# buckbaskin/parakeet_slam

Measured on AMD Instinct MI355X. Metric: particle*landmark EKF updates/sec (whole filter step), higher is better.
Workload: dtype f64

## Files before the change

### include/parakeet_slam.h

```cpp
#ifndef PARAKEET_SLAM_H_
#define PARAKEET_SLAM_H_

#include <stddef.h>
#include <stdint.h>

#ifdef __cplusplus
extern "C" {
#endif
#if defined(__GNUC__)
#pragma GCC visibility push(default)
#endif

#define PK_ABI_VERSION 1

typedef enum pk_status {
  PK_OK = 0,
  PK_ERR_INVALID = -1,
  PK_ERR_HIP = -2,
  PK_ERR_STATE = -3,
  PK_ERR_UNSUPPORTED = -4,
  PK_ERR_NOMEM = -5
} pk_status;

#define PK_LANDMARK_POTENTIAL 0x40000000
// ... 109 lines not shown
int pk_shard_plan_balanced_dev(pk_filter* f, const double* dev_global_state, int64_t global_particles, const double* dev_gmax,
                               int32_t weight_domain, double u, int32_t world, int32_t rank, int64_t* dev_table);
int pk_shard_pack_balanced_dev(pk_filter* f, const int64_t* table, int32_t world, int32_t rank, void* dev_buf);
int pk_shard_adopt_balanced_dev(pk_filter* f, const int64_t* table, int32_t world, int32_t rank, const void* dev_recv,
                                int64_t n_received, int32_t mode);
int pk_shard_pack_balanced_loop_dev(pk_filter* f, int64_t keep, int64_t a0, int64_t a1, void* dev_buf);
int pk_shard_download_logical(pk_filter* f, int64_t* logical);
int pk_shard_upload_logical(pk_filter* f, const int64_t* logical);
int pk_shard_download_balanced_plan(pk_filter* f, int64_t* rel, int64_t* Hl, int32_t* alive);
int pk_shard_reset_placement(pk_filter* f);
int pk_shard_download_balanced_offspring(pk_filter* f, int64_t global_particles, int64_t* H);
int pk_shard_balanced_errors(pk_filter* f, int64_t* count);

#define PK_PROBE_LEN 79
int pk_probe(int32_t device, const double pose[3], const double mean[5], const double cov[25],
             const double blob[4], const double Qt[16], double* out);

int pk_enable_timing(pk_filter* f, int32_t mask);
int pk_reset_timings(pk_filter* f);
int pk_timings(pk_filter* f, double ms[PK_T_COUNT], int64_t launches[PK_T_COUNT]);
int pk_observe_bytes(const pk_filter* f, int32_t num_blobs, int64_t* algorithmic, int64_t* moved);
enum {
  PK_ROUTE_NONE = 0,
  PK_ROUTE_KNOWN_IDS = 1,
  PK_ROUTE_ML_GENERAL = 2,
  PK_ROUTE_ML_HANDOFF = 3,
  PK_ROUTE_ML_SWEEP = 4,
  PK_ROUTE_ML_FUSED = 5,
  PK_ROUTE_ML_REGS = 6,
  PK_ROUTE_DENSE = 8,
  PK_ROUTE_ML_PUB_BIG = 9,
};
int pk_observe_route(const pk_filter* f);
int pk_download_sources(pk_filter* f, int32_t* src);
int pk_observe_flagged(pk_filter* f, int64_t* flagged, int64_t* cand_overflow);
int pk_observe_retry_rows(pk_filter* f, int64_t* wanted, int64_t* capacity);
int pk_observe_published(pk_filter* f, int32_t* published);
int pk_observe_pub_stats(pk_filter* f, int64_t stats[6]);
int pk_observe_flags(pk_filter* f, uint8_t* flags);

typedef struct pk_rng pk_rng;
int pk_rng_create_numpy(uint32_t seed, pk_rng** out);
int pk_rng_create_python(uint32_t seed, pk_rng** out);
int pk_rng_destroy(pk_rng* r);
int pk_rng_standard_normal(pk_rng* r, int64_t n, double* out);
int pk_rng_random(pk_rng* r, int64_t n, double* out);

#if defined(__GNUC__)
#pragma GCC visibility pop
#endif
#ifdef __cplusplus
}
#endif
#endif
```

### parakeet_slam_amd/_lib.py

```python
from __future__ import annotations

import ctypes as C
import os

import numpy as np

HERE = os.path.dirname(os.path.abspath(__file__))
LIB_PATH = os.path.join(HERE, "libparakeet_slam.so")

PK_OK = 0
PK_ERR_INVALID, PK_ERR_HIP, PK_ERR_STATE, PK_ERR_UNSUPPORTED, PK_ERR_NOMEM = -1, -2, -3, -4, -5
PK_WEIGHTS_LINEAR, PK_WEIGHTS_LOG = 0, 1
PK_LANDMARK_POTENTIAL = 0x40000000
PK_T_NAMES = ("motion", "assoc", "observe", "weights", "resample", "summary", "materialise")
PK_T_COUNT = len(PK_T_NAMES)
PK_PROBE_LEN = 79
PK_ABI_VERSION = 1

_dp = C.POINTER(C.c_double)
_ip = C.POINTER(C.c_int32)
_lp = C.POINTER(C.c_int64)
_bp = C.POINTER(C.c_uint8)
_h = C.c_void_p

# ... 43 lines not shown
    "pk_shard_plan_global_dev": (C.c_int, [_h, C.c_void_p, C.c_int64, C.c_void_p, C.c_int32, C.c_double, C.c_int32, C.c_int32,
                                           C.c_void_p]),
    "pk_shard_download_offspring": (C.c_int, [_h, _lp]),
    "pk_shard_pack_dev": (C.c_int, [_h, _lp, C.c_int32, C.c_int32, C.c_void_p]),
    "pk_shard_pack_slots_dev": (C.c_int, [_h, C.c_int64, C.c_int64, C.c_int64, C.c_int64, C.c_void_p]),
    "pk_shard_adopt_dev": (C.c_int, [_h, C.c_int32, C.c_void_p, C.c_int64]),
    "pk_shard_local_span_dev": (C.c_int, [_h, C.c_void_p]),
    "pk_shard_adopt_local_dev": (C.c_int, [_h, C.c_int32]),
    "pk_shard_adopt_remote_dev": (C.c_int, [_h, C.c_int32, C.c_void_p, C.c_int64]),
    "pk_shard_state_dev": (C.c_int, [_h, C.c_void_p]),
    "pk_shard_plan_balanced_dev": (C.c_int, [_h, C.c_void_p, C.c_int64, C.c_void_p, C.c_int32, C.c_double, C.c_int32, C.c_int32,
                                             C.c_void_p]),
    "pk_shard_pack_balanced_dev": (C.c_int, [_h, _lp, C.c_int32, C.c_int32, C.c_void_p]),
    "pk_shard_adopt_balanced_dev": (C.c_int, [_h, _lp, C.c_int32, C.c_int32, C.c_void_p, C.c_int64, C.c_int32]),
    "pk_shard_pack_balanced_loop_dev": (C.c_int, [_h, C.c_int64, C.c_int64, C.c_int64, C.c_void_p]),
    "pk_shard_download_logical": (C.c_int, [_h, _lp]),
    "pk_shard_reset_placement": (C.c_int, [_h]),
    "pk_shard_upload_logical": (C.c_int, [_h, _lp]),
    "pk_shard_download_balanced_plan": (C.c_int, [_h, _lp, _lp, _ip]),
    "pk_shard_download_balanced_offspring": (C.c_int, [_h, C.c_int64, _lp]),
    "pk_shard_balanced_errors": (C.c_int, [_h, _lp]),
    "pk_motion_range": (C.c_int, [_h, C.c_double, C.c_double, C.c_double, C.c_uint64, C.c_uint64, C.c_int64, C.c_int64]),
    "pk_staged_takes_regs": (C.c_int, [_h]),
    "pk_observe_staged_range": (C.c_int, [_h, C.c_int32, C.c_int64, C.c_int64, C.c_int32, C.c_int32]),
    "pk_particle_bytes": (C.c_int64, [_h]),
    "pk_pack_particles": (C.c_int, [_h, _lp, C.c_int64, C.c_void_p]),
    "pk_adopt_particles": (C.c_int, [_h, _lp, C.c_void_p, C.c_int64]),
    "pk_probe": (C.c_int, [C.c_int32, _dp, _dp, _dp, _dp, _dp, _dp]),
    "pk_enable_timing": (C.c_int, [_h, C.c_int32]),
    "pk_reset_timings": (C.c_int, [_h]),
    "pk_timings": (C.c_int, [_h, _dp, _lp]),
    "pk_observe_bytes": (C.c_int, [_h, C.c_int32, _lp, _lp]),
    "pk_observe_route": (C.c_int, [_h]),
    "pk_download_sources": (C.c_int, [_h, _ip]),
    "pk_observe_flagged": (C.c_int, [_h, _lp, _lp]),
    "pk_observe_retry_rows": (C.c_int, [_h, _lp, _lp]),
    "pk_grow_enable": (C.c_int, [_h, C.c_int32, C.c_int32, C.c_double]),
    "pk_grow_download": (C.c_int, [_h, C.c_int64, C.c_int64, _ip, _dp, _ip]),
    "pk_grow_upload": (C.c_int, [_h, C.c_int64, C.c_int64, _ip, _dp, _ip]),
    "pk_grow_shape": (C.c_int, [_h, C.POINTER(C.c_int32), C.POINTER(C.c_int32), C.POINTER(C.c_int32)]),
    "pk_observe_published": (C.c_int, [_h, C.POINTER(C.c_int32)]),
    "pk_observe_flags": (C.c_int, [_h, _bp]),
    "pk_observe_pub_stats": (C.c_int, [_h, _lp]),
    "pk_rng_create_numpy": (C.c_int, [C.c_uint32, C.POINTER(_h)]),
    "pk_rng_create_python": (C.c_int, [C.c_uint32, C.POINTER(_h)]),
    "pk_rng_destroy": (C.c_int, [_h]),
    "pk_rng_standard_normal": (C.c_int, [_h, C.c_int64, _dp]),
    "pk_rng_random": (C.c_int, [_h, C.c_int64, _dp]),
}


class PkError(RuntimeError):
    def __init__(self, status, message):
        super().__init__("parakeet_slam [%d]: %s" % (status, message))
        self.status = status


_lib = None


def load():
    global _lib
    if _lib is not None:
        return _lib
    if not os.path.exists(LIB_PATH):
        raise OSError(
# ... 264 lines not shown

    def shard_download_balanced_plan(self):
        rel, Hl, alive = np.empty(self.P + 1, dtype=np.int64), np.empty(self.P, dtype=np.int64), np.empty(self.P, dtype=np.int32)
        check(self._lib.pk_shard_download_balanced_plan(self._h, lptr(rel), lptr(Hl), iptr(alive)))
        return rel, Hl, alive[alive >= 0]

    def reset_placement(self):
        check(self._lib.pk_shard_reset_placement(self._h))

    def shard_download_balanced_offspring(self, global_particles):
        out = np.empty(int(global_particles) + 1, dtype=np.int64)
        check(self._lib.pk_shard_download_balanced_offspring(self._h, int(global_particles), lptr(out)))
        return out

    def shard_balanced_errors(self):
        out = np.zeros(1, dtype=np.int64)
        check(self._lib.pk_shard_balanced_errors(self._h, lptr(out)))
        return int(out[0])

    def motion_range(self, v, w, dt, seed, draw, p0, p1):
        check(self._lib.pk_motion_range(self._h, float(v), float(w), float(dt), int(seed), int(draw), int(p0), int(p1)))

    def staged_takes_regs(self):
        return bool(self._lib.pk_staged_takes_regs(self._h))

    def observe_staged_range(self, fresh, p0, p1, first, last):
        check(self._lib.pk_observe_staged_range(self._h, 1 if fresh else 0, int(p0), int(p1), 1 if first else 0, 1 if last else 0))

    ROUTES = {0: "none", 1: "known_ids", 2: "ml_general", 3: "ml_handoff", 4: "ml_sweep", 5: "ml_fused", 6: "ml_regs", 8: "dense", 9: "ml_pub_big"}

    def observe_route(self):
        return self.ROUTES[int(self._lib.pk_observe_route(self._h))]

    def observe_flagged(self):
        a, b = C.c_int64(), C.c_int64()
        check(self._lib.pk_observe_flagged(self._h, C.byref(a), C.byref(b)))
        return int(a.value), int(b.value)

    def observe_pub_stats(self):
        a = np.zeros(6, dtype=np.int64)
        check(self._lib.pk_observe_pub_stats(self._h, lptr(a)))
        return dict(zip(("entries", "contested_blobs", "multi_landmarks", "longest_list", "entry_capacity", "instance"), (int(v) for v in a)))

    def grow_enable(self, preset_landmarks, reading_capacity=64, pair_threshold=30.0):
        check(self._lib.pk_grow_enable(self._h, int(preset_landmarks), int(reading_capacity), float(pair_threshold)))

    def grow_shape(self):
        a, b, c = C.c_int32(), C.c_int32(), C.c_int32()
        check(self._lib.pk_grow_shape(self._h, C.byref(a), C.byref(b), C.byref(c)))
        return int(a.value), int(b.value), int(c.value)

    def grow_download(self, p0=0, p1=None, counters=True, readings=True, slot_ids=True):
        p1 = self.P if p1 is None else p1
        _, S, R = self.grow_shape()
        n = p1 - p0
        c = np.empty((n, 4), dtype=np.int32) if counters else None
        r = np.empty((n, R, 8), dtype=np.float64) if readings else None
        s = np.empty((n, S), dtype=np.int32) if slot_ids else None
        check(self._lib.pk_grow_download(self._h, int(p0), int(p1), iptr(c), dptr(r), iptr(s)))
        return c, r, s

    def grow_upload(self, p0, p1, counters=None, readings=None, slot_ids=None):
        _, S, R = self.grow_shape()
        n = p1 - p0
        c = None if counters is None else np.ascontiguousarray(counters, dtype=np.int32).reshape(n, 4)
        r = None if readings is None else f64(readings, (n, R, 8))
# ... 94 lines not shown
```

### parakeet_slam_amd/build.py

```python
from __future__ import annotations

import os
import shutil
import subprocess
import sys

_NO_LICM = ["-mllvm", "-disable-machine-licm"]
EXTRA_FLAGS = {"pk_k_observe_ml.hip": _NO_LICM, "pk_k_step_pub.hip": _NO_LICM, "pk_k_cand_entries.hip": _NO_LICM, "pk_k_assoc.hip": _NO_LICM}

HERE = os.path.dirname(os.path.abspath(__file__))
CSRC = os.path.join(HERE, "csrc")
LIB = os.path.join(HERE, "libparakeet_slam.so")
OBJDIR = os.path.join(HERE, "csrc", "_obj")

HIP_SOURCES = ["pk_k_motion.hip", "pk_k_assoc.hip", "pk_k_observe.hip", "pk_k_observe_ml.hip", "pk_k_step_pub.hip", "pk_k_cand_entries.hip", "pk_k_dense.hip", "pk_k_resample.hip", "pk_k_grow.hip", "pk_api.hip"]
CXX_SOURCES = ["pk_rng.cpp"]
HEADERS = [
    "pk_math.hpp", "pk_layout.hpp", "pk_kernels.hpp", "pk_philox.hpp", "pk_device.hpp", "pk_pub_math.hpp", "pk_pub_layout.hpp", "pk_k_step_duo.inl",
    os.path.join("..", "..", "include", "parakeet_slam.h"),
]

HIPCC_FLAGS = [
    "--offload-arch=gfx950", "-O3", "-std=c++17", "-fPIC", "-fvisibility=hidden",
    "-Wall", "-Wno-unused-function",
    "-ffp-contract=on",
]


def _hipcc():
    for cand in (os.environ.get("HIPCC"), shutil.which("hipcc"), "/opt/rocm/bin/hipcc"):
        if cand and os.path.exists(cand):
            return cand
    raise RuntimeError("hipcc not found (set HIPCC or add /opt/rocm/bin to PATH)")


def _stale(target, deps):
    if not os.path.exists(target):
        return True
    t = os.path.getmtime(target)
    return any(os.path.getmtime(d) > t for d in deps)


CXX_FLAGS = ["-x", "c++", "-O2", "-std=c++17", "-fPIC", "-fvisibility=hidden", "-ffp-contract=off", "-Wall"]


def _cxx_objects(hipcc, verbose=True):
    os.makedirs(OBJDIR, exist_ok=True)
    objs = []
# ... 68 lines not shown
```

### parakeet_slam_amd/csrc/pk_api.hip

```cpp
#include <hip/hip_runtime.h>

#include <cmath>
#include <cstdarg>
#include <cstdio>
#include <cstring>
#include <new>
#include <string>
#include <vector>

#include "../../include/parakeet_slam.h"
#include "pk_kernels.hpp"

using namespace pk;

extern "C" {
int pk_download_landmarks(pk_filter* f, int64_t p0, int64_t p1, double* means, double* covs, int32_t* counts);
int pk_upload_landmarks(pk_filter* f, int64_t p0, int64_t p1, const double* means, const double* covs, const int32_t* counts);
}

#ifdef PK_STAMPS
namespace pk { void debug_read_stamps(unsigned long long* out, bool reset); void debug_read_fused_stamps(unsigned long long* out, bool reset); void debug_read_regs_stamps(unsigned long long* out, bool reset); void debug_read_pub_stamps(unsigned long long* out, bool reset); void debug_read_pub_wave_stamps(unsigned long long* out, bool reset); }
#endif

namespace {
// ... 83 lines not shown
  int64_t* rlohi_dev = nullptr;
  int64_t rlohi_cap = 0;
  BalancedBuffers bal{};
  int64_t bal_m = -1;
  int64_t bal_loop_keep = -1;
  int assoc_kernel = 0;
  int assoc_dup = 1;
  struct Staged {
    bool valid = false;
    int B = 0;
    unsigned char* st = nullptr;
    int slot = 0;
    BlobGrid g{};
    int n9 = 0;
    bool use_grid = false;
    size_t tab_bytes = 0;
    bool uploaded = false;
  } staged;
  int route = PK_ROUTE_NONE;
  int upload_kernel = 1;
  int fused_step = 1;
  unsigned* bcnt_dev = nullptr;
  uint4* brec_dev = nullptr;
  int64_t bcand_cap = 0;
  int cand_lists = 1;
  int64_t loop_lo = INT64_MIN, loop_hi = INT64_MAX;
  uint4* cand_dev = nullptr;
  int regs_step = 1;
  int pub_step = 1;
  bool flag_folded = false;
  int pub_small = -1;
  int duo_park_limit = -1;
  int duo_on = 0;
  int pub_entry_limit = 0;
  uint4* erec_dev = nullptr;
  uint4* erec_dev2 = nullptr;
  unsigned* binfo_dev = nullptr;
  unsigned char* npass_dev = nullptr;
  unsigned* unm_dev = nullptr;
  int unm_words = 0;
  int64_t unm_cap = 0;
  bool grow_bits = false;
  uint4* prim_dev = nullptr;
  float4* gate4_dev = nullptr;
  uint4* far_dev = nullptr;
  int far_prune = 1;
  unsigned* glist_dev = nullptr;
  struct Split {
    bool active = false;
    AssocLaunch al;
    CandTable cand;
    int B = 0;
    bool reset = false;
  } split;
  bool adopt_local_done = false;
  int pub_ecap = 0;
  int split_reserve_cus = 16;
  int regs_retry = 1;
  int regs_warm = 1;
  int fast_observe = 1;
  uint4* sweep_results = nullptr;
  size_t sweep_cap = 0;
  unsigned* retry_seen = nullptr;
  int64_t retry_rows_min = 0;
  FastHandoff fh{};
  int64_t fh_cap_l = 0, fh_cap_b = 0;
// ... 153 lines not shown
    f->stage_cap = cap;
  }
  int i = f->stage_next;
  f->stage_next = (i + 1) % pk_filter::kRing;
  const uint64_t need = f->slot_seq[i];
  if (need != 0) {
    int ev = -1;
    for (int j = 0; j < pk_filter::kRing; ++j)
      if (f->event_seq[j] >= need && (ev < 0 || f->event_seq[j] < f->event_seq[ev])) ev = j;
    if (ev < 0) {
      PK_HIP(hipEventRecord(f->stage_done[i], f->stream));
      f->event_seq[i] = f->upload_seq;
      ev = i;
    }
    PK_HIP(hipEventSynchronize(f->stage_done[ev]));
    f->slot_seq[i] = 0;
  }
  *out = f->stage[i];
  *slot = i;
  return PK_OK;
}

int materialise(pk_filter* f) {
  if (f->src_identity) return PK_OK;
  {
    Span t(f, PK_T_MATERIALISE);
    launch_materialise(f->stream, f->d);
  }
  f->src_identity = true;
  f->d.alt = nullptr;
  return PK_OK;
}

void pack_landmark(const MapLayout& lay, unsigned char* slot, int l, const double* mean, const double* cov) {
  double* fl = reinterpret_cast<double*>(slot);
  const int Lp = lay.Lp;
  for (int i = 0; i < 5; ++i) fl[(size_t)i * Lp + l] = mean[i];
  if (lay.fields == kDenseFields) {
    for (int i = 0; i < 25; ++i) fl[(size_t)(5 + i) * Lp + l] = cov[i];
    return;
  }
  fl[(size_t)F_PXX * Lp + l] = cov[0];
  fl[(size_t)F_PXY * Lp + l] = 0.5 * (cov[1] + cov[5]);
  fl[(size_t)F_PYY * Lp + l] = cov[6];
  fl[(size_t)F_CRR * Lp + l] = cov[12];
  fl[(size_t)F_CRG * Lp + l] = 0.5 * (cov[13] + cov[17]);
  fl[(size_t)F_CRB * Lp + l] = 0.5 * (cov[14] + cov[22]);
  fl[(size_t)F_CGG * Lp + l] = cov[18];
  fl[(size_t)F_CGB * Lp + l] = 0.5 * (cov[19] + cov[23]);
  fl[(size_t)F_CBB * Lp + l] = cov[24];
}

void unpack_landmark(const MapLayout& lay, const unsigned char* slot, int l, double* mean, double* cov) {
  const double* fl = reinterpret_cast<const double*>(slot);
  const int Lp = lay.Lp;
  if (mean)
    for (int i = 0; i < 5; ++i) mean[i] = fl[(size_t)i * Lp + l];
  if (cov && lay.fields == kDenseFields) {
    for (int i = 0; i < 25; ++i) cov[i] = fl[(size_t)(5 + i) * Lp + l];
  } else if (cov) {
    for (int i = 0; i < 25; ++i) cov[i] = 0.0;
    cov[0] = fl[(size_t)F_PXX * Lp + l];
    cov[1] = cov[5] = fl[(size_t)F_PXY * Lp + l];
    cov[6] = fl[(size_t)F_PYY * Lp + l];
    cov[12] = fl[(size_t)F_CRR * Lp + l];
    cov[13] = cov[17] = fl[(size_t)F_CRG * Lp + l];
// ... 255 lines not shown
        (!onepass_only || (step_pub_entry_capacity(B) > 0 && regs_cand_lds_bytes(f->d.lay.Lp, B) <= kMaxDynLds && B <= 32 * 96))) {
      out->retry = f->regs_retry && observe_sweep_plan(f->d, B).grid > 0;
      if ((rc = ensure_handoff(f, B, out->retry ? kSweepSlots : kFastSlots, out->retry, true))) return rc;
      out->regs = true;
      out->grid = g;
      out->n9 = n9;
      out->tables = f->scan_dev + o_tab;
      out->exact = reinterpret_cast<const double*>(f->scan_dev + o_exact);
      const size_t cs_b = ((size_t)(g.ncell + 1) * 2 + 15) & ~(size_t)15;
      out->order = reinterpret_cast<const unsigned short*>(f->scan_dev + o_tab + cs_b + (size_t)B * 16 + (size_t)n9 * 2);
      return PK_OK;
    }
    if (out && want_fast && !finalize && f->fast_observe == 1 && f->pub_step && f->cand_lists && f->d.lay.L > kRegsMaxL &&
        f->d.lay.L <= kPubBigMaxL && B > 0 && step_pub_big_entry_capacity(B) > 0 && observe_sweep_plan(f->d, B).grid > 0 && pub_ok) {
      if ((rc = ensure_handoff(f, B, kSweepSlots, true, true))) return rc;
      out->big = true;
      out->retry = true;
      out->grid = g;
      out->n9 = n9;
      out->tables = f->scan_dev + o_tab;
      out->exact = reinterpret_cast<const double*>(f->scan_dev + o_exact);
      const size_t cs_b = ((size_t)(g.ncell + 1) * 2 + 15) & ~(size_t)15;
      out->order = reinterpret_cast<const unsigned short*>(f->scan_dev + o_tab + cs_b + (size_t)B * 16 + (size_t)n9 * 2);
      return PK_OK;
    }
    if (want_fast && !onepass_only && !finalize && f->fast_observe && B > 0 &&
        (sweep ? observe_sweep_plan(f->d, B).grid > 0 : observe_fast_lds_bytes(B) <= kMaxDynLds)) {
      const int slots = (sweep && (B >= 3000 || f->fast_observe == 3)) ? kSweepSlots : kFastSlots;
      if ((rc = ensure_handoff(f, B, slots))) return rc;
      f->fh.slots = slots;
      fh = f->fh;
      fh.n_flagged = ctl_n_flagged(f);
    }
    Span t(f, PK_T_ASSOC);
    CandTable cand;
    if (fh.lmpass && f->cand_lists && f->d.lay.L < 65535) {
      if (!f->cand_dev && (rc = dev_alloc(f, &f->cand_dev, ((size_t)f->d.lay.Lp + kCandSpare) * 3))) return rc;
      launch_summary_partials(f->stream, f->d, f->partial, f->out4);
      launch_candidates(f->stream, f->d, B, reinterpret_cast<const double*>(f->scan_dev + o_exact), 0, f->cand_dev, ctl_cand_over(f),
                        nullptr, nullptr, nullptr, 2 * kCandSlots, f->out4);
      cand.rec = f->cand_dev;
      cand.over = ctl_cand_over(f);
      cand.slots = 2 * kCandSlots;
    }
    launch_assoc_grid(f->stream, f->d, B, g, n9, f->scan_dev + o_tab, reinterpret_cast<const double*>(f->scan_dev + o_exact),
                      f->ids_dev, finalize, fh, cand);
    if (out) {
      out->fast = fh.lmpass != nullptr;
      out->exact = reinterpret_cast<const double*>(f->scan_dev + o_exact);
      const size_t cs_b = ((size_t)(g.ncell + 1) * 2 + 15) & ~(size_t)15;
      out->order = reinterpret_cast<const unsigned short*>(f->scan_dev + o_tab + cs_b + (size_t)B * 16 + (size_t)n9 * 2);
    }
    return PK_OK;
  }
  if (assoc_brute_lds_bytes(B) > kMaxDynLds)
    return fail(PK_ERR_UNSUPPORTED,
                "maximum-likelihood association of %d blobs: neither the colour-grid tables nor the brute-force kernel's "
                "%zu bytes of per-blob state fit the workgroup's %zu bytes of LDS", B, assoc_brute_lds_bytes(B), (size_t)kMaxDynLds);
  Span t(f, PK_T_ASSOC);
  launch_assoc_brute(f->stream, f->d, blobs_dev, dir_dev, B, f->ids_dev);
  return PK_OK;
}

int classify_covariance(const double* cov, int l) {
  double scale = 0.0;
  for (int i = 0; i < 25; ++i) {
    if (!std::isfinite(cov[i])) return fail(PK_ERR_INVALID, "landmark %d: covariance not finite", l + 1);
    if (i % 6 == 0) scale = fmax(scale, fabs(cov[i]));
  }
  const double tol = 1e-9 * (scale > 0 ? scale : 1.0);
  for (int i = 0; i < 2; ++i)
    for (int j = 2; j < 5; ++j)
      if (fabs(cov[i * 5 + j]) > 1e-14 * scale || fabs(cov[j * 5 + i]) > 1e-14 * scale) return 1;
  for (int i = 0; i < 5; ++i)
    for (int j = i + 1; j < 5; ++j)
      if (fabs(cov[i * 5 + j] - cov[j * 5 + i]) > tol) return 1;
  return 0;
}

int check_block_diagonal(const double* cov, int l) {
  double scale = 0.0;
  for (int i = 0; i < 5; ++i) scale = fmax(scale, fabs(cov[i * 6]));
  if (!(scale >= 0.0) || !std::isfinite(scale))
    return fail(PK_ERR_INVALID, "landmark %d: covariance diagonal is not finite", l + 1);
  const double tol = 1e-9 * (scale > 0 ? scale : 1.0);
  for (int i = 0; i < 2; ++i)
    for (int j = 2; j < 5; ++j)
      if (fabs(cov[i * 5 + j]) > 1e-14 * scale || fabs(cov[j * 5 + i]) > 1e-14 * scale)
        return fail(PK_ERR_UNSUPPORTED,
                    "landmark %d: covariance couples position and colour (entry [%d][%d]); the compact "
                    "device layout holds xy 2x2 (+) rgb 3x3 only",
                    l + 1, i, j);
  for (int i = 0; i < 5; ++i)
    for (int j = i + 1; j < 5; ++j) {
      if (!std::isfinite(cov[i * 5 + j])) return fail(PK_ERR_INVALID, "landmark %d: covariance not finite", l + 1);
      if (fabs(cov[i * 5 + j] - cov[j * 5 + i]) > tol)
        return fail(PK_ERR_UNSUPPORTED, "landmark %d: covariance is not symmetric", l + 1);
    }
  return PK_OK;
}

int relayout(pk_filter* f, bool dense, bool keep) {
  if (f->dense == dense) return PK_OK;
  int rc;
  DeviceState& d = f->d;
  const MapLayout old = d.lay;
  const MapLayout neu = MapLayout::make(old.L, sizeof(double), dense ? kDenseFields : (int)F_COUNT_FIELDS);
  const int64_t P = d.P;
  const int L = old.L;
  std::vector<double> means, covs;
  std::vector<int32_t> counts;
  if (keep && L > 0) {
    if ((rc = materialise(f))) return rc;
    if (!dense)
      return fail(PK_ERR_STATE, "relayout: a dense map cannot be folded back into the compact layout");
    try {
      means.resize((size_t)P * L * 5);
      covs.resize((size_t)P * L * 25);
      counts.resize((size_t)P * L);
    } catch (const std::bad_alloc&) {
      return fail(PK_ERR_NOMEM, "relayout: no host memory to stage %lld x %d landmarks for the layout conversion", (long long)P, L);
    }
    if ((rc = pk_download_landmarks(f, 0, P, means.data(), covs.data(), counts.data()))) return rc;
  }
  PK_HIP(hipStreamSynchronize(f->stream));
  for (int i = 0; i < 2; ++i) {
    if (d.map[i]) (void)hipFree(d.map[i]);
    d.map[i] = nullptr;
    f->device_bytes -= (int64_t)((size_t)P * old.slot_bytes);
  }
  if (f->slot_tmp) (void)hipFree(f->slot_tmp);
  f->slot_tmp = nullptr;
  f->device_bytes -= (int64_t)old.slot_bytes;
  d.lay = neu;
  f->dense = dense;
  d.alt = nullptr;
  for (int i = 0; i < 2; ++i) {
// ... 120 lines not shown
  }
  for (auto e : f->pool) (void)hipEventDestroy(e);
  DeviceState& d = f->d;
  for (int i = 0; i < 2; ++i) {
    (void)hipFree(d.x[i]);
    (void)hipFree(d.y[i]);
    (void)hipFree(d.h[i]);
    (void)hipFree(d.logw[i]);
    (void)hipFree(d.src[i]);
    (void)hipFree(d.map[i]);
  }
  if (f->scan_dev) (void)hipFree(f->scan_dev);
  for (void* q : {(void*)f->fh.lmpass, (void*)f->fh.bcount, (void*)f->fh.pflag, (void*)f->fh.row_of, (void*)f->sweep_results, (void*)f->cand_dev, (void*)f->bcnt_dev, (void*)f->brec_dev, (void*)f->erec_dev, (void*)f->erec_dev2, (void*)f->binfo_dev, (void*)f->glist_dev, (void*)f->gate4_dev, (void*)f->npass_dev, (void*)f->far_dev, (void*)f->prim_dev, (void*)f->unm_dev})
    if (q) (void)hipFree(q);
  for (int i = 0; i < 2; ++i)
    for (void* q : {(void*)f->grow.hyp[i], (void*)f->grow.cnt[i], (void*)f->grow.slot_id[i]})
      if (q) (void)hipFree(q);
  for (void* q : {(void*)f->g_totals, (void*)f->g_offsets, (void*)f->hi_dev, (void*)f->gl_clocal, (void*)f->gl_totals, (void*)f->gl_offsets, (void*)f->plan_ticket, (void*)f->idx_dev, (void*)f->srcs_dev, (void*)f->rlohi_dev})
    if (q) (void)hipFree(q);
  for (void* q : {(void*)d.logical[0], (void*)d.logical[1], (void*)f->bal.glogw, (void*)f->bal.clocal, (void*)f->bal.totals, (void*)f->bal.offsets,
                  (void*)f->bal.sum, (void*)f->bal.H, (void*)f->bal.cloc, (void*)f->bal.ctot, (void*)f->bal.coff, (void*)f->bal.rel, (void*)f->bal.Hl,
                  (void*)f->bal.alive, (void*)f->bal.bad})
    if (q) (void)hipFree(q);
  void* rest[] = {d.immutable, f->z_dev,  f->ids_dev,
                  f->partial,  f->gmax,   f->clocal,    f->totals,      f->offsets,   f->sum,      f->out4, f->pose_part,
                  f->anc,      f->slot_tmp};
  for (void* p : rest)
    if (p) (void)hipFree(p);
  for (int i = 0; i < pk_filter::kRing; ++i) {
    if (f->stage[i]) (void)hipHostFree(f->stage[i]);
    if (f->stage_done[i]) (void)hipEventDestroy(f->stage_done[i]);
  }
  if (f->retry_seen) (void)hipHostFree(f->retry_seen);
  if (f->own_stream) (void)hipStreamDestroy(f->own_stream);
  delete f;
  return PK_OK;
}

int pk_set_stream(pk_filter* f, void* hip_stream) {
  if (!f) return fail(PK_ERR_INVALID, "pk_set_stream: NULL handle");
  int rc;
  if ((rc = use_device(f))) return rc;
  if ((rc = drain_timings(f))) return rc;
  PK_HIP(hipStreamSynchronize(f->stream));
  f->stream = hip_stream ? (hipStream_t)hip_stream : f->own_stream;
  return PK_OK;
}

int pk_synchronize(pk_filter* f) {
  if (!f) return fail(PK_ERR_INVALID, "pk_synchronize: NULL handle");
  int rc;
  if ((rc = use_device(f))) return rc;
  PK_HIP(hipStreamSynchronize(f->stream));
  return PK_OK;
}

int64_t pk_num_particles(const pk_filter* f) { return f ? f->d.P : -1; }
int32_t pk_num_landmarks(const pk_filter* f) { return f ? f->d.lay.L : -1; }
int64_t pk_device_bytes(const pk_filter* f) { return f ? f->device_bytes : -1; }

int pk_set_measurement_noise(pk_filter* f, const double Qt[16]) {
  if (!f || !Qt) return fail(PK_ERR_INVALID, "pk_set_measurement_noise: NULL argument");
  for (int i = 0; i < 16; ++i)
    if (!std::isfinite(Qt[i])) return fail(PK_ERR_INVALID, "Qt is not finite");
  double scale = 0;
  for (int i = 0; i < 4; ++i) scale = fmax(scale, fabs(Qt[i * 5]));
  bool coupled = false;
  for (int j = 1; j < 4; ++j)
    if (fabs(Qt[j]) > 1e-14 * scale || fabs(Qt[j * 4]) > 1e-14 * scale) coupled = true;
  for (int i = 1; i < 4; ++i)
    for (int j = i + 1; j < 4; ++j)
      if (fabs(Qt[i * 4 + j] - Qt[j * 4 + i]) > 1e-9 * (scale > 0 ? scale : 1.0)) coupled = true;
  int rc;
  if ((rc = use_device(f))) return rc;
  if (coupled && !f->dense && (rc = relayout(f, true, f->map_loaded))) return rc;
  for (int i = 0; i < 16; ++i) f->qt16[i] = Qt[i];
  f->qt_dense = coupled;
  f->qt = NoiseD{Qt[0], Qt[5], 0.5 * (Qt[6] + Qt[9]), 0.5 * (Qt[7] + Qt[13]), Qt[10], 0.5 * (Qt[11] + Qt[14]), Qt[15]};
  return PK_OK;
}

int pk_upload_map(pk_filter* f, const double* means, const double* covs, const uint8_t* immutable) {
  if (!f) return fail(PK_ERR_INVALID, "pk_upload_map: NULL handle");
  const MapLayout& lay = f->d.lay;
  const int L = lay.L;
  if (L > 0 && (!means || !covs)) return fail(PK_ERR_INVALID, "pk_upload_map: NULL means/covs");
  int rc;
  if ((rc = use_device(f))) return rc;
  bool need_dense = f->qt_dense;
  for (int l = 0; l < L; ++l) {
    for (int i = 0; i < 5; ++i)
      if (!std::isfinite(means[l * 5 + i])) return fail(PK_ERR_INVALID, "landmark %d: mean is not finite", l + 1);
    const int c = classify_covariance(covs + (size_t)l * 25, l);
    if (c < 0) return c;
    need_dense |= c == 1;
  }
  if ((rc = relayout(f, need_dense, false))) return rc;
  std::vector<unsigned char> slot(lay.slot_bytes, 0);
  std::vector<unsigned char> imm((size_t)lay.Lp, 0);
  for (int l = 0; l < L; ++l) {
    pack_landmark(lay, slot.data(), l, means + (size_t)l * 5, covs + (size_t)l * 25);
    imm[l] = immutable ? (immutable[l] != 0) : 0;
  }
  PK_HIP(hipMemcpyAsync(f->slot_tmp, slot.data(), lay.slot_bytes, hipMemcpyHostToDevice, f->stream));
  PK_HIP(hipMemcpyAsync(f->d.immutable, imm.data(), imm.size(), hipMemcpyHostToDevice, f->stream));
  launch_broadcast_slot(f->stream, f->d, f->slot_tmp);
  PK_HIP(hipStreamSynchronize(f->stream));
  f->src_identity = true;
  f->map_loaded = true;
  return PK_OK;
}

int pk_upload_poses(pk_filter* f, const double* xyhw) {
  if (f) f->pose_part_ok = false;
  if (!f || !xyhw) return fail(PK_ERR_INVALID, "pk_upload_poses: NULL argument");
  int rc;
  if ((rc = use_device(f))) return rc;
  const int64_t P = f->d.P;
  std::vector<double> soa((size_t)P * 4);
  for (int64_t i = 0; i < P; ++i) {
    soa[i] = xyhw[4 * i];
    soa[P + i] = xyhw[4 * i + 1];
    soa[2 * P + i] = xyhw[4 * i + 2];
    double w = xyhw[4 * i + 3];
    if (!(w >= 0.0) || !std::isfinite(w)) return fail(PK_ERR_INVALID, "pk_upload_poses: weight of particle %lld is negative, infinite or NaN", (long long)i);
    soa[3 * P + i] = std::log(w);
  }
  const int c = f->d.cur;
  PK_HIP(hipMemcpyAsync(f->d.x[c], soa.data(), P * 8, hipMemcpyHostToDevice, f->stream));
  PK_HIP(hipMemcpyAsync(f->d.y[c], soa.data() + P, P * 8, hipMemcpyHostToDevice, f->stream));
  PK_HIP(hipMemcpyAsync(f->d.h[c], soa.data() + 2 * P, P * 8, hipMemcpyHostToDevice, f->stream));
  PK_HIP(hipMemcpyAsync(f->d.logw[c], soa.data() + 3 * P, P * 8, hipMemcpyHostToDevice, f->stream));
  PK_HIP(hipStreamSynchronize(f->stream));
  f->gmax_fused = false;
  return PK_OK;
}

int pk_upload_pose(pk_filter* f, int64_t p, const double xyhw[4]) {
  if (!f || !xyhw) return fail(PK_ERR_INVALID, "pk_upload_pose: NULL argument");
// ... 20 lines not shown
  const int64_t P = f->d.P;
  std::vector<double> soa((size_t)P * 4);
  const int c = f->d.cur;
  PK_HIP(hipMemcpyAsync(soa.data(), f->d.x[c], P * 8, hipMemcpyDeviceToHost, f->stream));
  PK_HIP(hipMemcpyAsync(soa.data() + P, f->d.y[c], P * 8, hipMemcpyDeviceToHost, f->stream));
  PK_HIP(hipMemcpyAsync(soa.data() + 2 * P, f->d.h[c], P * 8, hipMemcpyDeviceToHost, f->stream));
  PK_HIP(hipMemcpyAsync(soa.data() + 3 * P, f->d.logw[c], P * 8, hipMemcpyDeviceToHost, f->stream));
  PK_HIP(hipStreamSynchronize(f->stream));
  for (int64_t i = 0; i < P; ++i) {
    xyhw[4 * i] = soa[i];
    xyhw[4 * i + 1] = soa[P + i];
    xyhw[4 * i + 2] = soa[2 * P + i];
    xyhw[4 * i + 3] = std::exp(soa[3 * P + i]);
  }
  return PK_OK;
}

int pk_download_log_weights(pk_filter* f, double* logw) {
  if (!f || !logw) return fail(PK_ERR_INVALID, "pk_download_log_weights: NULL argument");
  int rc;
  if ((rc = use_device(f))) return rc;
  PK_HIP(hipMemcpyAsync(logw, f->d.logw[f->d.cur], (size_t)f->d.P * sizeof(double), hipMemcpyDeviceToHost, f->stream));
  PK_HIP(hipStreamSynchronize(f->stream));
  return PK_OK;
}

int pk_download_landmarks(pk_filter* f, int64_t p0, int64_t p1, double* means, double* covs, int32_t* counts) {
  if (!f) return fail(PK_ERR_INVALID, "pk_download_landmarks: NULL handle");
  if (p0 < 0 || p1 < p0 || p1 > f->d.P) return fail(PK_ERR_INVALID, "pk_download_landmarks: bad particle range");
  if (!f->map_loaded) return fail(PK_ERR_STATE, "pk_download_landmarks: no map uploaded");
  int rc;
  if ((rc = use_device(f))) return rc;
  if ((rc = materialise(f))) return rc;
  const MapLayout& lay = f->d.lay;
  const int L = lay.L;
  const int64_t chunk = std::max<int64_t>(1, (int64_t)(64u << 20) / (int64_t)lay.slot_bytes);
  std::vector<unsigned char> host((size_t)std::min<int64_t>(chunk, p1 - p0) * lay.slot_bytes);
  for (int64_t q0 = p0; q0 < p1; q0 += chunk) {
    int64_t q1 = std::min(p1, q0 + chunk);
    PK_HIP(hipMemcpyAsync(host.data(), f->d.map[f->d.mcur] + (size_t)q0 * lay.slot_bytes,
                          (size_t)(q1 - q0) * lay.slot_bytes, hipMemcpyDeviceToHost, f->stream));
    PK_HIP(hipStreamSynchronize(f->stream));
    for (int64_t q = q0; q < q1; ++q) {
      const unsigned char* slot = host.data() + (size_t)(q - q0) * lay.slot_bytes;
      const int32_t* cnt = reinterpret_cast<const int32_t*>(slot + lay.count_off);
      for (int l = 0; l < L; ++l) {
        size_t o = (size_t)(q - p0) * L + l;
        unpack_landmark(lay, slot, l, means ? means + o * 5 : nullptr, covs ? covs + o * 25 : nullptr);
        if (counts) counts[o] = cnt[l];
      }
    }
  }
  return PK_OK;
}

int pk_upload_landmarks(pk_filter* f, int64_t p0, int64_t p1, const double* means, const double* covs,
                        const int32_t* counts) {
  if (!f) return fail(PK_ERR_INVALID, "pk_upload_landmarks: NULL handle");
  if (p0 < 0 || p1 < p0 || p1 > f->d.P) return fail(PK_ERR_INVALID, "pk_upload_landmarks: bad particle range");
  if (!f->map_loaded) return fail(PK_ERR_STATE, "pk_upload_landmarks: no map uploaded");
  int rc;
  if ((rc = use_device(f))) return rc;
  if ((rc = materialise(f))) return rc;
  const int L = f->d.lay.L;
  if (means)
    for (int64_t o = 0; o < (p1 - p0) * L * 5; ++o)
      if (!std::isfinite(means[o])) return fail(PK_ERR_INVALID, "pk_upload_landmarks: mean of landmark %d not finite", (int)((o / 5) % L) + 1);
  if (covs) {
    bool need_dense = false;
    for (int64_t o = 0; o < (p1 - p0) * L; ++o) {
      const int c = classify_covariance(covs + (size_t)o * 25, (int)(o % L));
      if (c < 0) return c;
      need_dense |= c == 1;
    }
    if (need_dense && !f->dense && (rc = relayout(f, true, true))) return rc;
  }
  const MapLayout& lay = f->d.lay;
  const int64_t chunk = std::max<int64_t>(1, (int64_t)(64u << 20) / (int64_t)lay.slot_bytes);
  std::vector<unsigned char> host;
  try {
    host.resize((size_t)std::min<int64_t>(chunk, p1 - p0) * lay.slot_bytes);
  } catch (const std::bad_alloc&) {
    return fail(PK_ERR_NOMEM, "pk_upload_landmarks: no host memory for the staging buffer");
  }
  for (int64_t q0 = p0; q0 < p1; q0 += chunk) {
    int64_t q1 = std::min(p1, q0 + chunk);
    unsigned char* dev = f->d.map[f->d.mcur] + (size_t)q0 * lay.slot_bytes;
    PK_HIP(hipMemcpyAsync(host.data(), dev, (size_t)(q1 - q0) * lay.slot_bytes, hipMemcpyDeviceToHost, f->stream));
    PK_HIP(hipStreamSynchronize(f->stream));
    for (int64_t q = q0; q < q1; ++q) {
      unsigned char* slot = host.data() + (size_t)(q - q0) * lay.slot_bytes;
      int32_t* cnt = reinterpret_cast<int32_t*>(slot + lay.count_off);
      for (int l = 0; l < L; ++l) {
        size_t o = (size_t)(q - p0) * L + l;
        double m[5], c[25];
// ... 205 lines not shown
      const bool fold = whole && (far != nullptr || f->grow_on || al.fused);
      launch_cand_entries(f->stream, f->d, B, f->cand_dev, f->erec_dev, f->bcnt_dev, f->brec_dev, f->binfo_dev, f->glist_dev, ctl_cand_over(f),
                          ctl_skip_pub(f), ctl_skip_cand(f), ecap, kCandSlots, nullptr, nullptr, f->npass_dev, far != nullptr, ctl_pub_stats(f),
                          nullptr, nullptr, DuoLimits(), nullptr, fold ? f->fh.pflag : nullptr, fold ? ctl_n_flagged(f) : nullptr);
      f->flag_folded = fold;
      cand->far = far;
      cand->skip_cand = ctl_skip_cand(f);
      f->pub_ecap = ecap;
    } else {
      launch_candidates(f->stream, f->d, B, al.exact, ref, f->cand_dev, ctl_cand_over(f), nullptr, nullptr, nullptr, kCandSlots, f->out4, nullptr, nullptr, part);
    }
  }
  return PK_OK;
}
static int onepass_launch(pk_filter* f, const AssocLaunch& al, int B, const ObserveExtras& ex, const CandTable& cand, int64_t p0,
                          int64_t p1, int reserve_cus = 0) {
  FastHandoff fh = f->fh;
  fh.n_flagged = ctl_n_flagged(f);
  fh.flags_only = true;
  Span t(f, PK_T_OBSERVE);
  ObserveExtras e1 = ex;
  e1.flip = false;
  if (al.big) {
    const DuoLimits duo = duo_limits(f, B);
    if (duo.tbytes > 0)
      launch_step_pub_duo(f->stream, f->d, B, al.exact, al.order, fh, f->qt, e1, cand, f->erec_dev2, f->glist_dev, ctl_skip_duo(f), ctl_pub_stats(f), duo,
                          f->gate4_dev, f->prim_dev, p0, p1, reserve_cus);
    launch_step_pub_big(f->stream, f->d, B, al.exact, al.order, fh, f->qt, e1, cand, f->erec_dev2, f->glist_dev, ctl_skip_big(f), f->pub_ecap, f->gate4_dev,
                        p0, p1, reserve_cus, f->prim_dev, ctl_pub_stats(f));
    if (!f->flag_folded) launch_flag_range_if(f->stream, ctl_skip_pub(f), fh.pflag, fh.n_flagged, p0, p1);
  } else if (al.regs) {
    if (f->pub_ecap > 0 && cand.rec)
      launch_step_pub(f->stream, f->d, B, al.exact, al.order, fh, f->qt, e1, cand, f->erec_dev, f->glist_dev, ctl_skip_pub(f), f->pub_ecap,
                      p0, p1, reserve_cus);
    if ((cand.far || f->grow_on) && f->pub_ecap > 0) {
      if (!f->flag_folded) launch_flag_range_if(f->stream, ctl_skip_pub(f), fh.pflag, fh.n_flagged, p0, p1);
    } else
      launch_step_regs(f->stream, f->d, B, al.grid, al.n9, al.tables, al.exact, al.order, fh, f->qt, e1, f->regs_warm, cand, p0, p1,
                       reserve_cus);
  } else {
    if (f->pub_ecap > 0 && cand.rec)
      launch_step_pub(f->stream, f->d, B, al.exact, al.order, fh, f->qt, e1, cand, f->erec_dev, f->glist_dev, ctl_skip_pub(f), f->pub_ecap,
                      p0, p1, reserve_cus);
    if (f->pub_ecap > 0 && cand.rec) {
      if (!f->flag_folded) launch_flag_range_if(f->stream, ctl_skip_pub(f), fh.pflag, fh.n_flagged, p0, p1);
    } else
      launch_step_fused(f->stream, f->d, B, al.grid, al.n9, al.tables, al.exact, al.order, fh, f->qt, e1,
                        (f->pub_ecap > 0 && cand.rec) ? ctl_skip_pub(f) : nullptr);
  }
  return PK_OK;
}
static int onepass_finish(pk_filter* f, const AssocLaunch& al, int B, const ObserveExtras& ex, const CandTable& cand) {
  int rc;
  FastHandoff fh = f->fh;
  fh.n_flagged = ctl_n_flagged(f);
  fh.flags_only = true;
  if ((al.regs || al.big) && al.retry) {
    Span t(f, PK_T_ASSOC);
    const SweepPlan plan = observe_sweep_plan(f->d, B);
    const size_t need = (size_t)plan.grid * plan.results_per_wg;
    if (need > f->sweep_cap) {
      PK_HIP(hipStreamSynchronize(f->stream));
      if (f->sweep_results) (void)hipFree(f->sweep_results);
      f->sweep_results = nullptr;
      f->sweep_cap = 0;
      if ((rc = dev_alloc(f, &f->sweep_results, need))) return rc;
      f->sweep_cap = need;
    }
    FastHandoff fr = f->fh;
    fr.slots = kSweepSlots;
    fr.retry = true;
    fr.n_flagged = ctl_n_flagged(f);
    fr.row_next = ctl_retry_rows(f);
    fr.row_cap = retry_rows(f);
    launch_assoc_grid(f->stream, f->d, B, al.grid, al.n9, al.tables, al.exact, f->ids_dev, false, fr, cand.far ? CandTable{} : cand);
    ObserveExtras e3 = ex;
// ... 9 lines not shown
  launch_assoc_grid(f->stream, f->d, B, al.grid, al.n9, al.tables, al.exact, f->ids_dev, false, fh);
  ObserveExtras e2 = ex;
  e2.only_flagged = f->fh.pflag;
  e2.n_flagged = ctl_n_flagged(f);
  launch_observe(f->stream, f->d, al.blobs, al.dir, B, nullptr, nullptr, 0, f->ids_dev, f->qt, e2);
  return PK_OK;
}

static int observe_impl(pk_filter* f, const double* blobs, int32_t B, const int32_t* ids, int32_t* ids_out,
                        bool reset) {
  if (!f) return fail(PK_ERR_INVALID, "pk_observe: NULL handle");
  if (B < 0 || (B > 0 && !blobs)) return fail(PK_ERR_INVALID, "pk_observe: bad blobs");
  if (!f->map_loaded) return fail(PK_ERR_STATE, "pk_observe: no map uploaded (pk_upload_map)");
  if (f->split.active) return fail(PK_ERR_STATE, "pk_observe: a split observe is in progress (pk_observe_staged_range with last = 1 ends it)");
  int rc;
  if ((rc = use_device(f))) return rc;
  const MapLayout& lay = f->d.lay;
  const int L = lay.L;
  for (int i = 0; i < 4 * B; ++i)
    if (!std::isfinite(blobs[i])) return fail(PK_ERR_INVALID, "pk_observe: blob %d is not finite", i / 4);
  static const int32_t no_ids = 0;
  if (!ids && B == 0) ids = &no_ids;
  if (ids)
    for (int b = 0; b < B; ++b)
      if (ids[b] < 0 || ids[b] > L) return fail(PK_ERR_INVALID, "pk_observe: ids[%d] = %d outside 0..%d", b, ids[b], L);
  const bool grow = f->grow_on && B > 0;
  if (grow && ids) return fail(PK_ERR_STATE, "pk_observe: the new-landmark bookkeeping (pk_grow_enable) follows the maximum-likelihood association: no ids");
  if (grow && f->dense)
    return fail(PK_ERR_STATE, "pk_observe: the new-landmark bookkeeping (pk_grow_enable) writes the compact landmark layout; this filter "
                              "is on the dense one (a covariance or Qt that couples position and colour)");
  if (f->dense) return dense_observe(f, blobs, B, ids, ids_out, reset, true);
  ObserveExtras ex;
  ex.reset = reset;
  if (ids) {
    f->staged.valid = false;
    const size_t o_blobs = kCtlBytes;
    const size_t o_first = o_blobs + (size_t)B * 4 * sizeof(double);
    const size_t o_next = o_first + (size_t)lay.Lp * sizeof(int32_t);
    const size_t total = o_next + (size_t)B * sizeof(int32_t);
    unsigned char* st = nullptr;
    int slot = 0;
    if ((rc = take_stage(f, total, &st, &slot))) return rc;
    if ((rc = ensure_scan_capacity(f, total))) return rc;
    memset(st, 0, kCtlBytes);
    if (B > 0) memcpy(st + o_blobs, blobs, (size_t)B * 4 * sizeof(double));
    int32_t* first = reinterpret_cast<int32_t*>(st + o_first);
    int32_t* next = reinterpret_cast<int32_t*>(st + o_next);
    std::vector<int32_t> last((size_t)lay.Lp, -1);
    for (int l = 0; l < lay.Lp; ++l) first[l] = -1;
    int n0 = 0;
    ex.single_sightings = true;
    for (int b = 0; b < B; ++b) {
      next[b] = -1;
      int id = ids[b];
      if (id == 0) {
        ++n0;
        continue;
      }
      if (first[id - 1] < 0) {
        first[id - 1] = b;
      } else {
        next[last[id - 1]] = b;
        ex.single_sightings = false;
      }
      last[id - 1] = b;
    }
// ... 11 lines not shown
    f->d.alt = nullptr;
    f->gmax_fused = true;
    f->route = PK_ROUTE_KNOWN_IDS;
    if (ids_out)
      for (int64_t p = 0; p < f->d.P; ++p) memcpy(ids_out + (size_t)p * B, ids, (size_t)B * 4);
    return PK_OK;
  }
  AssocLaunch al;
  if ((rc = enqueue_association(f, blobs, B, false, ids_out == nullptr, &al, grow))) return rc;
  f->grow_bits = false;
  if (grow && (al.fused || al.regs || al.big)) {
    al.retry = false;
    const int words = 2 * ((B + 63) / 64);
    if ((int64_t)f->d.P * words > f->unm_cap) {
      PK_HIP(hipStreamSynchronize(f->stream));
      if (f->unm_dev) (void)hipFree(f->unm_dev);
      f->unm_dev = nullptr;
      f->unm_cap = 0;
      const int64_t cap = (int64_t)f->d.P * (words + words / 4 + 2);
      if ((rc = dev_alloc(f, &f->unm_dev, (size_t)cap))) return rc;
      f->unm_cap = cap;
    }
    f->unm_words = words;
    ex.unm = f->unm_dev;
    ex.unm_words = words;
    f->grow_bits = true;
  }
  ex.gmax_key = ctl_gmax_key(f);
  f->route = al.big ? PK_ROUTE_ML_PUB_BIG
             : al.fused ? PK_ROUTE_ML_FUSED
             : al.regs ? PK_ROUTE_ML_REGS
             : !al.fast ? PK_ROUTE_ML_GENERAL
             : (f->d.lay.L > kFastMaxL || f->fast_observe >= 2) ? PK_ROUTE_ML_SWEEP : PK_ROUTE_ML_HANDOFF;
  if (al.fused || al.regs || al.big) {
    CandTable cand;
    if ((rc = onepass_prepare(f, al, B, &cand, 0, true))) return rc;
    if ((rc = onepass_launch(f, al, B, ex, cand, 0, f->d.P))) return rc;
    if ((rc = onepass_finish(f, al, B, ex, cand))) return rc;
  } else {
    Span t(f, PK_T_OBSERVE);
    if (al.fast) {
      ObserveExtras e1 = ex;
      e1.flip = false;
      if (f->d.lay.L > kFastMaxL || f->fast_observe >= 2) {
        const SweepPlan plan = observe_sweep_plan(f->d, B);
        const size_t need = (size_t)plan.grid * plan.results_per_wg;
        if (need > f->sweep_cap) {
          PK_HIP(hipStreamSynchronize(f->stream));
          if (f->sweep_results) (void)hipFree(f->sweep_results);
          f->sweep_results = nullptr;
          f->sweep_cap = 0;
          if ((rc = dev_alloc(f, &f->sweep_results, need))) return rc;
          f->sweep_cap = need;
        }
        launch_observe_sweep(f->stream, f->d, B, al.exact, al.order, f->fh, f->qt, e1, plan, f->sweep_results);
      } else {
        launch_observe_fast(f->stream, f->d, B, al.exact, al.order, f->fh, f->qt, e1);
      }
      ObserveExtras e2 = ex;
      e2.only_flagged = f->fh.pflag;
      e2.n_flagged = ctl_n_flagged(f);
      launch_observe(f->stream, f->d, al.blobs, al.dir, B, nullptr, nullptr, 0, f->ids_dev, f->qt, e2);
    } else {
      launch_observe(f->stream, f->d, al.blobs, al.dir, B, nullptr, nullptr, 0, f->ids_dev, f->qt, ex);
    }
  }
  PK_LAUNCH_CHECK("pk_observe");
  f->src_identity = true;
  f->d.alt = nullptr;
  f->gmax_fused = true;
  if (grow) {
// ... 26 lines not shown
  int rc;
  if ((rc = use_device(f))) return rc;
  if (f->dense) {
    f->dense_staged.assign(blobs, blobs + 4 * (size_t)B);
    return PK_OK;
  }
  f->dense_staged.clear();
  return stage_ml_scan(f, blobs, B);
}

int pk_observe_staged(pk_filter* f, int32_t fresh) {
  if (!f) return fail(PK_ERR_INVALID, "pk_observe_staged: NULL handle");
  if (f->dense && !f->dense_staged.empty()) {
    std::vector<double> b;
    b.swap(f->dense_staged);
    return observe_impl(f, b.data(), (int32_t)(b.size() / 4), nullptr, nullptr, fresh != 0);
  }
  if (!f->staged.valid) return fail(PK_ERR_STATE, "pk_observe_staged: no staged scan (pk_stage_scan)");
  const double* blobs = reinterpret_cast<const double*>(f->staged.st + kCtlBytes);
  return observe_impl(f, blobs, f->staged.B, nullptr, nullptr, fresh != 0);
}

int pk_staged_takes_regs(pk_filter* f) {
  if (!f || f->dense || f->grow_on || !f->staged.valid || !f->staged.use_grid) return 0;
  return regs_route_taken(f, f->staged.g, f->staged.B, f->staged.n9) ? 1 : 0;
}

int pk_observe_staged_range(pk_filter* f, int32_t fresh, int64_t p0, int64_t p1, int32_t first, int32_t last) {
  if (!f) return fail(PK_ERR_INVALID, "pk_observe_staged_range: NULL handle");
  if (p0 < 0 || p1 < p0 || p1 > f->d.P) return fail(PK_ERR_INVALID, "pk_observe_staged_range: bad particle range [%lld, %lld)", (long long)p0, (long long)p1);
  if (f->grow_on) return fail(PK_ERR_STATE, "pk_observe_staged_range: the new-landmark bookkeeping (pk_grow_enable) runs behind whole observes (pk_observe / pk_observe_staged)");
  int rc;
  if ((rc = use_device(f))) return rc;
  pk_filter::Split& sp = f->split;
  if (first) {
    if (sp.active) return fail(PK_ERR_STATE, "pk_observe_staged_range: the previous split observe was not finished (last = 1)");
    if (!pk_staged_takes_regs(f))
      return fail(PK_ERR_STATE, "pk_observe_staged_range: needs a staged scan that takes the register route (pk_staged_takes_regs)");
    const double* blobs = reinterpret_cast<const double*>(f->staged.st + kCtlBytes);
    sp.B = f->staged.B;
    sp.reset = fresh != 0;
    sp.al = AssocLaunch();
    if ((rc = enqueue_association(f, blobs, sp.B, false, true, &sp.al))) return rc;
    if (!sp.al.regs && !sp.al.big) return fail(PK_ERR_STATE, "pk_observe_staged_range: the scan did not take the register route");
    f->route = sp.al.big ? PK_ROUTE_ML_PUB_BIG : PK_ROUTE_ML_REGS;
    sp.cand = CandTable();
    if ((rc = onepass_prepare(f, sp.al, sp.B, &sp.cand, p1 > p0 ? p0 : 0))) return rc;
    sp.active = true;
  } else if (!sp.active) {
    return fail(PK_ERR_STATE, "pk_observe_staged_range: no split observe in progress (first = 1)");
  }
  ObserveExtras ex;
  ex.reset = sp.reset;
  ex.gmax_key = ctl_gmax_key(f);
  if (p1 > p0 && (rc = onepass_launch(f, sp.al, sp.B, ex, sp.cand, p0, p1, (first && !last) ? f->split_reserve_cus : 0))) {
    sp.active = false;
    return rc;
  }
  if (last) {
    sp.active = false;
    if ((rc = onepass_finish(f, sp.al, sp.B, ex, sp.cand))) return rc;
    PK_LAUNCH_CHECK("pk_observe_staged_range");
    f->src_identity = true;
    f->d.alt = nullptr;
    f->gmax_fused = true;
  }
  return PK_OK;
}

int pk_motion_range(pk_filter* f, double v, double w, double dt, uint64_t seed, uint64_t draw, int64_t p0, int64_t p1) {
  if (f) f->pose_part_ok = false;
  if (!f) return fail(PK_ERR_INVALID, "pk_motion_range: NULL handle");
  if (!std::isfinite(v) || !std::isfinite(w) || !std::isfinite(dt)) return fail(PK_ERR_INVALID, "pk_motion_range: non-finite control");
  if (p0 < 0 || p1 < p0 || p1 > f->d.P) return fail(PK_ERR_INVALID, "pk_motion_range: bad particle range [%lld, %lld)", (long long)p0, (long long)p1);
  int rc;
  if ((rc = use_device(f))) return rc;
  Span t(f, PK_T_MOTION);
  launch_motion_range(f->stream, f->d, v, w, dt, seed, draw, p0, p1);
  PK_LAUNCH_CHECK("pk_motion_range");
  return PK_OK;
}

int pk_associate(pk_filter* f, const double* blobs, int32_t B, int32_t* ids_out) {
  if (!f || !ids_out) return fail(PK_ERR_INVALID, "pk_associate: NULL argument");
  if (B < 0 || (B > 0 && !blobs)) return fail(PK_ERR_INVALID, "pk_associate: bad blobs");
  if (!f->map_loaded) return fail(PK_ERR_STATE, "pk_associate: no map uploaded (pk_upload_map)");
  if (B == 0) return PK_OK;
  int rc;
  if ((rc = use_device(f))) return rc;
  for (int i = 0; i < 4 * B; ++i)
    if (!std::isfinite(blobs[i])) return fail(PK_ERR_INVALID, "pk_associate: blob %d is not finite", i / 4);
  if (f->dense) return dense_observe(f, blobs, B, nullptr, ids_out, false, false);
  if ((rc = enqueue_association(f, blobs, B, true, false, nullptr))) return rc;
  PK_LAUNCH_CHECK("pk_associate");
  PK_HIP(hipMemcpyAsync(ids_out, f->ids_dev, (size_t)f->d.P * B * 4, hipMemcpyDeviceToHost, f->stream));
  PK_HIP(hipStreamSynchronize(f->stream));
  return PK_OK;
}

int pk_set_option(pk_filter* f, const char* name, int64_t value) {
  if (!f || !name) return fail(PK_ERR_INVALID, "pk_set_option: NULL argument");
  if (!strcmp(name, "assoc_kernel")) {
    if (value != 0 && value != 1) return fail(PK_ERR_INVALID, "assoc_kernel: 0 (colour grid) or 1 (brute force)");
    f->assoc_kernel = (int)value;
    return PK_OK;
  }
  if (!strcmp(name, "fast_observe")) {
    if (value < 0 || value > 3)
      return fail(PK_ERR_INVALID, "fast_observe: 0 (general kernels), 1 (default), 2 (always the sweep kernel) or 3 (... with eight slots)");
    f->fast_observe = (int)value;
    return PK_OK;
  }
  if (!strcmp(name, "timing_stride")) {
    if (value < 1 || value > 1000000) return fail(PK_ERR_INVALID, "timing_stride: 1 .. 1000000");
    f->timing_stride = (int)value;
    return PK_OK;
  }
  if (!strcmp(name, "upload_kernel")) {
    f->upload_kernel = value != 0;
    return PK_OK;
  }
  if (!strcmp(name, "fused_step")) {
    f->fused_step = value != 0;
    return PK_OK;
  }
  if (!strcmp(name, "cand_lists")) {
    f->cand_lists = value != 0;
    return PK_OK;
  }
  if (!strcmp(name, "pub_step")) {
    f->pub_step = value != 0;
    return PK_OK;
  }
  if (!strcmp(name, "pub_small")) {
// ... 148 lines not shown
        {
          Span t(f, PK_T_MOTION);
          launch_motion(f->stream, f->d, v, w, dt, nullptr, seed, draw, 0, f->scan_dev, dev_view, staged_upload_bytes(sg), f->pose_part);
      f->pose_part_ok = true;
        }
        sg.uploaded = true;
        f->gmax_fused = false;
        if ((rc = note_upload(f, sg.slot))) return rc;
        const double* staged_blobs = reinterpret_cast<const double*>(sg.st + kCtlBytes);
        if ((rc = observe_impl(f, staged_blobs, B, nullptr, nullptr, true))) return rc;
        return pk_resample(f, u, weight_domain, nullptr);
      }
      (void)hipGetLastError();
    }
  }
  if ((rc = pk_motion(f, v, w, dt, z, seed, draw))) return rc;
  if ((rc = observe_impl(f, blobs, B, ids, nullptr, true))) return rc;
  return pk_resample(f, u, weight_domain, nullptr);
}

int pk_grow_enable(pk_filter* f, int32_t preset_landmarks, int32_t reading_capacity, double pair_threshold) {
  if (!f) return fail(PK_ERR_INVALID, "pk_grow_enable: NULL handle");
  const int L = f->d.lay.L;
  if (preset_landmarks < 0 || preset_landmarks >= L)
    return fail(PK_ERR_INVALID, "pk_grow_enable: %d preset landmarks leave no spare slot among the filter's %d", preset_landmarks, L);
  if (reading_capacity < 1 || reading_capacity > 65536) return fail(PK_ERR_INVALID, "pk_grow_enable: reading_capacity %d outside 1..65536", reading_capacity);
  if (!(pair_threshold >= 0.0)) return fail(PK_ERR_INVALID, "pk_grow_enable: pair_threshold %g", pair_threshold);
  if (f->grow_on) return fail(PK_ERR_STATE, "pk_grow_enable: already enabled on this filter");
  if (f->dense)
    return fail(PK_ERR_STATE, "pk_grow_enable: the bookkeeping kernel writes the compact landmark layout; this filter is on the dense one "
                              "(a covariance or Qt that couples position and colour)");
  int rc;
  if ((rc = use_device(f))) return rc;
  GrowState& g = f->grow;
  g.L0 = preset_landmarks;
  g.S = L - preset_landmarks;
  g.R = reading_capacity;
  g.pair_threshold = pair_threshold;
  g.cur = 0;
  const size_t P = (size_t)f->d.P;
  for (int i = 0; i < 2; ++i) {
    if ((rc = dev_alloc(f, &g.hyp[i], P * g.R * 8))) return rc;
    if ((rc = dev_alloc(f, &g.cnt[i], P * 4))) return rc;
    if ((rc = dev_alloc(f, &g.slot_id[i], P * g.S))) return rc;
  }
  std::vector<int32_t> c0(P * 4, 0);
  for (size_t p = 0; p < P; ++p) c0[4 * p + 2] = preset_landmarks + 1;
  PK_HIP(hipMemcpyAsync(g.cnt[0], c0.data(), P * 16, hipMemcpyHostToDevice, f->stream));
  PK_HIP(hipStreamSynchronize(f->stream));
  f->grow_on = true;
  return PK_OK;
}

static int grow_range(pk_filter* f, const char* who, int64_t p0, int64_t p1) {
  if (!f) return fail(PK_ERR_INVALID, "%s: NULL handle", who);
  if (!f->grow_on) return fail(PK_ERR_STATE, "%s: pk_grow_enable was not called on this filter", who);
  if (p0 < 0 || p1 < p0 || p1 > f->d.P) return fail(PK_ERR_INVALID, "%s: particles [%lld, %lld) of %lld", who, (long long)p0, (long long)p1, (long long)f->d.P);
  return use_device(f);
}

int pk_grow_download(pk_filter* f, int64_t p0, int64_t p1, int32_t* counters, double* readings, int32_t* slot_ids) {
  int rc;
  if ((rc = grow_range(f, "pk_grow_download", p0, p1))) return rc;
  const GrowState& g = f->grow;
  const size_t n = (size_t)(p1 - p0);
  if (n == 0) return PK_OK;
  if (counters) PK_HIP(hipMemcpyAsync(counters, g.cnt[g.cur] + 4 * p0, n * 16, hipMemcpyDeviceToHost, f->stream));
  if (readings) PK_HIP(hipMemcpyAsync(readings, g.hyp[g.cur] + (size_t)p0 * g.R * 8, n * g.R * 64, hipMemcpyDeviceToHost, f->stream));
  if (slot_ids) PK_HIP(hipMemcpyAsync(slot_ids, g.slot_id[g.cur] + (size_t)p0 * g.S, n * g.S * 4, hipMemcpyDeviceToHost, f->stream));
  PK_HIP(hipStreamSynchronize(f->stream));
  return PK_OK;
}

int pk_grow_upload(pk_filter* f, int64_t p0, int64_t p1, const int32_t* counters, const double* readings, const int32_t* slot_ids) {
  int rc;
  if ((rc = grow_range(f, "pk_grow_upload", p0, p1))) return rc;
  const GrowState& g = f->grow;
// ... 14 lines not shown
int pk_grow_shape(const pk_filter* f, int32_t* preset_landmarks, int32_t* spare_slots, int32_t* reading_capacity) {
  if (!f) return fail(PK_ERR_INVALID, "pk_grow_shape: NULL handle");
  if (preset_landmarks) *preset_landmarks = f->grow_on ? f->grow.L0 : 0;
  if (spare_slots) *spare_slots = f->grow_on ? f->grow.S : 0;
  if (reading_capacity) *reading_capacity = f->grow_on ? f->grow.R : 0;
  return PK_OK;
}

int pk_shard_max_logw(pk_filter* f, double* max_logw) {
  if (!f || !max_logw) return fail(PK_ERR_INVALID, "pk_shard_max_logw: NULL argument");
  int rc;
  if ((rc = use_device(f))) return rc;
  launch_block_max(f->stream, f->d, f->partial, f->gmax);
  PK_HIP(hipMemcpyAsync(max_logw, f->gmax, sizeof(double), hipMemcpyDeviceToHost, f->stream));
  PK_HIP(hipStreamSynchronize(f->stream));
  return PK_OK;
}

int64_t pk_shard_num_blocks(const pk_filter* f) { return f ? f->nblocks : -1; }

int pk_shard_block_totals(pk_filter* f, double gmax, int32_t weight_domain, double* totals) {
  if (!f || !totals) return fail(PK_ERR_INVALID, "pk_shard_block_totals: NULL argument");
  int rc;
  if ((rc = use_device(f))) return rc;
  PK_HIP(hipMemcpyAsync(f->gmax, &gmax, sizeof(double), hipMemcpyHostToDevice, f->stream));
  launch_scan_local(f->stream, f->d, f->gmax, weight_domain, f->clocal, f->totals);
  PK_HIP(hipMemcpyAsync(totals, f->totals, (size_t)f->nblocks * sizeof(double), hipMemcpyDeviceToHost, f->stream));
  PK_HIP(hipStreamSynchronize(f->stream));
  return PK_OK;
}

int pk_set_shard(pk_filter* f, int64_t global_offset) {
  if (!f || global_offset < 0) return fail(PK_ERR_INVALID, "pk_set_shard: bad argument");
  f->d.global_offset = global_offset;
  return PK_OK;
}

int pk_shard_offspring(pk_filter* f, const double* global_totals, int64_t n_global_blocks, int64_t first_block,
                       int64_t global_particles, double u, int32_t last_shard, int64_t* slot_hi) {
  if (!f || !global_totals || !slot_hi) return fail(PK_ERR_INVALID, "pk_shard_offspring: NULL argument");
  if (!(u >= 0.0 && u < 1.0)) return fail(PK_ERR_INVALID, "pk_shard_offspring: u = %g outside [0,1)", u);
  if (first_block < 0 || first_block + f->nblocks > n_global_blocks || global_particles < f->d.P)
    return fail(PK_ERR_INVALID, "pk_shard_offspring: shard [%lld, +%lld) does not fit %lld global blocks",
                (long long)first_block, (long long)f->nblocks, (long long)n_global_blocks);
  int rc;
  if ((rc = use_device(f))) return rc;
  if (n_global_blocks > f->gblocks_cap) {
    PK_HIP(hipStreamSynchronize(f->stream));
    if (f->g_totals) (void)hipFree(f->g_totals);
    if (f->g_offsets) (void)hipFree(f->g_offsets);
    f->g_totals = f->g_offsets = nullptr;
    f->gblocks_cap = 0;
    if ((rc = dev_alloc(f, &f->g_totals, (size_t)n_global_blocks))) return rc;
    if ((rc = dev_alloc(f, &f->g_offsets, (size_t)n_global_blocks + 1))) return rc;
    f->gblocks_cap = n_global_blocks;
  }
  if (!f->hi_dev && (rc = dev_alloc(f, &f->hi_dev, (size_t)f->d.P + 1))) return rc;
  PK_HIP(hipMemcpyAsync(f->g_totals, global_totals, (size_t)n_global_blocks * sizeof(double), hipMemcpyHostToDevice,
                        f->stream));
  {
    Span t(f, PK_T_WEIGHTS);
    launch_scan_blocks(f->stream, f->g_totals, n_global_blocks, f->g_offsets, f->sum);
    launch_offspring(f->stream, f->clocal, f->g_offsets, f->sum, first_block, f->d.P, global_particles, u,
                     last_shard ? 1 : 0, f->hi_dev);
  }
  PK_HIP(hipMemcpyAsync(slot_hi, f->hi_dev, ((size_t)f->d.P + 1) * sizeof(int64_t), hipMemcpyDeviceToHost, f->stream));
  PK_HIP(hipStreamSynchronize(f->stream));
  return PK_OK;
}

static size_t record_stride(const pk_filter* f) { return kPoseRecordBytes + f->d.lay.slot_bytes + (f->grow_on ? grow_tail_bytes(f->grow) : 0); }
int64_t pk_particle_bytes(const pk_filter* f) { return f ? (int64_t)record_stride(f) : -1; }

int pk_pack_particles(pk_filter* f, const int64_t* local_idx, int64_t n, void* dev_buf) {
  if (!f || n < 0 || (n > 0 && (!local_idx || !dev_buf))) return fail(PK_ERR_INVALID, "pk_pack_particles: bad argument");
  if (f->grow_on) return fail(PK_ERR_STATE, "pk_pack_particles: the new-landmark bookkeeping (pk_grow_enable) travels with the balanced placement only (pk_shard_*_balanced_dev)");
  if (n > f->d.P) return fail(PK_ERR_INVALID, "pk_pack_particles: %lld records from %lld particles", (long long)n, (long long)f->d.P);
  for (int64_t i = 0; i < n; ++i)
    if (local_idx[i] < 0 || local_idx[i] >= f->d.P) return fail(PK_ERR_INVALID, "pk_pack_particles: index %lld out of range", (long long)local_idx[i]);
  if (n == 0) return PK_OK;
  int rc;
  if ((rc = use_device(f))) return rc;
  if (!f->idx_dev && (rc = dev_alloc(f, &f->idx_dev, (size_t)f->d.P))) return rc;
  PK_HIP(hipMemcpyAsync(f->idx_dev, local_idx, (size_t)n * sizeof(int64_t), hipMemcpyHostToDevice, f->stream));
  {
    Span t(f, PK_T_RESAMPLE);
    launch_pack(f->stream, f->d, f->idx_dev, n, static_cast<unsigned char*>(dev_buf));
  }
  PK_HIP(hipStreamSynchronize(f->stream));
  return PK_OK;
}

int pk_adopt_particles(pk_filter* f, const int64_t* src, const void* dev_buf, int64_t n_received) {
  if (f) f->pose_part_ok = false;
  if (!f || !src || n_received < 0 || (n_received > 0 && !dev_buf)) return fail(PK_ERR_INVALID, "pk_adopt_particles: bad argument");
  if (f->grow_on) return fail(PK_ERR_STATE, "pk_adopt_particles: the new-landmark bookkeeping (pk_grow_enable) travels with the balanced placement only (pk_shard_*_balanced_dev)");
  const int64_t P = f->d.P;
  for (int64_t k = 0; k < P; ++k)
    if (src[k] >= P || src[k] < -n_received) return fail(PK_ERR_INVALID, "pk_adopt_particles: src[%lld] = %lld out of range", (long long)k, (long long)src[k]);
  if (f->d.logical[0]) return fail(PK_ERR_STATE, "pk_adopt_particles: the balanced placement is active on this filter (its slots carry logical indices): resample through pk_shard_plan_balanced_dev / pk_shard_adopt_balanced_dev");
  int rc;
  if ((rc = use_device(f))) return rc;
  if (f->d.alt) {
    f->src_identity = false;
    if ((rc = materialise(f))) return rc;
  }
  if (!f->srcs_dev && (rc = dev_alloc(f, &f->srcs_dev, (size_t)P))) return rc;
  PK_HIP(hipMemcpyAsync(f->srcs_dev, src, (size_t)P * sizeof(int64_t), hipMemcpyHostToDevice, f->stream));
  {
    Span t(f, PK_T_RESAMPLE);
    launch_adopt(f->stream, f->d, f->srcs_dev, static_cast<const unsigned char*>(dev_buf));
  }
  if (n_received == 0) f->d.alt = nullptr;
  f->src_identity = false;
  f->gmax_fused = false;
  PK_HIP(hipStreamSynchronize(f->stream));
  return PK_OK;
}

int pk_shard_max_logw_dev(pk_filter* f, double* dev_out) {
  if (!f || !dev_out) return fail(PK_ERR_INVALID, "pk_shard_max_logw_dev: NULL argument");
  int rc;
  if ((rc = use_device(f))) return rc;
  Span t(f, PK_T_WEIGHTS);
  if (f->gmax_fused)
    launch_keys_max(f->stream, ctl_gmax_key(f), dev_out);
  else
    launch_block_max(f->stream, f->d, f->partial, dev_out);
  return PK_OK;
}

int pk_shard_block_totals_dev(pk_filter* f, const double* dev_gmax, int32_t weight_domain, double* dev_totals) {
  if (!f || !dev_totals || (weight_domain == PK_WEIGHTS_LOG && !dev_gmax))
    return fail(PK_ERR_INVALID, "pk_shard_block_totals_dev: NULL argument");
  int rc;
// ... 70 lines not shown
    if ((rc = dev_alloc(f, &f->gl_clocal, (size_t)global_particles))) return rc;
    if ((rc = dev_alloc(f, &f->gl_totals, (size_t)nbg))) return rc;
    if ((rc = dev_alloc(f, &f->gl_offsets, (size_t)nbg + 1))) return rc;
    f->gl_cap = global_particles;
  }
  if (!f->hi_dev && (rc = dev_alloc(f, &f->hi_dev, (size_t)P + 1))) return rc;
  Span t(f, PK_T_WEIGHTS);
  launch_scan_local_of(f->stream, dev_global_logw, global_particles, dev_gmax ? dev_gmax : f->gmax, weight_domain, f->gl_clocal,
                       f->gl_totals);
  launch_scan_blocks(f->stream, f->gl_totals, nbg, f->gl_offsets, f->sum);
  launch_offspring_global(f->stream, f->gl_clocal, f->gl_offsets, f->sum, goff, P, global_particles, u, last_shard ? 1 : 0,
                          f->hi_dev);
  launch_shard_ranges(f->stream, f->hi_dev, P, world, dev_ranges);
  PK_LAUNCH_CHECK("pk_shard_plan_global_dev");
  return PK_OK;
}

int pk_shard_download_offspring(pk_filter* f, int64_t* slot_hi) {
  if (!f || !slot_hi) return fail(PK_ERR_INVALID, "pk_shard_download_offspring: NULL argument");
  if (!f->hi_dev) return fail(PK_ERR_STATE, "pk_shard_download_offspring: no plan yet");
  int rc;
  if ((rc = use_device(f))) return rc;
  PK_HIP(hipMemcpyAsync(slot_hi, f->hi_dev, ((size_t)f->d.P + 1) * sizeof(int64_t), hipMemcpyDeviceToHost, f->stream));
  PK_HIP(hipStreamSynchronize(f->stream));
  return PK_OK;
}

int pk_shard_pack_dev(pk_filter* f, const int64_t* ranges, int32_t world, int32_t rank, void* dev_buf) {
  if (f && f->grow_on) return fail(PK_ERR_STATE, "pk_shard_pack_dev: the new-landmark bookkeeping (pk_grow_enable) travels with the balanced placement only (pk_shard_*_balanced_dev)");
  if (!f || !ranges || world < 1 || rank < 0 || rank >= world) return fail(PK_ERR_INVALID, "pk_shard_pack_dev: bad argument");
  if (!f->hi_dev) return fail(PK_ERR_STATE, "pk_shard_pack_dev: call pk_shard_plan_dev first");
  int rc;
  if ((rc = use_device(f))) return rc;
  const int64_t P = f->d.P;
  const size_t stride = kPoseRecordBytes + f->d.lay.slot_bytes;
  int64_t rec = 0;
  Span t(f, PK_T_RESAMPLE);
  for (int d = 0; d < world; ++d) {
    if (d == rank) continue;
    const int64_t j0 = ranges[2 * d], j1 = ranges[2 * d + 1];
    if (j0 < 0 || j1 < j0 || j1 > P) return fail(PK_ERR_INVALID, "pk_shard_pack_dev: range [%lld, %lld) for rank %d", (long long)j0, (long long)j1, d);
    if (j1 > j0 && !dev_buf) return fail(PK_ERR_INVALID, "pk_shard_pack_dev: NULL buffer");
    launch_pack_range(f->stream, f->d, f->hi_dev, j0, j1 - j0, (int64_t)d * P, (int64_t)(d + 1) * P,
                      static_cast<unsigned char*>(dev_buf) + (size_t)rec * stride);
    rec += j1 - j0;
  }
  return PK_OK;
}

int pk_shard_pack_slots_dev(pk_filter* f, int64_t j0, int64_t j1, int64_t slot_lo, int64_t slot_hi, void* dev_buf) {
  if (f && f->grow_on) return fail(PK_ERR_STATE, "pk_shard_pack_slots_dev: the new-landmark bookkeeping (pk_grow_enable) travels with the balanced placement only (pk_shard_*_balanced_dev)");
  if (!f || j0 < 0 || j1 < j0 || j1 > f->d.P || slot_hi < slot_lo) return fail(PK_ERR_INVALID, "pk_shard_pack_slots_dev: bad argument");
  if (!f->hi_dev) return fail(PK_ERR_STATE, "pk_shard_pack_slots_dev: call pk_shard_plan_dev first");
  if (j1 > j0 && !dev_buf) return fail(PK_ERR_INVALID, "pk_shard_pack_slots_dev: NULL buffer");
  int rc;
  if ((rc = use_device(f))) return rc;
  Span t(f, PK_T_RESAMPLE);
  launch_pack_range(f->stream, f->d, f->hi_dev, j0, j1 - j0, slot_lo, slot_hi, static_cast<unsigned char*>(dev_buf));
  PK_LAUNCH_CHECK("pk_shard_pack_slots_dev");
  return PK_OK;
}

int pk_shard_adopt_dev(pk_filter* f, int32_t rank, const void* dev_recv, int64_t n_received) {
  if (f && f->grow_on) return fail(PK_ERR_STATE, "pk_shard_adopt_dev: the new-landmark bookkeeping (pk_grow_enable) travels with the balanced placement only (pk_shard_*_balanced_dev)");
  if (f) f->pose_part_ok = false;
  if (!f || rank < 0 || n_received < 0 || (n_received > 0 && !dev_recv)) return fail(PK_ERR_INVALID, "pk_shard_adopt_dev: bad argument");
  if (!f->hi_dev) return fail(PK_ERR_STATE, "pk_shard_adopt_dev: call pk_shard_plan_dev first");
  if (f->d.logical[0]) return fail(PK_ERR_STATE, "pk_shard_adopt_dev: the balanced placement is active on this filter (its slots carry logical indices): resample through pk_shard_plan_balanced_dev / pk_shard_adopt_balanced_dev");
  int rc;
  if ((rc = use_device(f))) return rc;
  if (f->d.alt) {
    f->src_identity = false;
    if ((rc = materialise(f))) return rc;
  }
  if (n_received > f->rlohi_cap) {
    PK_HIP(hipStreamSynchronize(f->stream));
    if (f->rlohi_dev) (void)hipFree(f->rlohi_dev);
    f->rlohi_dev = nullptr;
    f->rlohi_cap = 0;
    if ((rc = dev_alloc(f, &f->rlohi_dev, (size_t)(2 * n_received + 2 * n_received / 4 + 16)))) return rc;
    f->rlohi_cap = n_received + n_received / 4;
  }
  Span t(f, PK_T_RESAMPLE);
  launch_adopt_dev(f->stream, f->d, f->hi_dev, (int64_t)rank * f->d.P, static_cast<const unsigned char*>(dev_recv),
                   n_received, f->rlohi_dev);
  f->src_identity = false;
  f->gmax_fused = false;
  return PK_OK;
}

int pk_shard_adopt_local_dev(pk_filter* f, int32_t rank) {
  if (f && f->grow_on) return fail(PK_ERR_STATE, "pk_shard_adopt_local_dev: the new-landmark bookkeeping (pk_grow_enable) travels with the balanced placement only (pk_shard_*_balanced_dev)");
  if (f) f->pose_part_ok = false;
  if (!f || rank < 0) return fail(PK_ERR_INVALID, "pk_shard_adopt_local_dev: bad argument");
  if (!f->hi_dev) return fail(PK_ERR_STATE, "pk_shard_adopt_local_dev: call pk_shard_plan_dev first");
  if (f->d.logical[0]) return fail(PK_ERR_STATE, "pk_shard_adopt_local_dev: the balanced placement is active on this filter (its slots carry logical indices): resample through pk_shard_plan_balanced_dev / pk_shard_adopt_balanced_dev");
  int rc;
  if ((rc = use_device(f))) return rc;
  if (f->d.alt) {
    f->src_identity = false;
    if ((rc = materialise(f))) return rc;
  }
  Span t(f, PK_T_RESAMPLE);
  const int64_t base = (int64_t)rank * f->d.P;
  launch_adopt_dev(f->stream, f->d, f->hi_dev, base, nullptr, 0, nullptr, 1, f->loop_lo == INT64_MIN ? INT64_MIN : base + f->loop_lo,
                   f->loop_hi == INT64_MAX ? INT64_MAX : base + f->loop_hi);
  f->src_identity = false;
  f->gmax_fused = false;
  f->adopt_local_done = true;
  return PK_OK;
}

int pk_shard_adopt_remote_dev(pk_filter* f, int32_t rank, const void* dev_recv, int64_t n_received) {
  if (f && f->grow_on) return fail(PK_ERR_STATE, "pk_shard_adopt_remote_dev: the new-landmark bookkeeping (pk_grow_enable) travels with the balanced placement only (pk_shard_*_balanced_dev)");
  if (f) f->pose_part_ok = false;
  if (!f || rank < 0 || n_received < 0 || (n_received > 0 && !dev_recv)) return fail(PK_ERR_INVALID, "pk_shard_adopt_remote_dev: bad argument");
  if (!f->hi_dev) return fail(PK_ERR_STATE, "pk_shard_adopt_remote_dev: call pk_shard_plan_dev first");
  if (!f->adopt_local_done)
    return fail(PK_ERR_STATE, "pk_shard_adopt_remote_dev: pk_shard_adopt_local_dev first (it makes the new generation current)");
  f->adopt_local_done = false;
  int rc;
  if ((rc = use_device(f))) return rc;
  if (n_received > f->rlohi_cap) {
    PK_HIP(hipStreamSynchronize(f->stream));
    if (f->rlohi_dev) (void)hipFree(f->rlohi_dev);
    f->rlohi_dev = nullptr;
    f->rlohi_cap = 0;
    if ((rc = dev_alloc(f, &f->rlohi_dev, (size_t)(2 * n_received + 2 * n_received / 4 + 16)))) return rc;
    f->rlohi_cap = n_received + n_received / 4;
  }
  Span t(f, PK_T_RESAMPLE);
  const int64_t base = (int64_t)rank * f->d.P;
  launch_adopt_dev(f->stream, f->d, f->hi_dev, base, static_cast<const unsigned char*>(dev_recv), n_received, f->rlohi_dev, 2,
                   f->loop_lo == INT64_MIN ? INT64_MIN : base + f->loop_lo, f->loop_hi == INT64_MAX ? INT64_MAX : base + f->loop_hi);
  f->loop_lo = INT64_MIN;
  f->loop_hi = INT64_MAX;
  return PK_OK;
}

int pk_shard_local_span_dev(pk_filter* f, int64_t* dev_out2) {
  if (!f || !dev_out2) return fail(PK_ERR_INVALID, "pk_shard_local_span_dev: NULL argument");
  if (!f->hi_dev) return fail(PK_ERR_STATE, "pk_shard_local_span_dev: no plan yet");
  int rc;
  if ((rc = use_device(f))) return rc;
  PK_HIP(hipMemcpyAsync(dev_out2, f->hi_dev, sizeof(int64_t), hipMemcpyDeviceToDevice, f->stream));
  PK_HIP(hipMemcpyAsync(dev_out2 + 1, f->hi_dev + f->d.P, sizeof(int64_t), hipMemcpyDeviceToDevice, f->stream));
  return PK_OK;
}

static int ensure_logical(pk_filter* f) {
  DeviceState& d = f->d;
  if (d.logical[0]) return PK_OK;
  int rc;
  int64_t *a = nullptr, *b = nullptr;
  if ((rc = dev_alloc(f, &a, (size_t)d.P))) return rc;
// ... 123 lines not shown
  if (!f->bal.H || global_particles != f->bal.cap) return fail(PK_ERR_STATE, "pk_shard_download_balanced_offspring: no balanced plan of %lld particles yet", (long long)global_particles);
  int rc;
  if ((rc = use_device(f))) return rc;
  PK_HIP(hipMemcpyAsync(H, f->bal.H, ((size_t)global_particles + 1) * sizeof(int64_t), hipMemcpyDeviceToHost, f->stream));
  PK_HIP(hipStreamSynchronize(f->stream));
  return PK_OK;
}

static int balanced_row_check(const int64_t* table, int world, int64_t P, const char* who) {
  const int row = 2 * world + 4;
  int64_t e_sum = 0, d_sum = 0;
  for (int r = 0; r < world; ++r) {
    const int64_t n = table[(size_t)r * row + 2 * world], m = table[(size_t)r * row + 2 * world + 1];
    if (n < 0 || m != (n < P ? n : P) || table[(size_t)r * row + 2 * world + 2] != e_sum || table[(size_t)r * row + 2 * world + 3] != d_sum)
      return fail(PK_ERR_INVALID, "%s: the plan table is not one pk_shard_plan_balanced_dev wrote (rank %d)", who, r);
    e_sum += n - m;
    d_sum += P - m;
    for (int d = 0; d < world; ++d) {
      const int64_t a0 = table[(size_t)r * row + 2 * d], a1 = table[(size_t)r * row + 2 * d + 1];
      if (a0 < 0 || a1 < a0 || a1 > P) return fail(PK_ERR_INVALID, "%s: range [%lld, %lld) from rank %d to rank %d", who, (long long)a0, (long long)a1, r, d);
    }
  }
  if (e_sum != d_sum) return fail(PK_ERR_INVALID, "%s: excess %lld and free slots %lld differ", who, (long long)e_sum, (long long)d_sum);
  return PK_OK;
}

int pk_shard_pack_balanced_dev(pk_filter* f, const int64_t* table, int32_t world, int32_t rank, void* dev_buf) {
  if (!f || !table || world < 1 || world > 64 || rank < 0 || rank >= world) return fail(PK_ERR_INVALID, "pk_shard_pack_balanced_dev: bad argument");
  if (!f->bal.rel || !f->d.logical[0]) return fail(PK_ERR_STATE, "pk_shard_pack_balanced_dev: call pk_shard_plan_balanced_dev first");
  int rc;
  const int64_t P = f->d.P;
  if ((rc = balanced_row_check(table, world, P, "pk_shard_pack_balanced_dev"))) return rc;
  if ((rc = use_device(f))) return rc;
  const int row = 2 * world + 4;
  const size_t stride = record_stride(f);
  const int64_t ebase_s = table[(size_t)rank * row + 2 * world + 2];
  int64_t rec = 0;
  Span t(f, PK_T_RESAMPLE);
  for (int d = 0; d < world; ++d) {
    if (d == rank) continue;
    const int64_t a0 = table[(size_t)rank * row + 2 * d], a1 = table[(size_t)rank * row + 2 * d + 1];
    if (a1 <= a0) continue;
    if (!dev_buf) return fail(PK_ERR_INVALID, "pk_shard_pack_balanced_dev: NULL buffer");
    const int64_t m_d = table[(size_t)d * row + 2 * world + 1], dbase_d = table[(size_t)d * row + 2 * world + 3];
    launch_bal_pack(f->stream, f->d, f->bal, a0, a1 - a0, ebase_s, dbase_d, P - m_d, m_d,
                    static_cast<unsigned char*>(dev_buf) + (size_t)rec * stride, stride, f->grow_on ? &f->grow : nullptr);
    rec += a1 - a0;
  }
  PK_LAUNCH_CHECK("pk_shard_pack_balanced_dev");
  return PK_OK;
}

int pk_shard_pack_balanced_loop_dev(pk_filter* f, int64_t keep, int64_t a0, int64_t a1, void* dev_buf) {
  if (!f || keep < 0 || keep > f->d.P || a0 < 0 || a1 < a0 || a1 > f->d.P || (a1 > a0 && !dev_buf))
    return fail(PK_ERR_INVALID, "pk_shard_pack_balanced_loop_dev: bad argument");
  if (!f->bal.rel || !f->d.logical[0]) return fail(PK_ERR_STATE, "pk_shard_pack_balanced_loop_dev: call pk_shard_plan_balanced_dev first");
  int rc;
  if ((rc = use_device(f))) return rc;
  Span t(f, PK_T_RESAMPLE);
  launch_bal_pack(f->stream, f->d, f->bal, a0, a1 - a0, 0, 0, f->d.P - keep, keep, static_cast<unsigned char*>(dev_buf), record_stride(f),
                  f->grow_on ? &f->grow : nullptr, keep);
  PK_LAUNCH_CHECK("pk_shard_pack_balanced_loop_dev");
  return PK_OK;
}

int pk_shard_adopt_balanced_dev(pk_filter* f, const int64_t* table, int32_t world, int32_t rank, const void* dev_recv,
                                int64_t n_received, int32_t mode) {
  if (f) f->pose_part_ok = false;
  if (!f || !table || world < 1 || world > 64 || rank < 0 || rank >= world || n_received < 0 || mode < 0 || mode > 2 ||
      (n_received > 0 && !dev_recv))
    return fail(PK_ERR_INVALID, "pk_shard_adopt_balanced_dev: bad argument");
  if (!f->bal.rel || !f->d.logical[0]) return fail(PK_ERR_STATE, "pk_shard_adopt_balanced_dev: call pk_shard_plan_balanced_dev first");
  if (f->grow_on && mode != 0) return fail(PK_ERR_STATE, "pk_shard_adopt_balanced_dev: the new-landmark bookkeeping (pk_grow_enable) is adopted whole (mode 0)");
  int rc;
  const int64_t P = f->d.P;
  if ((rc = balanced_row_check(table, world, P, "pk_shard_adopt_balanced_dev"))) return rc;
  const int row = 2 * world + 4;
  int64_t m = table[(size_t)rank * row + 2 * world + 1];
  const bool loop = f->bal_loop_keep >= 0 && world == 1;
  if (loop) m = f->bal_loop_keep < m ? f->bal_loop_keep : m;
  if (mode == 2) {
    if (!f->adopt_local_done) return fail(PK_ERR_STATE, "pk_shard_adopt_balanced_dev: mode 1 first (it makes the new generation current)");
    f->adopt_local_done = false;
  }
  if (mode != 1) {
    int64_t expect = 0;
    for (int s = 0; s < world; ++s)
      if (s != rank) expect += table[(size_t)s * row + 2 * rank + 1] - table[(size_t)s * row + 2 * rank];
    if (!loop && expect != n_received) return fail(PK_ERR_INVALID, "pk_shard_adopt_balanced_dev: %lld records received, the plan sends %lld", (long long)n_received, (long long)expect);
    if (m < P && n_received == 0) return fail(PK_ERR_INVALID, "pk_shard_adopt_balanced_dev: %lld free slots and no records", (long long)(P - m));
    f->bal_loop_keep = -1;
  }
  if ((rc = use_device(f))) return rc;
  if (mode != 2 && f->d.alt) {
    f->src_identity = false;
    if ((rc = materialise(f))) return rc;
  }
  if (3 * n_received > 2 * f->rlohi_cap) {
    PK_HIP(hipStreamSynchronize(f->stream));
    if (f->rlohi_dev) (void)hipFree(f->rlohi_dev);
    f->rlohi_dev = nullptr;
    f->rlohi_cap = 0;
    if ((rc = dev_alloc(f, &f->rlohi_dev, (size_t)(3 * n_received + 3 * n_received / 4 + 16)))) return rc;
    f->rlohi_cap = (3 * n_received + 3 * n_received / 4) / 2;
  }
  Span t(f, PK_T_RESAMPLE);
  const size_t stride = record_stride(f);
// ... 80 lines not shown

int pk_enable_timing(pk_filter* f, int32_t on) {
  if (!f) return fail(PK_ERR_INVALID, "pk_enable_timing: NULL handle");
  int rc;
  if ((rc = use_device(f))) return rc;
  if ((rc = drain_timings(f))) return rc;
  f->timing_mask = on < 0 ? 0xffffffffu : (uint32_t)on;
  return PK_OK;
}
int pk_reset_timings(pk_filter* f) {
  if (!f) return fail(PK_ERR_INVALID, "pk_reset_timings: NULL handle");
  int rc;
  if ((rc = use_device(f))) return rc;
  if ((rc = drain_timings(f))) return rc;
  for (int i = 0; i < PK_T_COUNT; ++i) {
    f->ms[i] = 0;
    f->launches[i] = 0;
    f->timing_seen[i] = 0;
  }
  return PK_OK;
}
int pk_timings(pk_filter* f, double ms[PK_T_COUNT], int64_t launches[PK_T_COUNT]) {
  if (!f || !ms || !launches) return fail(PK_ERR_INVALID, "pk_timings: NULL argument");
  int rc;
  if ((rc = use_device(f))) return rc;
  if ((rc = drain_timings(f))) return rc;
  for (int i = 0; i < PK_T_COUNT; ++i) {
    ms[i] = f->ms[i];
    launches[i] = f->launches[i];
  }
  return PK_OK;
}
int pk_observe_route(const pk_filter* f) { return f ? f->route : PK_ROUTE_NONE; }
int pk_observe_flagged(pk_filter* f, int64_t* flagged, int64_t* cand_overflow) {
  if (!f) return fail(PK_ERR_INVALID, "pk_observe_flagged: NULL handle");
  int rc;
  if ((rc = use_device(f))) return rc;
  unsigned w[2] = {0u, 0u};
  if (f->scan_dev && f->route != PK_ROUTE_NONE && f->route != PK_ROUTE_KNOWN_IDS) {
    PK_HIP(hipMemcpyAsync(w, ctl_n_flagged(f), sizeof(w), hipMemcpyDeviceToHost, f->stream));
    PK_HIP(hipStreamSynchronize(f->stream));
  }
  if (flagged) *flagged = w[0];
  if (cand_overflow) *cand_overflow = w[1];
  return PK_OK;
}
int pk_observe_retry_rows(pk_filter* f, int64_t* wanted, int64_t* capacity) {
  if (!f) return fail(PK_ERR_INVALID, "pk_observe_retry_rows: NULL handle");
  int rc;
  if ((rc = use_device(f))) return rc;
  PK_HIP(hipStreamSynchronize(f->stream));
  if (wanted) *wanted = f->retry_seen ? (int64_t)*f->retry_seen : 0;
  if (capacity) *capacity = retry_rows(f);
  return PK_OK;
}
int pk_observe_flags(pk_filter* f, uint8_t* flags) {
  if (!f || !flags) return fail(PK_ERR_INVALID, "pk_observe_flags: NULL argument");
  int rc;
  if ((rc = use_device(f))) return rc;
  const bool onepass = f->route == PK_ROUTE_ML_REGS || f->route == PK_ROUTE_ML_FUSED || f->route == PK_ROUTE_ML_PUB_BIG;
  if (onepass && f->fh.pflag) {
    PK_HIP(hipMemcpyAsync(flags, f->fh.pflag, (size_t)f->d.P, hipMemcpyDeviceToHost, f->stream));
    PK_HIP(hipStreamSynchronize(f->stream));
  } else {
    memset(flags, 0, (size_t)f->d.P);
  }
// ... 50 lines not shown
```

### parakeet_slam_amd/csrc/pk_k_step_pub.hip

```cpp
#include <type_traits>

#include "pk_device.hpp"
#include "pk_pub_math.hpp"
#include "pk_pub_layout.hpp"

namespace pk {

#ifndef PK_PUB_ABLATE
#define PK_PUB_ABLATE 0
#endif

typedef double Double2 __attribute__((ext_vector_type(2)));
typedef int Int2 __attribute__((ext_vector_type(2)));

__device__ __forceinline__ double pose_scalar(const double* a, int64_t p) {
  return ((const __attribute__((address_space(4))) double*)a)[p];
}
__device__ __forceinline__ int32_t regs_source_pub(const int32_t* src, int64_t p) {
  return ((const __attribute__((address_space(4))) int32_t*)src)[p];
}

struct PubArgs {
  SlotSource ss;
  unsigned char* map_dst;
  size_t count_off;
  int32_t* src;
  const double *x, *y, *h;
  double* logw;
  const double* exact;
  const unsigned short* order;
  const unsigned char* immutable;
  const uint4* cand;
  const uint4* erec;
  const unsigned* glist;
  const unsigned* skip;
  const float4* gate4;
  const uint4* far;
  unsigned char* pflag_out;
  unsigned* n_flagged;
  int64_t P, p_begin;
  int L, Lp, B;
  int ecap;
  int reset;
  unsigned long long* gmax_key;
  Noise<double> qt;
  const unsigned* stats;
  int tbytes;
  const uint4* prim;
  unsigned* unm;
  int unm_words;
};

constexpr int kPubUnmWords = 176;
template <int THREADS>
__device__ __forceinline__ void pub_note_unmatched(int tid, const unsigned char* anyc, const unsigned short* order, int B, unsigned Bp, unsigned* ubits) {
  for (unsigned w = (unsigned)tid; w < Bp / 4u; w += THREADS) {
    const unsigned v = reinterpret_cast<const unsigned*>(anyc)[w];
#pragma unroll
    for (int b = 0; b < 4; ++b)
      if ((int)(4 * w + b) < B && ((v >> (8 * b)) & 0xFFu) == 0u) {
        const unsigned o = order[4 * w + b];
        atomicOr(&ubits[o >> 5], 1u << (o & 31u));
      }
  }
}
template <int THREADS>
__device__ __forceinline__ void pub_store_unmatched(int tid, unsigned* ubits, unsigned* row, int words) {
  for (int w = tid; w < words; w += THREADS) {
    row[w] = ubits[w];
    ubits[w] = 0u;
  }
}

struct PubPrim {
  const uint4* tab;
  size_t Lpp;
  int lc;
  __device__ __forceinline__ double2 z01(int j) const { return reinterpret_cast<const double2*>(tab + Lpp)[lc + j]; }
  __device__ __forceinline__ double2 z23(int j) const { return reinterpret_cast<const double2*>(tab + 2 * Lpp)[lc + j]; }
  __device__ __forceinline__ double2 dir(int j) const { return reinterpret_cast<const double2*>(tab + 3 * Lpp)[lc + j]; }
  __device__ __forceinline__ unsigned t0(int j) const { return reinterpret_cast<const unsigned*>(tab + 4 * Lpp)[lc + j]; }
};

// ... 753 lines not shown
#endif

typedef const __attribute__((address_space(4))) PubArgs* PubArgsPtr;
__device__ __forceinline__ PubArgsPtr pub_args_now(PubArgsPtr rp) {
  asm volatile("" : "+s"(rp));
  return rp;
}
__device__ __forceinline__ SlotSource pub_slot_source(PubArgsPtr R) {
  return SlotSource{R->ss.map, R->ss.slot_bytes, R->ss.alt, R->ss.alt_stride, R->ss.alt_off};
}
__device__ __forceinline__ Noise<double> pub_noise(PubArgsPtr R) {
  return Noise<double>{R->qt.q00, R->qt.rr, R->qt.rg, R->qt.rb, R->qt.gg, R->qt.gb, R->qt.bb, R->qt.diag};
}

#ifdef PK_DIAG_NO_XCD_RUNS
__device__ __forceinline__ int64_t pub_walk_first(int64_t p_begin, int64_t) { return p_begin + blockIdx.x; }
__device__ __forceinline__ int64_t pub_walk_stride() { return (int64_t)gridDim.x; }
__device__ __forceinline__ int64_t pub_walk_limit(int64_t, int64_t p_end) { return p_end; }
#else
__device__ __forceinline__ int64_t pub_walk_first(int64_t p_begin, int64_t p_end) {
  const unsigned g = gridDim.x, b = blockIdx.x;
  if ((g & 7u) != 0u) return p_begin + b;
  const int64_t chunk = (p_end - p_begin + 7) / 8;
  return p_begin + (int64_t)(b & 7u) * chunk + (int64_t)(b >> 3);
}
__device__ __forceinline__ int64_t pub_walk_stride() { return (gridDim.x & 7u) != 0u ? (int64_t)gridDim.x : (int64_t)(gridDim.x >> 3); }
__device__ __forceinline__ int64_t pub_walk_limit(int64_t p_begin, int64_t p_end) {
  const unsigned g = gridDim.x, b = blockIdx.x;
  if ((g & 7u) != 0u) return p_end;
  const int64_t chunk = (p_end - p_begin + 7) / 8, e = p_begin + (int64_t)((b & 7u) + 1u) * chunk;
  return e < p_end ? e : p_end;
}
#endif
template <int NP, int THREADS>
__global__ void __launch_bounds__(THREADS, THREADS == 256 ? 3 : 1) k_step_pub(PubArgs a_unused) {
  constexpr int kPubThreads = THREADS, kPubWaves = THREADS / kWave;
  extern __shared__ __align__(16) unsigned char smem[];
  __shared__ double red[2][kPubWaves];
  __shared__ int wg_flag[2];
  constexpr bool kPerm = NP == 2 && THREADS == 512;
  __shared__ unsigned short s_perm[kPerm ? 2 * kPubOctets : 1];
  __shared__ unsigned s_rb[kCandSlots];
  constexpr int kUnmWords = THREADS == kPubSmallThreads ? 32 : 96;
  __shared__ unsigned s_ubits[kUnmWords];
#define PK_PUB_L0(q_, t_) (!kPerm ? 2 * kPubThreads * (q_) + 2 * (t_) : (int)(((lw >> (16 + 8 * (q_))) & 0xFFu) << 4) + 2 * ((t_)&7))
  PubArgsPtr rp = (PubArgsPtr)__builtin_amdgcn_kernarg_segment_ptr();
  const int tid0 = threadIdx.x;
  int B, Lp, L, ecap;
  {
    PubArgsPtr R = pub_args_now(rp);
    if (*R->skip != 0u) return;
    B = R->B;
    Lp = R->Lp;
    L = R->L;
    ecap = R->ecap;
  }
  const unsigned Bp = ((unsigned)B + 15u) & ~15u;
  const unsigned o_pub = Bp * 48u, o_binfo = o_pub + ((unsigned)ecap + 2u) * 8u, o_order = o_binfo + Bp * 4u, o_any = o_order + Bp * 2u;
  const unsigned o_imm = o_any + 2u * (Bp + 16u);
  const unsigned o_bnd = o_imm + (unsigned)kPubImmBytes;
  const unsigned dump = (unsigned)ecap, anydump = Bp;
  unsigned G;
  {
    const int tid = tid0;
    PubArgsPtr R = pub_args_now(rp);
    {
// ... 22 lines not shown
    }
    for (unsigned i = (unsigned)tid; i < 2u * (Bp + 16u) / 4u; i += kPubThreads) reinterpret_cast<unsigned*>(smem + o_any)[i] = 0u;
    const unsigned char* gi = R->immutable;
    for (int i = tid; i < Lp; i += kPubThreads) smem[o_imm + (unsigned)i] = i < L ? gi[i] : (unsigned char)0;
    if constexpr (kPerm) {
      if (tid < 2 * kPubOctets) s_perm[tid] = reinterpret_cast<const unsigned short*>(gb + B + 1)[tid];
    }
    if (tid < kCandSlots) s_rb[tid] = gb[B + 1 + kPubTailWords + tid];
    for (int i = tid; i < kUnmWords; i += kPubThreads) s_ubits[i] = 0u;
    if (tid == 0) {
      wg_flag[0] = 0;
      wg_flag[1] = 0;
    }
  }
  __syncthreads();

  int64_t prev = -1;
  int cur = 0;
  int32_t nsrc;
  {
    PubArgsPtr R = pub_args_now(rp);
    const int64_t p0 = pub_walk_first(R->p_begin, R->P), pl = pub_walk_limit(R->p_begin, R->P);
    nsrc = regs_source_pub(R->src, p0 < pl ? p0 : pl - 1);
  }
#ifdef PK_STAMPS
  unsigned long long pst[12] = {0, 0, 0, 0, 0, 0, 0, 0, 0, 0, 0, 0};
#endif
#define PK_PUB_ROW(q_, field, F)                                                                  \
  {                                                                                               \
    const Double2 v_ = *reinterpret_cast<const Double2*>(sf_ + (size_t)F * Lp + lbq_);            \
    S[2 * (q_)].field = v_.x;                                                                     \
    S[2 * (q_) + 1].field = v_.y;                                                                 \
  }
#define PK_PUB_LOAD_MEANS(q_, sslot_, lb_)                                                        \
  {                                                                                               \
    const double* sf_ = reinterpret_cast<const double*>(sslot_);                                  \
    const int lbq_ = (lb_);                                                                       \
    PK_PUB_ROW(q_, mx, F_MX)                                                                      \
    PK_PUB_ROW(q_, my, F_MY)                                                                      \
    PK_PUB_ROW(q_, mr, F_MR)                                                                      \
    PK_PUB_ROW(q_, mg, F_MG)                                                                      \
    PK_PUB_ROW(q_, mb, F_MB)                                                                      \
    asm volatile("" ::: "memory");                                                                \
  }
#define PK_PUB_LOAD_COVS(q_, sslot_, coff_, lb_)                                                  \
  {                                                                                               \
    const double* sf_ = reinterpret_cast<const double*>(sslot_);                                  \
    const int* sc_ = reinterpret_cast<const int*>((sslot_) + (coff_));                            \
    const int lbq_ = (lb_);                                                                       \
    PK_PUB_ROW(q_, pxx, F_PXX)                                                                    \
    PK_PUB_ROW(q_, pxy, F_PXY)                                                                    \
    PK_PUB_ROW(q_, pyy, F_PYY)                                                                    \
    PK_PUB_ROW(q_, crr, F_CRR)                                                                    \
    PK_PUB_ROW(q_, crg, F_CRG)                                                                    \
    PK_PUB_ROW(q_, crb, F_CRB)                                                                    \
    PK_PUB_ROW(q_, cgg, F_CGG)                                                                    \
    PK_PUB_ROW(q_, cgb, F_CGB)                                                                    \
    PK_PUB_ROW(q_, cbb, F_CBB)                                                                    \
    const Int2 c_ = *reinterpret_cast<const Int2*>(sc_ + lbq_);                                   \
    S[2 * (q_)].count = c_.x;                                                                     \
    S[2 * (q_) + 1].count = c_.y;                                                                 \
    asm volatile("" ::: "memory");                                                                \
  }
#define PK_PUB_LOAD_PAIR(q_, sslot_, coff_, lb_)                                                  \
  {                                                                                               \
    const double* sf_ = reinterpret_cast<const double*>(sslot_);                                  \
    const int* sc_ = reinterpret_cast<const int*>((sslot_) + (coff_));                            \
    const int lbq_ = (lb_);                                                                       \
    PK_PUB_ROW(q_, mx, F_MX)                                                                      \
    PK_PUB_ROW(q_, my, F_MY)                                                                      \
    PK_PUB_ROW(q_, mr, F_MR)                                                                      \
    PK_PUB_ROW(q_, mg, F_MG)                                                                      \
    PK_PUB_ROW(q_, mb, F_MB)                                                                      \
    asm volatile("" ::: "memory");                                                                \
    PK_PUB_ROW(q_, pxx, F_PXX)                                                                    \
    PK_PUB_ROW(q_, pxy, F_PXY)                                                                    \
    PK_PUB_ROW(q_, pyy, F_PYY)                                                                    \
    PK_PUB_ROW(q_, crr, F_CRR)                                                                    \
    PK_PUB_ROW(q_, crg, F_CRG)                                                                    \
    PK_PUB_ROW(q_, crb, F_CRB)                                                                    \
    PK_PUB_ROW(q_, cgg, F_CGG)                                                                    \
    PK_PUB_ROW(q_, cgb, F_CGB)                                                                    \
    PK_PUB_ROW(q_, cbb, F_CBB)                                                                    \
    const Int2 c_ = *reinterpret_cast<const Int2*>(sc_ + lbq_);                                   \
    S[2 * (q_)].count = c_.x;                                                                     \
    S[2 * (q_) + 1].count = c_.y;                                                                 \
    asm volatile("" ::: "memory");                                                                \
  }
  Landmark<double> S[2 * NP];
  constexpr int kPipe = 1;
  unsigned lane_word = (unsigned)tid0;
  if constexpr (kPerm) {
    const unsigned octs = (unsigned)(s_perm[tid0 >> 3] & 0xFFu) | ((unsigned)(s_perm[kPubOctets + (tid0 >> 3)] & 0xFFu) << 8);
    lane_word = (unsigned)tid0 | (octs << 16);
  }
  {
    const unsigned lw = lane_word;
    PubArgsPtr R = pub_args_now(rp);
    const unsigned char* ns = pub_slot_source(R).at(nsrc);
    const int coff = R->count_off;
#pragma unroll
    for (int q = 0; q < kPipe; ++q) PK_PUB_LOAD_PAIR(q, ns, coff, min(PK_PUB_L0(q, tid0), Lp - 2))
  }
  for (int64_t p = pub_walk_first(pub_args_now(rp)->p_begin, pub_args_now(rp)->P);; p += pub_walk_stride(), cur ^= 1) {
    unsigned lw = lane_word;
    asm volatile("" : "+v"(lw));
    int tid;
    if constexpr (!kPerm) {
      tid = (int)lw;
    } else {
      tid = (int)(lw & 0xFFFFu);
    }
    double* ex = reinterpret_cast<double*>(smem);
    double* pub = reinterpret_cast<double*>(smem + o_pub);
    const unsigned* glist = reinterpret_cast<const unsigned*>(smem + o_binfo);
    const unsigned short* order = reinterpret_cast<const unsigned short*>(smem + o_order);
    unsigned char* anyc = smem + o_any + (unsigned)cur * (Bp + 16u);
    PubSlots Q[2 * NP];
    double pse[2 * NP];
    bool done;
    PK_STAMP(s0)
#ifdef PK_STAMPS
// ... 12 lines not shown
#pragma unroll
        for (int q = 0; q < NP; ++q) lbase[q] = min(PK_PUB_L0(q, tid), Lp - 2);
        uint4 cref[2 * NP], ccw[2 * NP], cew[2 * NP];
        auto request_cand = [&](int q) {
          PubArgsPtr R2 = pub_args_now(rp);
#ifdef PK_DIAG_TAIL_LISTS
          const int lc = lbase[q];
#else
          const int lc = min(PK_PUB_L0(q, tid), Lp);
#endif
          const uint4* cr = R2->cand + 2 * (size_t)lc;
          const uint4* er = R2->erec + lc;
          cref[2 * q] = cr[0];
          ccw[2 * q] = cr[1];
          cref[2 * q + 1] = cr[2];
          ccw[2 * q + 1] = cr[3];
          cew[2 * q] = er[0];
          cew[2 * q + 1] = er[1];
        };
        request_cand(0);
        asm volatile("" ::: "memory");
        {
          PubArgsPtr R4 = pub_args_now(rp);
          const int64_t pn = p + pub_walk_stride(), pl = pub_walk_limit(R4->p_begin, R4->P);
          nsrc = regs_source_pub(R4->src, pn < pl ? pn : pl - 1);
          asm volatile("" : "+s"(nsrc));
        }
        PK_STAMP(s1)
        PK_PSTAMP(0, s0, s1)
        auto do_pair = [&](auto qc) {
          constexpr int q = decltype(qc)::value;

    const int l0 = PK_PUB_L0(q, tid);
    const PubGateIn gi[2] = {{cref[2 * q], {ccw[2 * q], ccw[2 * q]}, {cew[2 * q], cew[2 * q]}, S[2 * q].mx, S[2 * q].my,
                              S[2 * q].mr, S[2 * q].mg, S[2 * q].mb, l0 < L},
                             {cref[2 * q + 1], {ccw[2 * q + 1], ccw[2 * q + 1]}, {cew[2 * q + 1], cew[2 * q + 1]},
                              S[2 * q + 1].mx, S[2 * q + 1].my, S[2 * q + 1].mr, S[2 * q + 1].mg, S[2 * q + 1].mb,
                              l0 + 1 < L}};
    PubSlots qq[2] = {kPubNoSlots,
                      kPubNoSlots};
    double pp[2] = {0.0, 0.0};
    if constexpr (THREADS == kPubSmallThreads) {
      
#pragma unroll
      for (int j_ = 0; j_ < 2; ++j_) {
        const PubGateIn g1[1] = {gi[j_]};
        PubSlots q1[1] = {qq[j_]};
        double p1[1] = {0.0};
        const Landmark<double>* const l1[1] = {&S[2 * q + j_]};
        if (PK_PUB_ABLATE < 4) pub_gatesN<1>(q1, p1, g1, ex, pub, dump, &wg_flag[cur], sx, sy, sh);
        if (PK_PUB_ABLATE < 3) {
          struct Chk1 {
            const float2* bnd_;
            int l_, L_, Lp_;
            PubArgsPtr rp_;
            double sh;
            __device__ __forceinline__ float2 bnd(int) const { return bnd_[min(l_, Lp_ - 1)]; }
            __device__ __forceinline__ bool has(int) const { return l_ < L_; }
            __device__ __forceinline__ const uint4* far_row() const {
              const uint4* fr = pub_args_now(rp_)->far;
              return fr ? fr + 2 * (size_t)min(l_, Lp_) : nullptr;
            }
          };
          const Chk1 chk{reinterpret_cast<const float2*>(smem + o_bnd), l0 + j_, L, Lp, rp, sh};
          pub_keysN<1, kPubSlots, false, true, 1, Chk1>(q1, l1, p1, ex, pub, dump, anyc, anydump, &wg_flag[cur], sx, sy, nullptr, nullptr, chk);
        }
// ... 10 lines not shown
          unsigned lw, tid_;
          int L_, Lp_;
          PubArgsPtr rp_;
          double sh;
          __device__ __forceinline__ int l0() const { const unsigned lw = this->lw; const int tid = (int)tid_; (void)tid; return PK_PUB_L0(q, tid); }
          __device__ __forceinline__ float2 bnd(int j) const { return bnd_[min(l0() + j, Lp_ - 1)]; }
          __device__ __forceinline__ bool has(int j) const { return l0() + j < L_; }
          __device__ __forceinline__ const uint4* far_row() const {
            const uint4* fr = pub_args_now(rp_)->far;
            return fr ? fr + 2 * (size_t)min(l0(), Lp_) : nullptr;
          }
        };
        const Chk2 chk{reinterpret_cast<const float2*>(smem + o_bnd), lw, (unsigned)tid, L, Lp, rp, sh};
        pub_keysN<2, kPubSlots, false, true, 1, Chk2>(qq, l2, pp, ex, pub, dump, anyc, anydump, &wg_flag[cur], sx, sy, nullptr, nullptr, chk);
        {
          PubArgsPtr R9 = pub_args_now(rp);
          const int lc9 = min(l0, Lp);
          if (pub_refill_slots<2>(qq, R9->cand + 2 * (size_t)lc9, R9->erec + lc9, &wg_flag[cur]))
            pub_keysN<2>(qq, l2, pp, ex, pub, dump, anyc, anydump, &wg_flag[cur], sx, sy);
        }
      }
      PK_STAMP(sk1_)
      PK_PSTAMP(2, sk0_, sk1_)
    }
    Q[2 * q] = qq[0];
    Q[2 * q + 1] = qq[1];
    pse[2 * q] = pp[0];
    pse[2 * q + 1] = pp[1];
  
        };
        if (!done) {
          do_pair(std::integral_constant<int, 0>{});
          if constexpr (NP > 1) {
            PK_PUB_LOAD_MEANS(1, sslot, lbase[1])
            request_cand(NP - 1);
            {
              asm volatile("" ::: "memory");
              PubArgsPtr R7 = pub_args_now(rp);
              PK_PUB_LOAD_COVS(1, sslot, R7->count_off, lbase[1])
            }
            do_pair(std::integral_constant<int, 1>{});
          }
        }
        PK_STAMP(s2)
        PK_PSTAMP(1, s1, s2)
#ifdef PK_STAMPS
        s3 = s2;
#endif
      }
    }
    lds_barrier();
    PK_STAMP(s4)
    PK_PSTAMP(3, s3, s4)
    if (prev >= 0 && tid == 0) {
      PubArgsPtr R = pub_args_now(rp);
      double tot = red[cur ^ 1][0];
#pragma unroll
      for (int i = 1; i < kPubWaves; ++i) tot += red[cur ^ 1][i];
      double* logw = R->logw;
      const double w = (R->reset ? 0.0 : logw[prev]) + tot;
      logw[prev] = w;
      unsigned long long* gk = R->gmax_key;
      if (gk) atomicMax(gk + (prev & (kGmaxKeys - 1)), double_to_key(w));
      R->src[prev] = (int32_t)prev;
    }
    if (done) break;
    prev = -1;
    double acc;
    {
      int nun = 0;
      for (unsigned w = (unsigned)tid; w < Bp / 4u; w += kPubThreads) {
        const unsigned v = reinterpret_cast<const unsigned*>(anyc)[w];
// ... 47 lines not shown
      {
        double nprod = 1.0;
        auto do_apply = [&](auto qc) {
          constexpr int q = decltype(qc)::value;
          const int l0 = PK_PUB_L0(q, tid);
#pragma unroll
          for (int j = 0; j < 2; ++j) {
            const int i = 2 * q + j;
            const bool imm = immutable[min(l0 + j, Lp - 1)] != 0;
            if (PK_PUB_ABLATE < 1)
              acc += THREADS == kPubSmallThreads ? pub_apply_loop(Q[i], ex, order, qt, S[i], imm, sx, sy, pse[i], nullptr, 0, 0, 0xFFFFu, PK_PROD_PTR(nprod))
                                                 : pub_apply(Q[i], ex, order, qt, S[i], imm, sx, sy, pse[i], PK_PROD_PTR(nprod));
          }
          pub_fold_norms(acc, nprod, q == NP - 1);
        };
        auto do_store = [&](auto qc) {
          constexpr int q = decltype(qc)::value;
          const int l0 = PK_PUB_L0(q, tid);
          PK_STAMP(su0_)
          if (l0 < Lp) {
#define PK_PUB_STORE(field, F)                                                             \
    {                                                                                        \
      const Double2 v = {S[2 * q].field, S[2 * q + 1].field};                                \
      __builtin_nontemporal_store(v, reinterpret_cast<Double2*>(df + (size_t)F * Lp + l0)); \
    }
            PK_PUB_STORE(mx, F_MX)
            PK_PUB_STORE(my, F_MY)
            PK_PUB_STORE(mr, F_MR)
            PK_PUB_STORE(mg, F_MG)
            PK_PUB_STORE(mb, F_MB)
            PK_PUB_STORE(pxx, F_PXX)
            PK_PUB_STORE(pxy, F_PXY)
            PK_PUB_STORE(pyy, F_PYY)
            PK_PUB_STORE(crr, F_CRR)
            PK_PUB_STORE(crg, F_CRG)
            PK_PUB_STORE(crb, F_CRB)
            PK_PUB_STORE(cgg, F_CGG)
            PK_PUB_STORE(cgb, F_CGB)
            PK_PUB_STORE(cbb, F_CBB)
#undef PK_PUB_STORE
            const Int2 c = {S[2 * q].count, S[2 * q + 1].count};
            __builtin_nontemporal_store(c, reinterpret_cast<Int2*>(dc + l0));
          }
          if (q < kPipe) {
            PubArgsPtr R6 = pub_args_now(rp);
            const unsigned char* ns = pub_slot_source(R6).at(nsrc);
            PK_PUB_LOAD_PAIR(q, ns, R6->count_off, min(PK_PUB_L0(q, tid), Lp - 2))
          }
          PK_STAMP(su1_)
          PK_PSTAMP(10, su0_, su1_)
        };
        using Q0 = std::integral_constant<int, 0>;
        using Q1 = std::integral_constant<int, 1>;
        do_apply(Q0{});
        do_store(Q0{});
        if constexpr (NP == 2) {
          do_apply(Q1{});
          do_store(Q1{});
        }
      }
    }
    PK_STAMP(s7)
    PK_PSTAMP(6, s6, s7)
    {
      const double ws = wave_sum(acc);
      if ((tid & (kWave - 1)) == 0) red[cur][tid / kWave] = ws;
      prev = p;
    }
    PK_STAMP(s8)
    PK_PSTAMP(7, s7, s8)
    PK_PSTAMP(8, s0, s8)
#ifdef PK_STAMPS
    pst[9] += 1ull;
#endif
  }
#ifdef PK_STAMPS
  if ((tid0 & 63) == 0)
    for (int k = 0; k < 12; ++k) {
      atomicAdd(&pk_pstamp_acc[k], pst[k]);
      if (THREADS == 512) atomicAdd(&pk_pstamp_wave[tid0 >> 6][k], pst[k]);
    }
#endif
}

constexpr int kPubBigSlots = 2 * kCandSlots;
constexpr int kPubBigGateSlots = 8;
__device__ __forceinline__ PubSlots pub_keep_positive(const PubSlotsT<kPubBigGateSlots>& g, int* flag) {
  PubSlots o = kPubNoSlots;
#pragma unroll
  for (int k = kPubBigGateSlots - 1; k >= 0; --k) {
    const bool pos = ((g.st >> (4 * k)) & 1u) != 0u;
    o.s[3] = pos ? o.s[2] : o.s[3];
    o.s[2] = pos ? o.s[1] : o.s[2];
    o.s[1] = pos ? o.s[0] : o.s[1];
    o.s[0] = pos ? g.s[k] : o.s[0];
    o.st = pos ? ((o.st << 4) | 1u) : o.st;
  }
  if (flag && __popc(g.st & 0x11111111u) > kPubSlots) *flag = 1;
  o.st &= 0xFFFFu;
  return o;
}
__device__ __forceinline__ uint4 pub_positive_beyond_four(const PubSlotsT<kPubBigGateSlots>& g) {
  unsigned x[4] = {0xFFFFFFFFu, 0xFFFFFFFFu, 0xFFFFFFFFu, 0xFFFFFFFFu};
  int c = 0;
#pragma unroll
  for (int k = 0; k < kPubBigGateSlots; ++k) {
    const bool pos = ((g.st >> (4 * k)) & 1u) != 0u;
// ... 540 lines not shown
  a.gate4 = gate4_dev;
  a.far = cand.far;
  a.prim = prim_dev;
  a.stats = stats_dev;
  a.tbytes = 0;
  a.unm = ex.unm;
  a.unm_words = ex.unm_words;
  a.pflag_out = fh.pflag;
  a.n_flagged = fh.n_flagged;
  a.P = p1;
  a.p_begin = p0;
  a.L = d.lay.L;
  a.Lp = d.lay.Lp;
  a.B = B;
  a.ecap = ecap;
  a.reset = ex.reset ? 1 : 0;
  a.gmax_key = ex.gmax_key;
  a.qt = make_noise(qt.q00, qt.rr, qt.rg, qt.rb, qt.gg, qt.gb, qt.bb);
  const int n_cu = device_cu_count();
  int64_t grid_n = n_cu - (reserve_cus > 0 && reserve_cus < n_cu ? reserve_cus : 0);
  if (grid_n > p1 - p0) grid_n = p1 - p0;
  const size_t lds = step_pub_big_lds_bytes(B, ecap);
  const int nch = (d.lay.Lp + 2 * kPubThreads - 1) / (2 * kPubThreads);
  if (nch <= 3)
    hipLaunchKernelGGL(k_step_pub_big<3>, dim3((unsigned)grid_n), dim3(kPubThreads), lds, s, a);
  else if (nch <= 5)
    hipLaunchKernelGGL(k_step_pub_big<5>, dim3((unsigned)grid_n), dim3(kPubThreads), lds, s, a);
  else
    hipLaunchKernelGGL(k_step_pub_big<6>, dim3((unsigned)grid_n), dim3(kPubThreads), lds, s, a);
}

void launch_step_pub(hipStream_t s, DeviceState& d, int B, const double* exact_dev, const unsigned short* order_dev,
                     const FastHandoff& fh, const NoiseD& qt, const ObserveExtras& ex, const CandTable& cand, const uint4* erec_dev,
                     const unsigned* glist_dev, const unsigned* skip_dev, int ecap, int64_t p0, int64_t p1, int reserve_cus) {
  if (p1 < 0) p1 = d.P;
  if (d.P == 0 || p1 <= p0) return;
  static bool attr_set[kMaxDevices] = {false};
  if (first_time_on_this_device(attr_set)) {
    for (const void* fn : {reinterpret_cast<const void*>(k_step_pub<1, kPubSmallThreads>), reinterpret_cast<const void*>(k_step_pub<1, kPubThreads>),
                           reinterpret_cast<const void*>(k_step_pub<2, kPubThreads>)})
      if (hipFuncSetAttribute(fn, hipFuncAttributeMaxDynamicSharedMemorySize, (int)kMaxDynLds) != hipSuccess) (void)hipGetLastError();
  }
  PubArgs a;
  a.ss = slot_source(d);
  a.map_dst = d.map[d.mcur ^ 1];
  a.count_off = d.lay.count_off;
  a.src = d.src[d.cur];
  a.x = d.x[d.cur];
  a.y = d.y[d.cur];
  a.h = d.h[d.cur];
  a.logw = d.logw[d.cur];
  a.exact = exact_dev;
  a.order = order_dev;
  a.immutable = d.immutable;
  a.cand = cand.rec;
  a.erec = erec_dev;
  a.glist = glist_dev;
  a.skip = skip_dev;
  a.gate4 = nullptr;
  a.prim = nullptr;
  a.stats = nullptr;
  a.tbytes = 0;
  a.unm = ex.unm;
  a.unm_words = ex.unm_words;
  a.far = cand.far;
  a.pflag_out = fh.pflag;
  a.n_flagged = fh.n_flagged;
  a.P = p1;
  a.p_begin = p0;
  a.L = d.lay.L;
  a.Lp = d.lay.Lp;
  a.B = B;
  a.ecap = ecap;
  a.reset = ex.reset ? 1 : 0;
  a.gmax_key = ex.gmax_key;
  a.qt = make_noise(qt.q00, qt.rr, qt.rg, qt.rb, qt.gg, qt.gb, qt.bb);
  const int n_cu = device_cu_count();
  const bool small = d.lay.Lp <= 2 * kPubSmallThreads;
  const size_t lds = step_pub_lds_bytes(B, ecap, small);
  int per_cu = 1;
  if (small) per_cu = (int)std::min<size_t>(3, std::max<size_t>(1, (160 * 1024 - 1024) / (lds + 256)));
  int64_t grid_n = (int64_t)(n_cu - (reserve_cus > 0 && reserve_cus < n_cu ? reserve_cus : 0)) * per_cu;
  if (grid_n > p1 - p0) grid_n = p1 - p0;
  if (small)
    hipLaunchKernelGGL((k_step_pub<1, kPubSmallThreads>), dim3((unsigned)grid_n), dim3(kPubSmallThreads), lds, s, a);
  else if (d.lay.Lp <= 2 * kPubThreads)
    hipLaunchKernelGGL((k_step_pub<1, kPubThreads>), dim3((unsigned)grid_n), dim3(kPubThreads), lds, s, a);
  else
    hipLaunchKernelGGL((k_step_pub<2, kPubThreads>), dim3((unsigned)grid_n), dim3(kPubThreads), lds, s, a);
}

#include "pk_k_step_duo.inl"

}
```

### parakeet_slam_amd/csrc/pk_kernels.hpp

```cpp
#pragma once
#include <hip/hip_runtime.h>

#include <cstdint>

#include "pk_layout.hpp"

namespace pk {

struct NoiseD {
  double q00, rr, rg, rb, gg, gb, bb;
};

struct DeviceState {
  int64_t P;
  MapLayout lay;
  double* x[2];
  double* y[2];
  double* h[2];
  double* logw[2];
  int32_t* src[2];
  int cur;
  unsigned char* map[2];
  int mcur;
  unsigned char* immutable;
// ... 142 lines not shown
                       bool finalize, const FastHandoff& fh, const CandTable& cand);
void launch_candidates(hipStream_t s, DeviceState& d, int B, const double* exact_dev, int64_t ref_particle, uint4* rec_dev,
                       unsigned* over_dev, unsigned* bcnt_dev = nullptr, uint4* brec_dev = nullptr, unsigned* stray_dev = nullptr,
                       int slots = kCandSlots, const double* pose_sums4_dev = nullptr, unsigned char* npass_dev = nullptr,
                       uint4* far_dev = nullptr, const double* pose_part_dev = nullptr);
constexpr int kRegsMaxL = 2048;
size_t regs_lds_bytes(int ncell, int B, int n9);
size_t regs_cand_lds_bytes(int Lp, int B);
void launch_step_regs(hipStream_t s, DeviceState& d, int B, const BlobGrid& grid, int n9, const unsigned char* tables_dev,
                      const double* exact_dev, const unsigned short* order_dev, const FastHandoff& fh, const NoiseD& qt,
                      const ObserveExtras& ex, int warm, const CandTable& cand = CandTable(), int64_t p0 = 0, int64_t p1 = -1,
                      int reserve_cus = 0);
int step_pub_entry_capacity(int B);
int step_pub_entry_capacity_small(int B);
size_t step_pub_lds_bytes(int B, int ecap, bool small = false);
struct DuoLimits {
  int tbytes = 0;
  int ecap = 0;
  int gcap = 0;
  int nl = 1;
  int park_limit = -1;
};
void launch_cand_entries(hipStream_t s, const DeviceState& d, int B, const uint4* cand_dev, uint4* erec_dev, unsigned* bcnt_dev,
                         uint4* brec_dev, unsigned* binfo_dev, unsigned* glist_dev, const unsigned* over_dev, unsigned* skip_pub_dev,
                         unsigned* skip_cand_dev, int ecap, int slots = kCandSlots, const double* exact_dev = nullptr,
                         float4* gate4_dev = nullptr, const unsigned char* npass_dev = nullptr, bool pruned = false,
                         unsigned* stats_dev = nullptr, unsigned* skip_duo_dev = nullptr, unsigned* skip_big_dev = nullptr,
                         const DuoLimits& duo = DuoLimits(), uint4* prim_dev = nullptr, unsigned char* flag_all_dev = nullptr,
                         unsigned* n_flagged_dev = nullptr);
inline size_t prim_table_uint4(int Lp) { const size_t Lpp = (size_t)Lp + kCandSpare; return 4 * Lpp + (Lpp + 3) / 4; }
void launch_step_pub(hipStream_t s, DeviceState& d, int B, const double* exact_dev, const unsigned short* order_dev,
                     const FastHandoff& fh, const NoiseD& qt, const ObserveExtras& ex, const CandTable& cand, const uint4* erec_dev,
                     const unsigned* glist_dev, const unsigned* skip_dev, int ecap, int64_t p0 = 0, int64_t p1 = -1,
                     int reserve_cus = 0);
void launch_flag_range_if(hipStream_t s, const unsigned* over_dev, unsigned char* pflag_dev, unsigned* n_flagged_dev, int64_t p0, int64_t p1);
constexpr int kPubBigMaxL = 6144;
int step_pub_big_entry_capacity(int B);
size_t step_pub_big_lds_bytes(int B, int ecap);
void launch_step_pub_big(hipStream_t s, DeviceState& d, int B, const double* exact_dev, const unsigned short* order_dev,
                         const FastHandoff& fh, const NoiseD& qt, const ObserveExtras& ex, const CandTable& cand, const uint4* erec_dev,
                         const unsigned* glist_dev, const unsigned* skip_dev, int ecap, const float4* gate4_dev = nullptr, int64_t p0 = 0,
                         int64_t p1 = -1, int reserve_cus = 0, const uint4* prim_dev = nullptr, const unsigned* stats_dev = nullptr);
void step_pub_duo_limits(int B, int Lp, int nl, DuoLimits* out);
size_t step_pub_duo_lds_bytes(int B, const DuoLimits& lim);
void launch_step_pub_duo(hipStream_t s, DeviceState& d, int B, const double* exact_dev, const unsigned short* order_dev,
                         const FastHandoff& fh, const NoiseD& qt, const ObserveExtras& ex, const CandTable& cand, const uint4* erec_dev,
                         const unsigned* glist_dev, const unsigned* skip_duo_dev, const unsigned* stats_dev, const DuoLimits& lim,
                         const float4* gate4_dev, const uint4* prim_dev, int64_t p0 = 0, int64_t p1 = -1, int reserve_cus = 0);
extern int g_observe_nv;
inline size_t observe_general_lds_bytes(int Lp, int B) { return sizeof(int32_t) * ((size_t)Lp + 2 * (size_t)B); }
inline size_t assoc_brute_lds_bytes(int B) { return (size_t)B * 12; }
void launch_block_max(hipStream_t s, DeviceState& d, double* partial_dev, double* gmax_dev);
void launch_keys_max(hipStream_t s, const unsigned long long* keys_dev, double* gmax_dev);
void launch_scan_local(hipStream_t s, DeviceState& d, const double* gmax_dev, int domain,
                       double* clocal_dev, double* totals_dev, const unsigned long long* gmax_key_dev = nullptr);
void launch_scan_blocks(hipStream_t s, const double* totals_dev, int64_t nb, double* offsets_dev,
                        double* sum_dev);
constexpr int64_t kAncestorsScanMaxBlocks = 256;
void launch_ancestors(hipStream_t s, const double* clocal_dev, const double* totals_dev,
                      const double* offsets_dev, const double* sum_dev, int64_t nb, int64_t P_global,
                      int64_t P_scan, double u, int64_t slot0, int64_t n, int32_t* anc_dev,
                      DeviceState* gather = nullptr);
void launch_summary_partials(hipStream_t s, DeviceState& d, double* partial_dev, double* out4_dev);
void launch_materialise(hipStream_t s, DeviceState& d);
void launch_broadcast_slot(hipStream_t s, DeviceState& d, const unsigned char* slot_dev);
void launch_probe(hipStream_t s, const double* in_dev, double* out_dev);
size_t dense_lds_bytes(int Lp, int B);
// ... 56 lines not shown
```

### parakeet_slam_amd/csrc/pk_math.hpp

```cpp
#pragma once
#include <hip/hip_runtime.h>

namespace pk {

template <typename T>
struct Consts;
template <>
struct Consts<double> {
  static constexpr double two_pi = 6.283185307179586476925286766559;
  static constexpr double half_pi = 1.5707963267948966192313216916398;
  static constexpr double log_two_pi = 1.8378770664093454835606594728112;
  static constexpr double log_no_match = -2.3025850929940456840179914546844;
};

template <typename T>
struct Landmark {
  T mx, my, mr, mg, mb;
  T pxx, pxy, pyy;
  T crr, crg, crb, cgg, cgb, cbb;
  int count;
};

constexpr int kPotentialBit = 0x40000000;
__device__ __forceinline__ void count_update(int& count) {
// ... 167 lines not shown
  const double z = s * s;
  double p = 1.0 / 21.0;
  p = fma_k(p, z, 1.0 / 19.0);
  p = fma_k(p, z, 1.0 / 17.0);
  p = fma_k(p, z, 1.0 / 15.0);
  p = fma_k(p, z, 1.0 / 13.0);
  p = fma_k(p, z, 1.0 / 11.0);
  p = fma_k(p, z, 1.0 / 9.0);
  p = fma_k(p, z, 1.0 / 7.0);
  p = fma_k(p, z, 1.0 / 5.0);
  p = fma_k(p, z, 1.0 / 3.0);
  const double lm = 2.0 * s + 2.0 * s * (z * p);
  const double ed = (double)e;
  return ed * 0.69314718055994528623 + (ed * 2.3190468138462995584e-17 + lm);
}

__device__ __forceinline__ double pr_from_parts(double det2, double det3, double num2, double num3) {
  const double maha2 = num2 / det2, maha3 = num3 / det3;
  const double bp = 500.0 * exp(-0.5 * (2.0 * Consts<double>::log_two_pi + log_few_ulp(det2) + maha2));
  const double cp = 500.0 * exp(-0.5 * (3.0 * Consts<double>::log_two_pi + log_few_ulp(det3) + maha3));
  return bp * cp / 250000.0;
}

template <typename T>
struct EkfAux {
  T zhat0, h0, h1;
  T q00;
  Sym3<T> qc;
  T k0, k1;
  T kc[9];
};

template <typename T>
__device__ __forceinline__ T ekf_update(Landmark<T>& f, T sx, T sy, const BlobT<T>& z,
                                        const Noise<T>& qt, bool immutable,
                                        EkfAux<T>* aux = nullptr, const T* zhat0_known = nullptr, T* fro_prod = nullptr) {
  T dx = f.mx - sx, dy = f.my - sy;
  T zhat0 = zhat0_known ? *zhat0_known : pk_atan2(dy, dx);
  T q = dx * dx + dy * dy;
  T h0, h1;
  if (q == T(0)) {
    h0 = T(0);
    h1 = T(0);
  } else {
    T iq = T(1) / q;
    h0 = dy * iq;
    h1 = dx * iq;
  }
  T a0 = f.pxx * h0 + f.pxy * h1;
  T a1 = f.pxy * h0 + f.pyy * h1;
  T q00 = h0 * a0 + h1 * a1 + qt.q00;
  Sym3<T> qc{f.crr + qt.rr, f.crg + qt.rg, f.crb + qt.rb, f.cgg + qt.gg, f.cgb + qt.gb, f.cbb + qt.bb};
  T detc;
  Sym3<T> qci = sym3_inverse(qc, detc);
  T iq00 = T(1) / q00;

  T d0 = z.bearing - zhat0;
  T d1 = z.r - f.mr, d2 = z.g - f.mg, d3 = z.b - f.mb;

  T fro2 = q00 * q00 + qc.a * qc.a + qc.d * qc.d + qc.f * qc.f +
           T(2) * (qc.b * qc.b + qc.c * qc.c + qc.e * qc.e);
  T v0 = qci.a * d1 + qci.b * d2 + qci.c * d3;
  T v1 = qci.b * d1 + qci.d * d2 + qci.e * d3;
  T v2 = qci.c * d1 + qci.e * d2 + qci.f * d3;
  T maha = d0 * d0 * iq00 + (d1 * v0 + d2 * v1 + d3 * v2);
  T logw;
  if (fro_prod) {
    logw = T(-0.5) * Consts<T>::log_two_pi - T(0.5) * maha;
    if (f.count & kPotentialBit)
      logw = (T)Consts<double>::log_no_match;
    else
      *fro_prod *= fro2;
  } else {
    logw = T(-0.5) * (Consts<T>::log_two_pi + T(0.5) * log_few_ulp(fro2)) - T(0.5) * maha;
    if (f.count & kPotentialBit) logw = (T)Consts<double>::log_no_match;
  }
  T k0 = a0 * iq00, k1 = a1 * iq00;

  if (aux) {
    aux->zhat0 = zhat0;
    aux->h0 = h0;
    aux->h1 = h1;
    aux->q00 = q00;
    aux->qc = qc;
    aux->k0 = k0;
    aux->k1 = k1;
    const T C[3][3] = {{f.crr, f.crg, f.crb}, {f.crg, f.cgg, f.cgb}, {f.crb, f.cgb, f.cbb}};
    const T I[3][3] = {{qci.a, qci.b, qci.c}, {qci.b, qci.d, qci.e}, {qci.c, qci.e, qci.f}};
    for (int i = 0; i < 3; ++i)
      for (int j = 0; j < 3; ++j) aux->kc[i * 3 + j] = C[i][0] * I[0][j] + C[i][1] * I[1][j] + C[i][2] * I[2][j];
  }

  if (!immutable) {
    f.mx += k0 * d0;
    f.my += k1 * d0;
    T nr = f.mr + (f.crr * v0 + f.crg * v1 + f.crb * v2);
    T ng = f.mg + (f.crg * v0 + f.cgg * v1 + f.cgb * v2);
    T nb = f.mb + (f.crb * v0 + f.cgb * v1 + f.cbb * v2);
    T nxx = f.pxx - k0 * a0;
    T nxy = f.pxy - T(0.5) * (k0 * a1 + k1 * a0);
    T nyy = f.pyy - k1 * a1;
    T nrr, nrg, nrb, ngg, ngb, nbb;
    T m00 = qci.a * f.crr + qci.b * f.crg + qci.c * f.crb;
    T m01 = qci.a * f.crg + qci.b * f.cgg + qci.c * f.cgb;
    T m02 = qci.a * f.crb + qci.b * f.cgb + qci.c * f.cbb;
    T m11 = qci.b * f.crg + qci.d * f.cgg + qci.e * f.cgb;
    T m12 = qci.b * f.crb + qci.d * f.cgb + qci.e * f.cbb;
    T m22 = qci.c * f.crb + qci.e * f.cgb + qci.f * f.cbb;
    if (qt.diag) {
      nrr = qt.rr * m00;
      nrg = qt.rr * m01;
      nrb = qt.rr * m02;
      ngg = qt.gg * m11;
      ngb = qt.gg * m12;
      nbb = qt.bb * m22;
    } else {
      T m10 = qci.b * f.crr + qci.d * f.crg + qci.e * f.crb;
      T m20 = qci.c * f.crr + qci.e * f.crg + qci.f * f.crb;
      T m21 = qci.c * f.crg + qci.e * f.cgg + qci.f * f.cgb;
      nrr = f.crr - (f.crr * m00 + f.crg * m10 + f.crb * m20);
      nrg = f.crg - (f.crr * m01 + f.crg * m11 + f.crb * m21);
      nrb = f.crb - (f.crr * m02 + f.crg * m12 + f.crb * m22);
      ngg = f.cgg - (f.crg * m01 + f.cgg * m11 + f.cgb * m21);
      ngb = f.cgb - (f.crg * m02 + f.cgg * m12 + f.cgb * m22);
      nbb = f.cbb - (f.crb * m02 + f.cgb * m12 + f.cbb * m22);
    }
    f.mr = nr;
    f.mg = ng;
    f.mb = nb;
    f.pxx = nxx;
    f.pxy = nxy;
    f.pyy = nyy;
    f.crr = nrr;
    f.crg = nrg;
    f.crb = nrb;
    f.cgg = ngg;
    f.cgb = ngb;
    f.cbb = nbb;
    count_update(f.count);
  }
  return logw;
}

template <typename T>
__device__ __forceinline__ void motion_model(T& x, T& y, T& h, T v, T w, T dt, T n0, T n1, T n2) {
  T dheading = w * dt;
  T ds = v * dt + n0;
  T h1 = h + dheading / T(2) + n1;
  T h2 = h1 + dheading / T(2) + n2;
  T s, c;
  sincos(h1, &s, &c);
  x += ds * c;
  y += ds * s;
  h = wrap_heading(h2);
}

}
```

Before: 25.80 billion.

## Share colour covariances through a per-landmark level table indexed by update count

Because the colour-block covariance update depends only on its prior value and the noise, particles that share a landmark's initial colour covariance and update count share its colour covariance. A device table of per-level colour covariances is built and extended each observe, and the fused publish kernel reads colour covariances from the table and skips storing them per particle. Rows are materialised back into particle storage whenever another path needs them. This cuts per-particle memory traffic in the hot observe kernel, at the cost of extra bookkeeping kernels, a host sync when the table grows, and many exit points that must keep state consistent.

```diff
diff --git a/include/parakeet_slam.h b/include/parakeet_slam.h
--- a/include/parakeet_slam.h
+++ b/include/parakeet_slam.h
@@ -165,6 +165,7 @@
   PK_ROUTE_ML_PUB_BIG = 9,
 };
 int pk_observe_route(const pk_filter* f);
+int pk_colour_levels(pk_filter* f, int64_t out[3]);
 int pk_download_sources(pk_filter* f, int32_t* src);
 int pk_observe_flagged(pk_filter* f, int64_t* flagged, int64_t* cand_overflow);
 int pk_observe_retry_rows(pk_filter* f, int64_t* wanted, int64_t* capacity);
diff --git a/parakeet_slam_amd/_lib.py b/parakeet_slam_amd/_lib.py
--- a/parakeet_slam_amd/_lib.py
+++ b/parakeet_slam_amd/_lib.py
@@ -99,6 +99,7 @@
     "pk_timings": (C.c_int, [_h, _dp, _lp]),
     "pk_observe_bytes": (C.c_int, [_h, C.c_int32, _lp, _lp]),
     "pk_observe_route": (C.c_int, [_h]),
+    "pk_colour_levels": (C.c_int, [_h, _lp]),
     "pk_download_sources": (C.c_int, [_h, _ip]),
     "pk_observe_flagged": (C.c_int, [_h, _lp, _lp]),
     "pk_observe_retry_rows": (C.c_int, [_h, _lp, _lp]),
@@ -429,6 +430,11 @@
     def observe_route(self):
         return self.ROUTES[int(self._lib.pk_observe_route(self._h))]
 
+    def colour_levels(self):
+        out = np.zeros(3, np.int64)
+        check(self._lib.pk_colour_levels(self._h, out.ctypes.data_as(_lp)))
+        return tuple(int(v) for v in out)
+
     def observe_flagged(self):
         a, b = C.c_int64(), C.c_int64()
         check(self._lib.pk_observe_flagged(self._h, C.byref(a), C.byref(b)))
diff --git a/parakeet_slam_amd/build.py b/parakeet_slam_amd/build.py
--- a/parakeet_slam_amd/build.py
+++ b/parakeet_slam_amd/build.py
@@ -13,7 +13,7 @@
 LIB = os.path.join(HERE, "libparakeet_slam.so")
 OBJDIR = os.path.join(HERE, "csrc", "_obj")
 
-HIP_SOURCES = ["pk_k_motion.hip", "pk_k_assoc.hip", "pk_k_observe.hip", "pk_k_observe_ml.hip", "pk_k_step_pub.hip", "pk_k_cand_entries.hip", "pk_k_dense.hip", "pk_k_resample.hip", "pk_k_grow.hip", "pk_api.hip"]
+HIP_SOURCES = ["pk_k_motion.hip", "pk_k_assoc.hip", "pk_k_observe.hip", "pk_k_observe_ml.hip", "pk_k_step_pub.hip", "pk_k_cand_entries.hip", "pk_k_dense.hip", "pk_k_resample.hip", "pk_k_grow.hip", "pk_k_colour.hip", "pk_api.hip"]
 CXX_SOURCES = ["pk_rng.cpp"]
 HEADERS = [
     "pk_math.hpp", "pk_layout.hpp", "pk_kernels.hpp", "pk_philox.hpp", "pk_device.hpp", "pk_pub_math.hpp", "pk_pub_layout.hpp", "pk_k_step_duo.inl",
diff --git a/parakeet_slam_amd/csrc/pk_api.hip b/parakeet_slam_amd/csrc/pk_api.hip
--- a/parakeet_slam_amd/csrc/pk_api.hip
+++ b/parakeet_slam_amd/csrc/pk_api.hip
@@ -139,6 +139,15 @@
   int pub_small = -1;
   int duo_park_limit = -1;
   int duo_on = 0;
+  int colour_levels = 1;
+  int colour_cap_init = 512;
+  bool colour_on = false;
+  bool colour_observed = false;
+  bool shard_set = false;
+  double* ctab = nullptr;
+  int ctab_cap = 0;
+  unsigned* cctl = nullptr;
+  unsigned* cctl_seen = nullptr;
   int pub_entry_limit = 0;
   uint4* erec_dev = nullptr;
   uint4* erec_dev2 = nullptr;
@@ -358,6 +367,60 @@
   return PK_OK;
 }
 
+int colour_levels_exit(pk_filter* f) {
+  if (!f->colour_on) return PK_OK;
+  f->colour_on = false;
+  launch_colour_rows(f->stream, f->d, f->ctab, f->cctl, f->qt, nullptr, nullptr, 0, f->d.P);
+  PK_LAUNCH_CHECK("colour levels: leaving the mode");
+  return PK_OK;
+}
+int colour_levels_enter(pk_filter* f) {
+  f->colour_on = false;
+  if (!f->colour_levels || f->dense || f->grow_on || f->shard_set || f->d.lay.L <= 0 || f->d.lay.L > kRegsMaxL) return PK_OK;
+  int rc;
+  const size_t plane = 6 * (size_t)f->d.lay.Lp;
+  if (f->ctab && f->ctab_cap != f->colour_cap_init) {
+    PK_HIP(hipStreamSynchronize(f->stream));
+    (void)hipFree(f->ctab);
+    f->ctab = nullptr;
+  }
+  if (!f->ctab) {
+    f->ctab_cap = 0;
+    if ((rc = dev_alloc(f, &f->ctab, plane * (size_t)f->colour_cap_init))) return rc;
+    f->ctab_cap = f->colour_cap_init;
+  }
+  if (!f->cctl && (rc = dev_alloc(f, &f->cctl, 2))) return rc;
+  if (!f->cctl_seen && hipHostMalloc((void**)&f->cctl_seen, 64, hipHostMallocDefault) != hipSuccess) {
+    f->cctl_seen = nullptr;
+    return fail(PK_ERR_NOMEM, "colour levels: pinned word");
+  }
+  *f->cctl_seen = 0u;
+  launch_colour_level0(f->stream, f->d, f->slot_tmp, f->ctab, f->cctl);
+  PK_LAUNCH_CHECK("colour levels: level 0");
+  f->colour_on = true;
+  f->colour_observed = false;
+  return PK_OK;
+}
+int colour_levels_prepare(pk_filter* f) {
+  if (!f->colour_on) return PK_OK;
+  int rc;
+  if (*f->cctl_seen + 1u > (unsigned)f->ctab_cap / 2u) {
+    PK_HIP(hipStreamSynchronize(f->stream));
+    const size_t plane = 6 * (size_t)f->d.lay.Lp;
+    double* neu = nullptr;
+    if ((rc = dev_alloc(f, &neu, plane * 2 * (size_t)f->ctab_cap))) return rc;
+    PK_HIP(hipMemcpyAsync(neu, f->ctab, plane * (size_t)f->ctab_cap * sizeof(double), hipMemcpyDeviceToDevice, f->stream));
+    PK_HIP(hipStreamSynchronize(f->stream));
+    (void)hipFree(f->ctab);
+    f->ctab = neu;
+    f->ctab_cap *= 2;
+  }
+  launch_colour_extend(f->stream, f->d, f->ctab, f->cctl, f->ctab_cap, f->qt, 0);
+  PK_LAUNCH_CHECK("colour levels: extension");
+  f->colour_observed = true;
+  return PK_OK;
+}
+
 void pack_landmark(const MapLayout& lay, unsigned char* slot, int l, const double* mean, const double* cov) {
   double* fl = reinterpret_cast<double*>(slot);
   const int Lp = lay.Lp;
@@ -679,6 +742,7 @@
       fh = f->fh;
       fh.n_flagged = ctl_n_flagged(f);
     }
+    if ((rc = colour_levels_exit(f))) return rc;
     Span t(f, PK_T_ASSOC);
     CandTable cand;
     if (fh.lmpass && f->cand_lists && f->d.lay.L < 65535) {
@@ -704,6 +768,7 @@
     return fail(PK_ERR_UNSUPPORTED,
                 "maximum-likelihood association of %d blobs: neither the colour-grid tables nor the brute-force kernel's "
                 "%zu bytes of per-blob state fit the workgroup's %zu bytes of LDS", B, assoc_brute_lds_bytes(B), (size_t)kMaxDynLds);
+  if ((rc = colour_levels_exit(f))) return rc;
   Span t(f, PK_T_ASSOC);
   launch_assoc_brute(f->stream, f->d, blobs_dev, dir_dev, B, f->ids_dev);
   return PK_OK;
@@ -750,6 +815,8 @@
 int relayout(pk_filter* f, bool dense, bool keep) {
   if (f->dense == dense) return PK_OK;
   int rc;
+  if (keep && (rc = colour_levels_exit(f))) return rc;
+  f->colour_on = false;
   DeviceState& d = f->d;
   const MapLayout old = d.lay;
   const MapLayout neu = MapLayout::make(old.L, sizeof(double), dense ? kDenseFields : (int)F_COUNT_FIELDS);
@@ -936,6 +1003,9 @@
     if (f->stage_done[i]) (void)hipEventDestroy(f->stage_done[i]);
   }
   if (f->retry_seen) (void)hipHostFree(f->retry_seen);
+  if (f->ctab) (void)hipFree(f->ctab);
+  if (f->cctl) (void)hipFree(f->cctl);
+  if (f->cctl_seen) (void)hipHostFree(f->cctl_seen);
   if (f->own_stream) (void)hipStreamDestroy(f->own_stream);
   delete f;
   return PK_OK;
@@ -977,6 +1047,12 @@
       if (fabs(Qt[i * 4 + j] - Qt[j * 4 + i]) > 1e-9 * (scale > 0 ? scale : 1.0)) coupled = true;
   int rc;
   if ((rc = use_device(f))) return rc;
+  if (f->colour_on && f->colour_observed && (rc = colour_levels_exit(f))) return rc;
+  if (f->colour_on) {
+    static const unsigned level0_only[2] = {1u, 0u};
+    PK_HIP(hipMemcpyAsync(f->cctl, level0_only, sizeof(level0_only), hipMemcpyHostToDevice, f->stream));
+    PK_HIP(hipStreamSynchronize(f->stream));
+  }
   if (coupled && !f->dense && (rc = relayout(f, true, f->map_loaded))) return rc;
   for (int i = 0; i < 16; ++i) f->qt16[i] = Qt[i];
   f->qt_dense = coupled;
@@ -1009,6 +1085,7 @@
   PK_HIP(hipMemcpyAsync(f->slot_tmp, slot.data(), lay.slot_bytes, hipMemcpyHostToDevice, f->stream));
   PK_HIP(hipMemcpyAsync(f->d.immutable, imm.data(), imm.size(), hipMemcpyHostToDevice, f->stream));
   launch_broadcast_slot(f->stream, f->d, f->slot_tmp);
+  if ((rc = colour_levels_enter(f))) return rc;
   PK_HIP(hipStreamSynchronize(f->stream));
   f->src_identity = true;
   f->map_loaded = true;
@@ -1095,6 +1172,10 @@
   int rc;
   if ((rc = use_device(f))) return rc;
   if ((rc = materialise(f))) return rc;
+  if (f->colour_on) {
+    launch_colour_rows(f->stream, f->d, f->ctab, f->cctl, f->qt, nullptr, nullptr, p0, p1);
+    PK_LAUNCH_CHECK("pk_download_landmarks (colour rows)");
+  }
   const MapLayout& lay = f->d.lay;
   const int L = lay.L;
   const int64_t chunk = std::max<int64_t>(1, (int64_t)(64u << 20) / (int64_t)lay.slot_bytes);
@@ -1124,6 +1205,7 @@
   if (!f->map_loaded) return fail(PK_ERR_STATE, "pk_upload_landmarks: no map uploaded");
   int rc;
   if ((rc = use_device(f))) return rc;
+  if ((rc = colour_levels_exit(f))) return rc;
   if ((rc = materialise(f))) return rc;
   const int L = f->d.lay.L;
   if (means)
@@ -1395,7 +1477,7 @@
   } else if (al.regs) {
     if (f->pub_ecap > 0 && cand.rec)
       launch_step_pub(f->stream, f->d, B, al.exact, al.order, fh, f->qt, e1, cand, f->erec_dev, f->glist_dev, ctl_skip_pub(f), f->pub_ecap,
-                      p0, p1, reserve_cus);
+                      p0, p1, reserve_cus, f->colour_on ? f->ctab : nullptr, f->colour_on ? f->cctl : nullptr);
     if ((cand.far || f->grow_on) && f->pub_ecap > 0) {
       if (!f->flag_folded) launch_flag_range_if(f->stream, ctl_skip_pub(f), fh.pflag, fh.n_flagged, p0, p1);
     } else
@@ -1404,7 +1486,7 @@
   } else {
     if (f->pub_ecap > 0 && cand.rec)
       launch_step_pub(f->stream, f->d, B, al.exact, al.order, fh, f->qt, e1, cand, f->erec_dev, f->glist_dev, ctl_skip_pub(f), f->pub_ecap,
-                      p0, p1, reserve_cus);
+                      p0, p1, reserve_cus, f->colour_on ? f->ctab : nullptr, f->colour_on ? f->cctl : nullptr);
     if (f->pub_ecap > 0 && cand.rec) {
       if (!f->flag_folded) launch_flag_range_if(f->stream, ctl_skip_pub(f), fh.pflag, fh.n_flagged, p0, p1);
     } else
@@ -1480,6 +1562,7 @@
   if (f->dense) return dense_observe(f, blobs, B, ids, ids_out, reset, true);
   ObserveExtras ex;
   ex.reset = reset;
+  if (ids && (rc = colour_levels_exit(f))) return rc;
   if (ids) {
     f->staged.valid = false;
     const size_t o_blobs = kCtlBytes;
@@ -1557,11 +1640,19 @@
              : al.regs ? PK_ROUTE_ML_REGS
              : !al.fast ? PK_ROUTE_ML_GENERAL
              : (f->d.lay.L > kFastMaxL || f->fast_observe >= 2) ? PK_ROUTE_ML_SWEEP : PK_ROUTE_ML_HANDOFF;
+  if (f->colour_on && !(al.fused || al.regs) && (rc = colour_levels_exit(f))) return rc;
+  if ((rc = colour_levels_prepare(f))) return rc;
   if (al.fused || al.regs || al.big) {
     CandTable cand;
     if ((rc = onepass_prepare(f, al, B, &cand, 0, true))) return rc;
+    if (f->colour_on && !(!al.big && f->pub_ecap > 0 && cand.rec && (al.fused || cand.far)) && (rc = colour_levels_exit(f))) return rc;
     if ((rc = onepass_launch(f, al, B, ex, cand, 0, f->d.P))) return rc;
+    if (f->colour_on) {
+      Span t(f, PK_T_ASSOC);
+      launch_colour_rows(f->stream, f->d, f->ctab, f->cctl, f->qt, f->fh.pflag, ctl_n_flagged(f), 0, f->d.P);
+    }
     if ((rc = onepass_finish(f, al, B, ex, cand))) return rc;
+    if (f->colour_on) (void)hipMemcpyAsync(f->cctl_seen, f->cctl + 1, sizeof(unsigned), hipMemcpyDeviceToHost, f->stream);
   } else {
     Span t(f, PK_T_OBSERVE);
     if (al.fast) {
@@ -1654,6 +1745,7 @@
   if (f->grow_on) return fail(PK_ERR_STATE, "pk_observe_staged_range: the new-landmark bookkeeping (pk_grow_enable) runs behind whole observes (pk_observe / pk_observe_staged)");
   int rc;
   if ((rc = use_device(f))) return rc;
+  if ((rc = colour_levels_exit(f))) return rc;
   pk_filter::Split& sp = f->split;
   if (first) {
     if (sp.active) return fail(PK_ERR_STATE, "pk_observe_staged_range: the previous split observe was not finished (last = 1)");
@@ -1710,6 +1802,7 @@
   if (B == 0) return PK_OK;
   int rc;
   if ((rc = use_device(f))) return rc;
+  if ((rc = colour_levels_exit(f))) return rc;
   for (int i = 0; i < 4 * B; ++i)
     if (!std::isfinite(blobs[i])) return fail(PK_ERR_INVALID, "pk_associate: blob %d is not finite", i / 4);
   if (f->dense) return dense_observe(f, blobs, B, nullptr, ids_out, false, false);
@@ -1722,6 +1815,18 @@
 
 int pk_set_option(pk_filter* f, const char* name, int64_t value) {
   if (!f || !name) return fail(PK_ERR_INVALID, "pk_set_option: NULL argument");
+  if (!strcmp(name, "colour_levels")) {
+    if (value != 0 && value != 1) return fail(PK_ERR_INVALID, "colour_levels: 1 (where eligible, from the next pk_upload_map) or 0 (never)");
+    f->colour_levels = (int)value;
+    int rc;
+    if (!value && f->colour_on && ((rc = use_device(f)) || (rc = colour_levels_exit(f)))) return rc;
+    return PK_OK;
+  }
+  if (!strcmp(name, "colour_level_capacity")) {
+    if (value < 2 || value > 65536) return fail(PK_ERR_INVALID, "colour_level_capacity: 2 .. 65536 levels");
+    f->colour_cap_init = (int)value;
+    return PK_OK;
+  }
   if (!strcmp(name, "assoc_kernel")) {
     if (value != 0 && value != 1) return fail(PK_ERR_INVALID, "assoc_kernel: 0 (colour grid) or 1 (brute force)");
     f->assoc_kernel = (int)value;
@@ -1936,6 +2041,7 @@
                               "(a covariance or Qt that couples position and colour)");
   int rc;
   if ((rc = use_device(f))) return rc;
+  if ((rc = colour_levels_exit(f))) return rc;
   GrowState& g = f->grow;
   g.L0 = preset_landmarks;
   g.S = L - preset_landmarks;
@@ -1947,6 +2053,9 @@
     if ((rc = dev_alloc(f, &g.hyp[i], P * g.R * 8))) return rc;
     if ((rc = dev_alloc(f, &g.cnt[i], P * 4))) return rc;
     if ((rc = dev_alloc(f, &g.slot_id[i], P * g.S))) return rc;
+    PK_HIP(hipMemsetAsync(g.hyp[i], 0, P * g.R * 8 * sizeof(double), f->stream));
+    PK_HIP(hipMemsetAsync(g.cnt[i], 0, P * 4 * sizeof(int32_t), f->stream));
+    PK_HIP(hipMemsetAsync(g.slot_id[i], 0, P * g.S * sizeof(int32_t), f->stream));
   }
   std::vector<int32_t> c0(P * 4, 0);
   for (size_t p = 0; p < P; ++p) c0[4 * p + 2] = preset_landmarks + 1;
@@ -2027,6 +2136,9 @@
 
 int pk_set_shard(pk_filter* f, int64_t global_offset) {
   if (!f || global_offset < 0) return fail(PK_ERR_INVALID, "pk_set_shard: bad argument");
+  int rc;
+  if (f->colour_on && ((rc = use_device(f)) || (rc = colour_levels_exit(f)))) return rc;
+  f->shard_set = true;
   f->d.global_offset = global_offset;
   return PK_OK;
 }
@@ -2076,6 +2188,7 @@
   if (n == 0) return PK_OK;
   int rc;
   if ((rc = use_device(f))) return rc;
+  if ((rc = colour_levels_exit(f))) return rc;
   if (!f->idx_dev && (rc = dev_alloc(f, &f->idx_dev, (size_t)f->d.P))) return rc;
   PK_HIP(hipMemcpyAsync(f->idx_dev, local_idx, (size_t)n * sizeof(int64_t), hipMemcpyHostToDevice, f->stream));
   {
@@ -2096,6 +2209,7 @@
   if (f->d.logical[0]) return fail(PK_ERR_STATE, "pk_adopt_particles: the balanced placement is active on this filter (its slots carry logical indices): resample through pk_shard_plan_balanced_dev / pk_shard_adopt_balanced_dev");
   int rc;
   if ((rc = use_device(f))) return rc;
+  if ((rc = colour_levels_exit(f))) return rc;
   if (f->d.alt) {
     f->src_identity = false;
     if ((rc = materialise(f))) return rc;
@@ -2232,6 +2346,7 @@
   if (!f->hi_dev) return fail(PK_ERR_STATE, "pk_shard_pack_dev: call pk_shard_plan_dev first");
   int rc;
   if ((rc = use_device(f))) return rc;
+  if ((rc = colour_levels_exit(f))) return rc;
   const int64_t P = f->d.P;
   const size_t stride = kPoseRecordBytes + f->d.lay.slot_bytes;
   int64_t rec = 0;
@@ -2255,6 +2370,7 @@
   if (j1 > j0 && !dev_buf) return fail(PK_ERR_INVALID, "pk_shard_pack_slots_dev: NULL buffer");
   int rc;
   if ((rc = use_device(f))) return rc;
+  if ((rc = colour_levels_exit(f))) return rc;
   Span t(f, PK_T_RESAMPLE);
   launch_pack_range(f->stream, f->d, f->hi_dev, j0, j1 - j0, slot_lo, slot_hi, static_cast<unsigned char*>(dev_buf));
   PK_LAUNCH_CHECK("pk_shard_pack_slots_dev");
@@ -2269,6 +2385,7 @@
   if (f->d.logical[0]) return fail(PK_ERR_STATE, "pk_shard_adopt_dev: the balanced placement is active on this filter (its slots carry logical indices): resample through pk_shard_plan_balanced_dev / pk_shard_adopt_balanced_dev");
   int rc;
   if ((rc = use_device(f))) return rc;
+  if ((rc = colour_levels_exit(f))) return rc;
   if (f->d.alt) {
     f->src_identity = false;
     if ((rc = materialise(f))) return rc;
@@ -2297,6 +2414,7 @@
   if (f->d.logical[0]) return fail(PK_ERR_STATE, "pk_shard_adopt_local_dev: the balanced placement is active on this filter (its slots carry logical indices): resample through pk_shard_plan_balanced_dev / pk_shard_adopt_balanced_dev");
   int rc;
   if ((rc = use_device(f))) return rc;
+  if ((rc = colour_levels_exit(f))) return rc;
   if (f->d.alt) {
     f->src_identity = false;
     if ((rc = materialise(f))) return rc;
@@ -2321,6 +2439,7 @@
   f->adopt_local_done = false;
   int rc;
   if ((rc = use_device(f))) return rc;
+  if ((rc = colour_levels_exit(f))) return rc;
   if (n_received > f->rlohi_cap) {
     PK_HIP(hipStreamSynchronize(f->stream));
     if (f->rlohi_dev) (void)hipFree(f->rlohi_dev);
@@ -2510,6 +2629,7 @@
   const int64_t P = f->d.P;
   if ((rc = balanced_row_check(table, world, P, "pk_shard_pack_balanced_dev"))) return rc;
   if ((rc = use_device(f))) return rc;
+  if ((rc = colour_levels_exit(f))) return rc;
   const int row = 2 * world + 4;
   const size_t stride = record_stride(f);
   const int64_t ebase_s = table[(size_t)rank * row + 2 * world + 2];
@@ -2535,6 +2655,7 @@
   if (!f->bal.rel || !f->d.logical[0]) return fail(PK_ERR_STATE, "pk_shard_pack_balanced_loop_dev: call pk_shard_plan_balanced_dev first");
   int rc;
   if ((rc = use_device(f))) return rc;
+  if ((rc = colour_levels_exit(f))) return rc;
   Span t(f, PK_T_RESAMPLE);
   launch_bal_pack(f->stream, f->d, f->bal, a0, a1 - a0, 0, 0, f->d.P - keep, keep, static_cast<unsigned char*>(dev_buf), record_stride(f),
                   f->grow_on ? &f->grow : nullptr, keep);
@@ -2551,6 +2672,7 @@
   if (!f->bal.rel || !f->d.logical[0]) return fail(PK_ERR_STATE, "pk_shard_adopt_balanced_dev: call pk_shard_plan_balanced_dev first");
   if (f->grow_on && mode != 0) return fail(PK_ERR_STATE, "pk_shard_adopt_balanced_dev: the new-landmark bookkeeping (pk_grow_enable) is adopted whole (mode 0)");
   int rc;
+  if (f->colour_on && ((rc = use_device(f)) || (rc = colour_levels_exit(f)))) return rc;
   const int64_t P = f->d.P;
   if ((rc = balanced_row_check(table, world, P, "pk_shard_adopt_balanced_dev"))) return rc;
   const int row = 2 * world + 4;
@@ -2697,6 +2819,21 @@
   return PK_OK;
 }
 int pk_observe_route(const pk_filter* f) { return f ? f->route : PK_ROUTE_NONE; }
+int pk_colour_levels(pk_filter* f, int64_t out[3]) {
+  if (!f || !out) return fail(PK_ERR_INVALID, "pk_colour_levels: NULL argument");
+  out[0] = f->colour_on ? 1 : 0;
+  out[1] = f->colour_on ? f->ctab_cap : 0;
+  out[2] = 0;
+  if (f->colour_on) {
+    int rc;
+    if ((rc = use_device(f))) return rc;
+    unsigned held = 0;
+    PK_HIP(hipMemcpyAsync(&held, f->cctl, sizeof(unsigned), hipMemcpyDeviceToHost, f->stream));
+    PK_HIP(hipStreamSynchronize(f->stream));
+    out[2] = held;
+  }
+  return PK_OK;
+}
 int pk_observe_flagged(pk_filter* f, int64_t* flagged, int64_t* cand_overflow) {
   if (!f) return fail(PK_ERR_INVALID, "pk_observe_flagged: NULL handle");
   int rc;
diff --git a/parakeet_slam_amd/csrc/pk_k_colour.hip b/parakeet_slam_amd/csrc/pk_k_colour.hip
--- /dev/null
+++ b/parakeet_slam_amd/csrc/pk_k_colour.hip
@@ -0,0 +1,117 @@
+#include <hip/hip_runtime.h>
+
+#include "pk_kernels.hpp"
+#include "pk_math.hpp"
+
+namespace pk {
+
+namespace {
+
+constexpr int kColourThreads = 1024;
+
+__device__ __forceinline__ Sym3<double> colour_tab_load(const double* tab, size_t plane, int Lp, unsigned level, int l) {
+  const double* t = tab + (size_t)level * plane + l;
+  return Sym3<double>{t[0], t[(size_t)Lp], t[2 * (size_t)Lp], t[3 * (size_t)Lp], t[4 * (size_t)Lp], t[5 * (size_t)Lp]};
+}
+__device__ __forceinline__ void colour_tab_store(double* tab, size_t plane, int Lp, unsigned level, int l, const Sym3<double>& c) {
+  double* t = tab + (size_t)level * plane + l;
+  t[0] = c.a;
+  t[(size_t)Lp] = c.b;
+  t[2 * (size_t)Lp] = c.c;
+  t[3 * (size_t)Lp] = c.d;
+  t[4 * (size_t)Lp] = c.e;
+  t[5 * (size_t)Lp] = c.f;
+}
+__device__ __forceinline__ Sym3<double> colour_at(const double* tab, size_t plane, int Lp, unsigned built, unsigned level, int l,
+                                                  const Noise<double>& qt) {
+  const unsigned top = built - 1u;
+  Sym3<double> c = colour_tab_load(tab, plane, Lp, min(level, top), l);
+  for (unsigned k = top; k < level; ++k) c = colour_step(c, qt);
+  return c;
+}
+__device__ __forceinline__ unsigned colour_level(int count) { return (unsigned)(count & ~kPotentialBit) >> 1; }
+
+__device__ __forceinline__ void colour_rows_store(unsigned char* slot, int Lp, int l, const Sym3<double>& c) {
+  double* f = reinterpret_cast<double*>(slot);
+  f[(size_t)F_CRR * Lp + l] = c.a;
+  f[(size_t)F_CRG * Lp + l] = c.b;
+  f[(size_t)F_CRB * Lp + l] = c.c;
+  f[(size_t)F_CGG * Lp + l] = c.d;
+  f[(size_t)F_CGB * Lp + l] = c.e;
+  f[(size_t)F_CBB * Lp + l] = c.f;
+}
+
+__global__ void __launch_bounds__(256) k_colour_level0(const unsigned char* __restrict__ slot, int Lp, double* __restrict__ tab,
+                                                       unsigned* __restrict__ ctl) {
+  const int l = blockIdx.x * blockDim.x + threadIdx.x;
+  if (l < Lp) {
+    const double* f = reinterpret_cast<const double*>(slot);
+    for (int k = 0; k < 6; ++k) tab[(size_t)k * Lp + l] = f[(size_t)(F_CRR + k) * Lp + l];
+  }
+  if (l == 0) {
+    ctl[0] = 1u;
+    ctl[1] = 0u;
+  }
+}
+
+__global__ void __launch_bounds__(kColourThreads) k_colour_extend(double* __restrict__ tab, unsigned* __restrict__ ctl, int cap, int L, int Lp,
+                                                                  Noise<double> qt, SlotSource ss, const int32_t* __restrict__ src, int64_t ref,
+                                                                  size_t count_off) {
+  const unsigned built = ctl[0];
+  const unsigned want = min(ctl[1] + 1u, (unsigned)cap);
+  const size_t plane = 6 * (size_t)Lp;
+  for (int l = threadIdx.x; l < Lp; l += kColourThreads) {
+    if (want > built) {
+      Sym3<double> c = colour_tab_load(tab, plane, Lp, built - 1u, l);
+      for (unsigned v = built; v < want; ++v) {
+        c = colour_step(c, qt);
+        colour_tab_store(tab, plane, Lp, v, l, c);
+      }
+    }
+    if (ref >= 0 && l < L) {
+      unsigned char* slot = const_cast<unsigned char*>(ss.at(src[ref]));
+      const int cnt = reinterpret_cast<const int*>(slot + count_off)[l];
+      colour_rows_store(slot, Lp, l, colour_at(tab, plane, Lp, max(want, built), colour_level(cnt), l, qt));
+    }
+  }
+  __syncthreads();
+  if (threadIdx.x == 0 && want > built) ctl[0] = want;
+}
+
+__global__ void __launch_bounds__(256) k_colour_rows(const double* __restrict__ tab, const unsigned* __restrict__ ctl, int L, int Lp,
+                                                     Noise<double> qt, SlotSource ss, const int32_t* __restrict__ src, size_t count_off,
+                                                     const unsigned char* __restrict__ pflag, const unsigned* __restrict__ n_flagged,
+                                                     int64_t p0, int64_t p1) {
+  if (n_flagged && *n_flagged == 0u) return;
+  const unsigned built = ctl[0];
+  const size_t plane = 6 * (size_t)Lp;
+  for (int64_t p = p0 + blockIdx.x; p < p1; p += gridDim.x) {
+    if (pflag && pflag[p] == 0) continue;
+    unsigned char* slot = const_cast<unsigned char*>(ss.at(src[p]));
+    const int* cnt = reinterpret_cast<const int*>(slot + count_off);
+    for (int l = threadIdx.x; l < L; l += blockDim.x) colour_rows_store(slot, Lp, l, colour_at(tab, plane, Lp, built, colour_level(cnt[l]), l, qt));
+  }
+}
+
+}
+
+void launch_colour_level0(hipStream_t s, const DeviceState& d, const unsigned char* slot_dev, double* tab, unsigned* ctl) {
+  const int Lp = d.lay.Lp;
+  hipLaunchKernelGGL(k_colour_level0, dim3((unsigned)((Lp + 255) / 256)), dim3(256), 0, s, slot_dev, Lp, tab, ctl);
+}
+
+void launch_colour_extend(hipStream_t s, const DeviceState& d, double* tab, unsigned* ctl, int cap, const NoiseD& qt, int64_t ref) {
+  hipLaunchKernelGGL(k_colour_extend, dim3(1), dim3(kColourThreads), 0, s, tab, ctl, cap, d.lay.L, d.lay.Lp,
+                     make_noise(qt.q00, qt.rr, qt.rg, qt.rb, qt.gg, qt.gb, qt.bb), slot_source(d), d.src[d.cur], ref, d.lay.count_off);
+}
+
+void launch_colour_rows(hipStream_t s, const DeviceState& d, const double* tab, const unsigned* ctl, const NoiseD& qt,
+                        const unsigned char* pflag, const unsigned* n_flagged, int64_t p0, int64_t p1) {
+  if (p1 <= p0) return;
+  const int64_t grid = std::min<int64_t>(p1 - p0, pflag ? 2048 : 65536);
+  hipLaunchKernelGGL(k_colour_rows, dim3((unsigned)grid), dim3(256), 0, s, tab, ctl, d.lay.L, d.lay.Lp,
+                     make_noise(qt.q00, qt.rr, qt.rg, qt.rb, qt.gg, qt.gb, qt.bb), slot_source(d), d.src[d.cur], d.lay.count_off, pflag,
+                     n_flagged, p0, p1);
+}
+
+}
diff --git a/parakeet_slam_amd/csrc/pk_k_step_pub.hip b/parakeet_slam_amd/csrc/pk_k_step_pub.hip
--- a/parakeet_slam_amd/csrc/pk_k_step_pub.hip
+++ b/parakeet_slam_amd/csrc/pk_k_step_pub.hip
@@ -49,6 +49,8 @@
   const uint4* prim;
   unsigned* unm;
   int unm_words;
+  const double* ctab = nullptr;
+  unsigned* cctl = nullptr;
 };
 
 constexpr int kPubUnmWords = 176;
@@ -868,6 +870,32 @@
   return e < p_end ? e : p_end;
 }
 #endif
+__device__ __forceinline__ void pub_colour_from_table(Landmark<double>& A, Landmark<double>& B, const double* tab, unsigned built, int Lp, int L,
+                                                      int l0, int* flag) {
+  const unsigned v0 = (unsigned)(A.count & ~kPotentialBit) >> 1, v1 = (unsigned)(B.count & ~kPotentialBit) >> 1;
+  if ((v0 >= built && l0 < L) || (v1 >= built && l0 + 1 < L)) *flag = 1;
+  const int lb = min(l0, Lp - 2);
+  const size_t plane = 6 * (size_t)Lp;
+  const unsigned c0 = min(v0, built - 1u), c1 = min(v1, built - 1u);
+  const double* t0 = tab + (size_t)c0 * plane + lb;
+  if (c0 == c1) {
+    const Double2 rr = *reinterpret_cast<const Double2*>(t0), rg = *reinterpret_cast<const Double2*>(t0 + Lp),
+                  rb = *reinterpret_cast<const Double2*>(t0 + 2 * (size_t)Lp), gg = *reinterpret_cast<const Double2*>(t0 + 3 * (size_t)Lp),
+                  gb = *reinterpret_cast<const Double2*>(t0 + 4 * (size_t)Lp), bb = *reinterpret_cast<const Double2*>(t0 + 5 * (size_t)Lp);
+    A.crr = rr.x, A.crg = rg.x, A.crb = rb.x, A.cgg = gg.x, A.cgb = gb.x, A.cbb = bb.x;
+    B.crr = rr.y, B.crg = rg.y, B.crb = rb.y, B.cgg = gg.y, B.cgb = gb.y, B.cbb = bb.y;
+  } else {
+    const double* t1 = tab + (size_t)c1 * plane + lb + 1;
+    A.crr = t0[0], A.crg = t0[Lp], A.crb = t0[2 * (size_t)Lp], A.cgg = t0[3 * (size_t)Lp], A.cgb = t0[4 * (size_t)Lp], A.cbb = t0[5 * (size_t)Lp];
+    B.crr = t1[0], B.crg = t1[Lp], B.crb = t1[2 * (size_t)Lp], B.cgg = t1[3 * (size_t)Lp], B.cgb = t1[4 * (size_t)Lp], B.cbb = t1[5 * (size_t)Lp];
+  }
+}
+__device__ __forceinline__ unsigned wave_max_u32(unsigned v) {
+#pragma unroll
+  for (int o = kWave / 2; o > 0; o >>= 1) v = max(v, (unsigned)__shfl_xor((int)v, o));
+  return v;
+}
+
 template <int NP, int THREADS>
 __global__ void __launch_bounds__(THREADS, THREADS == 256 ? 3 : 1) k_step_pub(PubArgs a_unused) {
   constexpr int kPubThreads = THREADS, kPubWaves = THREADS / kWave;
@@ -956,10 +984,27 @@
     S[2 * (q_)].field = v_.x;                                                                     \
     S[2 * (q_) + 1].field = v_.y;                                                                 \
   }
-#define PK_PUB_LOAD_MEANS(q_, sslot_, lb_)                                                        \
+#define PK_PUB_COUNTS(q_)                                                                         \
+  {                                                                                               \
+    const Int2 c_ = *reinterpret_cast<const Int2*>(sc_ + lbq_);                                   \
+    S[2 * (q_)].count = c_.x;                                                                     \
+    S[2 * (q_) + 1].count = c_.y;                                                                 \
+  }
+#define PK_PUB_COLOUR_ROWS(q_)                                                                    \
+  if (!pub_args_now(rp)->ctab) {                                                                  \
+    PK_PUB_ROW(q_, crr, F_CRR)                                                                    \
+    PK_PUB_ROW(q_, crg, F_CRG)                                                                    \
+    PK_PUB_ROW(q_, crb, F_CRB)                                                                    \
+    PK_PUB_ROW(q_, cgg, F_CGG)                                                                    \
+    PK_PUB_ROW(q_, cgb, F_CGB)                                                                    \
+    PK_PUB_ROW(q_, cbb, F_CBB)                                                                    \
+  }
+#define PK_PUB_LOAD_MEANS(q_, sslot_, coff_, lb_)                                                 \
   {                                                                                               \
     const double* sf_ = reinterpret_cast<const double*>(sslot_);                                  \
+    const int* sc_ = reinterpret_cast<const int*>((sslot_) + (coff_));                            \
     const int lbq_ = (lb_);                                                                       \
+    PK_PUB_COUNTS(q_)                                                                             \
     PK_PUB_ROW(q_, mx, F_MX)                                                                      \
     PK_PUB_ROW(q_, my, F_MY)                                                                      \
     PK_PUB_ROW(q_, mr, F_MR)                                                                      \
@@ -967,23 +1012,14 @@
     PK_PUB_ROW(q_, mb, F_MB)                                                                      \
     asm volatile("" ::: "memory");                                                                \
   }
-#define PK_PUB_LOAD_COVS(q_, sslot_, coff_, lb_)                                                  \
+#define PK_PUB_LOAD_COVS(q_, sslot_, lb_)                                                         \
   {                                                                                               \
     const double* sf_ = reinterpret_cast<const double*>(sslot_);                                  \
-    const int* sc_ = reinterpret_cast<const int*>((sslot_) + (coff_));                            \
     const int lbq_ = (lb_);                                                                       \
     PK_PUB_ROW(q_, pxx, F_PXX)                                                                    \
     PK_PUB_ROW(q_, pxy, F_PXY)                                                                    \
     PK_PUB_ROW(q_, pyy, F_PYY)                                                                    \
-    PK_PUB_ROW(q_, crr, F_CRR)                                                                    \
-    PK_PUB_ROW(q_, crg, F_CRG)                                                                    \
-    PK_PUB_ROW(q_, crb, F_CRB)                                                                    \
-    PK_PUB_ROW(q_, cgg, F_CGG)                                                                    \
-    PK_PUB_ROW(q_, cgb, F_CGB)                                                                    \
-    PK_PUB_ROW(q_, cbb, F_CBB)                                                                    \
-    const Int2 c_ = *reinterpret_cast<const Int2*>(sc_ + lbq_);                                   \
-    S[2 * (q_)].count = c_.x;                                                                     \
-    S[2 * (q_) + 1].count = c_.y;                                                                 \
+    PK_PUB_COLOUR_ROWS(q_)                                                                        \
     asm volatile("" ::: "memory");                                                                \
   }
 #define PK_PUB_LOAD_PAIR(q_, sslot_, coff_, lb_)                                                  \
@@ -991,6 +1027,7 @@
     const double* sf_ = reinterpret_cast<const double*>(sslot_);                                  \
     const int* sc_ = reinterpret_cast<const int*>((sslot_) + (coff_));                            \
     const int lbq_ = (lb_);                                                                       \
+    PK_PUB_COUNTS(q_)                                                                             \
     PK_PUB_ROW(q_, mx, F_MX)                                                                      \
     PK_PUB_ROW(q_, my, F_MY)                                                                      \
     PK_PUB_ROW(q_, mr, F_MR)                                                                      \
@@ -1000,18 +1037,11 @@
     PK_PUB_ROW(q_, pxx, F_PXX)                                                                    \
     PK_PUB_ROW(q_, pxy, F_PXY)                                                                    \
     PK_PUB_ROW(q_, pyy, F_PYY)                                                                    \
-    PK_PUB_ROW(q_, crr, F_CRR)                                                                    \
-    PK_PUB_ROW(q_, crg, F_CRG)                                                                    \
-    PK_PUB_ROW(q_, crb, F_CRB)                                                                    \
-    PK_PUB_ROW(q_, cgg, F_CGG)                                                                    \
-    PK_PUB_ROW(q_, cgb, F_CGB)                                                                    \
-    PK_PUB_ROW(q_, cbb, F_CBB)                                                                    \
-    const Int2 c_ = *reinterpret_cast<const Int2*>(sc_ + lbq_);                                   \
-    S[2 * (q_)].count = c_.x;                                                                     \
-    S[2 * (q_) + 1].count = c_.y;                                                                 \
+    PK_PUB_COLOUR_ROWS(q_)                                                                        \
     asm volatile("" ::: "memory");                                                                \
   }
   Landmark<double> S[2 * NP];
+  unsigned cmax = 0u;
   constexpr int kPipe = 1;
   unsigned lane_word = (unsigned)tid0;
   if constexpr (kPerm) {
@@ -1090,6 +1120,10 @@
           constexpr int q = decltype(qc)::value;
 
     const int l0 = PK_PUB_L0(q, tid);
+    {
+      PubArgsPtr Rc = pub_args_now(rp);
+      if (Rc->ctab) pub_colour_from_table(S[2 * q], S[2 * q + 1], Rc->ctab, *Rc->cctl, Lp, L, l0, &wg_flag[cur]);
+    }
     const PubGateIn gi[2] = {{cref[2 * q], {ccw[2 * q], ccw[2 * q]}, {cew[2 * q], cew[2 * q]}, S[2 * q].mx, S[2 * q].my,
                               S[2 * q].mr, S[2 * q].mg, S[2 * q].mb, l0 < L},
                              {cref[2 * q + 1], {ccw[2 * q + 1], ccw[2 * q + 1]}, {cew[2 * q + 1], cew[2 * q + 1]},
@@ -1166,12 +1200,11 @@
         if (!done) {
           do_pair(std::integral_constant<int, 0>{});
           if constexpr (NP > 1) {
-            PK_PUB_LOAD_MEANS(1, sslot, lbase[1])
+            PK_PUB_LOAD_MEANS(1, sslot, pub_args_now(rp)->count_off, lbase[1])
             request_cand(NP - 1);
             {
               asm volatile("" ::: "memory");
-              PubArgsPtr R7 = pub_args_now(rp);
-              PK_PUB_LOAD_COVS(1, sslot, R7->count_off, lbase[1])
+              PK_PUB_LOAD_COVS(1, sslot, lbase[1])
             }
             do_pair(std::integral_constant<int, 1>{});
           }
@@ -1285,15 +1318,18 @@
             PK_PUB_STORE(pxx, F_PXX)
             PK_PUB_STORE(pxy, F_PXY)
             PK_PUB_STORE(pyy, F_PYY)
-            PK_PUB_STORE(crr, F_CRR)
-            PK_PUB_STORE(crg, F_CRG)
-            PK_PUB_STORE(crb, F_CRB)
-            PK_PUB_STORE(cgg, F_CGG)
-            PK_PUB_STORE(cgb, F_CGB)
-            PK_PUB_STORE(cbb, F_CBB)
+            if (!pub_args_now(rp)->ctab) {
+              PK_PUB_STORE(crr, F_CRR)
+              PK_PUB_STORE(crg, F_CRG)
+              PK_PUB_STORE(crb, F_CRB)
+              PK_PUB_STORE(cgg, F_CGG)
+              PK_PUB_STORE(cgb, F_CGB)
+              PK_PUB_STORE(cbb, F_CBB)
+            }
 #undef PK_PUB_STORE
             const Int2 c = {S[2 * q].count, S[2 * q + 1].count};
             __builtin_nontemporal_store(c, reinterpret_cast<Int2*>(dc + l0));
+            cmax = max(cmax, (unsigned)max(c.x & ~kPotentialBit, c.y & ~kPotentialBit));
           }
           if (q < kPipe) {
             PubArgsPtr R6 = pub_args_now(rp);
@@ -1326,6 +1362,13 @@
 #ifdef PK_STAMPS
     pst[9] += 1ull;
 #endif
+  }
+  {
+    PubArgsPtr R = pub_args_now(rp);
+    if (R->ctab) {
+      const unsigned m = wave_max_u32(cmax);
+      if ((tid0 & (kWave - 1)) == 0) atomicMax(R->cctl + 1, m >> 1);
+    }
   }
 #ifdef PK_STAMPS
   if ((tid0 & 63) == 0)
@@ -1932,7 +1975,8 @@
 
 void launch_step_pub(hipStream_t s, DeviceState& d, int B, const double* exact_dev, const unsigned short* order_dev,
                      const FastHandoff& fh, const NoiseD& qt, const ObserveExtras& ex, const CandTable& cand, const uint4* erec_dev,
-                     const unsigned* glist_dev, const unsigned* skip_dev, int ecap, int64_t p0, int64_t p1, int reserve_cus) {
+                     const unsigned* glist_dev, const unsigned* skip_dev, int ecap, int64_t p0, int64_t p1, int reserve_cus,
+                     const double* ctab, unsigned* cctl) {
   if (p1 < 0) p1 = d.P;
   if (d.P == 0 || p1 <= p0) return;
   static bool attr_set[kMaxDevices] = {false};
@@ -1975,6 +2019,8 @@
   a.reset = ex.reset ? 1 : 0;
   a.gmax_key = ex.gmax_key;
   a.qt = make_noise(qt.q00, qt.rr, qt.rg, qt.rb, qt.gg, qt.gb, qt.bb);
+  a.ctab = ctab;
+  a.cctl = cctl;
   const int n_cu = device_cu_count();
   const bool small = d.lay.Lp <= 2 * kPubSmallThreads;
   const size_t lds = step_pub_lds_bytes(B, ecap, small);
diff --git a/parakeet_slam_amd/csrc/pk_kernels.hpp b/parakeet_slam_amd/csrc/pk_kernels.hpp
--- a/parakeet_slam_amd/csrc/pk_kernels.hpp
+++ b/parakeet_slam_amd/csrc/pk_kernels.hpp
@@ -198,7 +198,11 @@
 void launch_step_pub(hipStream_t s, DeviceState& d, int B, const double* exact_dev, const unsigned short* order_dev,
                      const FastHandoff& fh, const NoiseD& qt, const ObserveExtras& ex, const CandTable& cand, const uint4* erec_dev,
                      const unsigned* glist_dev, const unsigned* skip_dev, int ecap, int64_t p0 = 0, int64_t p1 = -1,
-                     int reserve_cus = 0);
+                     int reserve_cus = 0, const double* ctab = nullptr, unsigned* cctl = nullptr);
+void launch_colour_level0(hipStream_t s, const DeviceState& d, const unsigned char* slot_dev, double* tab, unsigned* ctl);
+void launch_colour_extend(hipStream_t s, const DeviceState& d, double* tab, unsigned* ctl, int cap, const NoiseD& qt, int64_t ref);
+void launch_colour_rows(hipStream_t s, const DeviceState& d, const double* tab, const unsigned* ctl, const NoiseD& qt,
+                        const unsigned char* pflag, const unsigned* n_flagged, int64_t p0, int64_t p1);
 void launch_flag_range_if(hipStream_t s, const unsigned* over_dev, unsigned char* pflag_dev, unsigned* n_flagged_dev, int64_t p0, int64_t p1);
 constexpr int kPubBigMaxL = 6144;
 int step_pub_big_entry_capacity(int B);
diff --git a/parakeet_slam_amd/csrc/pk_math.hpp b/parakeet_slam_amd/csrc/pk_math.hpp
--- a/parakeet_slam_amd/csrc/pk_math.hpp
+++ b/parakeet_slam_amd/csrc/pk_math.hpp
@@ -223,6 +223,48 @@
 };
 
 template <typename T>
+__device__ __forceinline__ Sym3<T> colour_qci(const Sym3<T>& C, const Noise<T>& qt, Sym3<T>& qc, T& detc) {
+  qc = Sym3<T>{C.a + qt.rr, C.b + qt.rg, C.c + qt.rb, C.d + qt.gg, C.e + qt.gb, C.f + qt.bb};
+  return sym3_inverse(qc, detc);
+}
+template <typename T>
+__device__ __forceinline__ Sym3<T> colour_next(const Sym3<T>& C, const Sym3<T>& qci, const Noise<T>& qt) {
+  T nrr, nrg, nrb, ngg, ngb, nbb;
+  T m00 = qci.a * C.a + qci.b * C.b + qci.c * C.c;
+  T m01 = qci.a * C.b + qci.b * C.d + qci.c * C.e;
+  T m02 = qci.a * C.c + qci.b * C.e + qci.c * C.f;
+  T m11 = qci.b * C.b + qci.d * C.d + qci.e * C.e;
+  T m12 = qci.b * C.c + qci.d * C.e + qci.e * C.f;
+  T m22 = qci.c * C.c + qci.e * C.e + qci.f * C.f;
+  if (qt.diag) {
+    nrr = qt.rr * m00;
+    nrg = qt.rr * m01;
+    nrb = qt.rr * m02;
+    ngg = qt.gg * m11;
+    ngb = qt.gg * m12;
+    nbb = qt.bb * m22;
+  } else {
+    T m10 = qci.b * C.a + qci.d * C.b + qci.e * C.c;
+    T m20 = qci.c * C.a + qci.e * C.b + qci.f * C.c;
+    T m21 = qci.c * C.b + qci.e * C.d + qci.f * C.e;
+    nrr = C.a - (C.a * m00 + C.b * m10 + C.c * m20);
+    nrg = C.b - (C.a * m01 + C.b * m11 + C.c * m21);
+    nrb = C.c - (C.a * m02 + C.b * m12 + C.c * m22);
+    ngg = C.d - (C.b * m01 + C.d * m11 + C.e * m21);
+    ngb = C.e - (C.b * m02 + C.d * m12 + C.e * m22);
+    nbb = C.f - (C.c * m02 + C.e * m12 + C.f * m22);
+  }
+  return Sym3<T>{nrr, nrg, nrb, ngg, ngb, nbb};
+}
+template <typename T>
+__device__ __forceinline__ Sym3<T> colour_step(const Sym3<T>& C, const Noise<T>& qt) {
+  Sym3<T> qc;
+  T detc;
+  const Sym3<T> qci = colour_qci(C, qt, qc, detc);
+  return colour_next(C, qci, qt);
+}
+
+template <typename T>
 __device__ __forceinline__ T ekf_update(Landmark<T>& f, T sx, T sy, const BlobT<T>& z,
                                         const Noise<T>& qt, bool immutable,
                                         EkfAux<T>* aux = nullptr, const T* zhat0_known = nullptr, T* fro_prod = nullptr) {
@@ -241,9 +283,9 @@
   T a0 = f.pxx * h0 + f.pxy * h1;
   T a1 = f.pxy * h0 + f.pyy * h1;
   T q00 = h0 * a0 + h1 * a1 + qt.q00;
-  Sym3<T> qc{f.crr + qt.rr, f.crg + qt.rg, f.crb + qt.rb, f.cgg + qt.gg, f.cgb + qt.gb, f.cbb + qt.bb};
+  Sym3<T> qc;
   T detc;
-  Sym3<T> qci = sym3_inverse(qc, detc);
+  Sym3<T> qci = colour_qci(Sym3<T>{f.crr, f.crg, f.crb, f.cgg, f.cgb, f.cbb}, qt, qc, detc);
   T iq00 = T(1) / q00;
 
   T d0 = z.bearing - zhat0;
@@ -291,43 +333,19 @@
     T nxx = f.pxx - k0 * a0;
     T nxy = f.pxy - T(0.5) * (k0 * a1 + k1 * a0);
     T nyy = f.pyy - k1 * a1;
-    T nrr, nrg, nrb, ngg, ngb, nbb;
-    T m00 = qci.a * f.crr + qci.b * f.crg + qci.c * f.crb;
-    T m01 = qci.a * f.crg + qci.b * f.cgg + qci.c * f.cgb;
-    T m02 = qci.a * f.crb + qci.b * f.cgb + qci.c * f.cbb;
-    T m11 = qci.b * f.crg + qci.d * f.cgg + qci.e * f.cgb;
-    T m12 = qci.b * f.crb + qci.d * f.cgb + qci.e * f.cbb;
-    T m22 = qci.c * f.crb + qci.e * f.cgb + qci.f * f.cbb;
-    if (qt.diag) {
-      nrr = qt.rr * m00;
-      nrg = qt.rr * m01;
-      nrb = qt.rr * m02;
-      ngg = qt.gg * m11;
-      ngb = qt.gg * m12;
-      nbb = qt.bb * m22;
-    } else {
-      T m10 = qci.b * f.crr + qci.d * f.crg + qci.e * f.crb;
-      T m20 = qci.c * f.crr + qci.e * f.crg + qci.f * f.crb;
-      T m21 = qci.c * f.crg + qci.e * f.cgg + qci.f * f.cgb;
-      nrr = f.crr - (f.crr * m00 + f.crg * m10 + f.crb * m20);
-      nrg = f.crg - (f.crr * m01 + f.crg * m11 + f.crb * m21);
-      nrb = f.crb - (f.crr * m02 + f.crg * m12 + f.crb * m22);
-      ngg = f.cgg - (f.crg * m01 + f.cgg * m11 + f.cgb * m21);
-      ngb = f.cgb - (f.crg * m02 + f.cgg * m12 + f.cgb * m22);
-      nbb = f.cbb - (f.crb * m02 + f.cgb * m12 + f.cbb * m22);
-    }
+    const Sym3<T> nc = colour_next(Sym3<T>{f.crr, f.crg, f.crb, f.cgg, f.cgb, f.cbb}, qci, qt);
     f.mr = nr;
     f.mg = ng;
     f.mb = nb;
     f.pxx = nxx;
     f.pxy = nxy;
     f.pyy = nyy;
-    f.crr = nrr;
-    f.crg = nrg;
-    f.crb = nrb;
-    f.cgg = ngg;
-    f.cgb = ngb;
-    f.cbb = nbb;
+    f.crr = nc.a;
+    f.crg = nc.b;
+    f.crb = nc.c;
+    f.cgg = nc.d;
+    f.cgb = nc.e;
+    f.cbb = nc.f;
     count_update(f.count);
   }
   return logw;
```

Measured after the change: 26.84 billion, median of 6. 4.0% higher.
